# iDC-NEU/NeutronStarLite

Measured on NVIDIA H100. Metric: gcn_aggregated_edges_per_sec, higher is better.
Workload: dtype f32

## Files before the change

### include/nts_b200.h

```cpp
#ifndef NTS_B200_H
#define NTS_B200_H

#include <stddef.h>
#include <stdint.h>

#ifdef __cplusplus
extern "C" {
#endif

typedef uint32_t nts_vid_t;

int nts_version(void);
const char *nts_last_error(void);
int nts_device_count(void);
int nts_set_device(int device);
int nts_device_sm_count(int *sm_count);
int nts_device_synchronize(void);
int nts_device_reset(void);

void *nts_malloc_device(size_t bytes);
int nts_free_device(void *ptr);
void *nts_malloc_pinned(size_t bytes);
int nts_free_pinned(void *ptr);
void *nts_pinned_device_pointer(void *host_ptr);
int nts_memcpy_h2d(void *dst_device, const void *src_host, size_t bytes, void *stream, int sync);
int nts_memcpy_d2h(void *dst_host, const void *src_device, size_t bytes, void *stream, int sync);
int nts_memcpy_d2d(void *dst_device, const void *src_device, size_t bytes, void *stream);
int nts_zero(void *device_ptr, size_t bytes, void *stream);

void *nts_stream_create(int non_blocking);
int nts_stream_destroy(void *stream);
int nts_stream_synchronize(void *stream);
void *nts_event_create(int with_timing);
int nts_event_destroy(void *event);
int nts_event_record(void *event, void *stream);
int nts_stream_wait_event(void *stream, void *event);
int nts_event_elapsed_ms(void *start, void *stop, float *ms);

int nts_segment_gather_sum(const float *input, float *output, const float *weight,
                           const nts_vid_t *indices, const nts_vid_t *offsets, nts_vid_t index_base,
                           nts_vid_t n_rows, uint64_t n_edges, nts_vid_t feature_size, void *stream);

int nts_gather_by_dst_from_src(const float *input, float *output, const float *weight_forward,
                               const nts_vid_t *row_indices, const nts_vid_t *column_offset,
                               nts_vid_t src_start, nts_vid_t src_end, nts_vid_t dst_start,
                               nts_vid_t dst_end, nts_vid_t edges, nts_vid_t batch_size,
                               nts_vid_t feature_size, int with_weight, void *stream);

int nts_gather_by_src_from_dst(const float *input, float *output, const float *weight_backward,
                               const nts_vid_t *row_offset, const nts_vid_t *column_indices,
                               nts_vid_t src_start, nts_vid_t src_end, nts_vid_t dst_start,
                               nts_vid_t dst_end, nts_vid_t edges, nts_vid_t batch_size,
                               nts_vid_t feature_size, int with_weight, void *stream);

int nts_segment_gather_sum_range(const float *input, float *output, const float *weight, const nts_vid_t *indices,
                                 const nts_vid_t *offsets, const nts_vid_t *slot_of, nts_vid_t index_base,
                                 nts_vid_t n_rows, uint64_t edge_begin, uint64_t edge_end, nts_vid_t feature_size,
                                 void *stream);

typedef struct nts_gather_plan nts_gather_plan;
int nts_gather_plan_pick_slabs(nts_vid_t gather_rows, uint64_t n_edges, nts_vid_t n_rows, nts_vid_t feature_size,
                               uint64_t l2_budget_bytes );
nts_gather_plan *nts_gather_plan_create(const nts_vid_t *offsets, const nts_vid_t *indices, const float *weight,
                                        const nts_vid_t *slot_of, nts_vid_t index_base, nts_vid_t n_rows,
                                        uint64_t n_edges, nts_vid_t gather_rows, int n_slabs, void *stream);
nts_gather_plan *nts_gather_plan_create_hybrid(const nts_vid_t *offsets, const nts_vid_t *indices,
                                               const float *weight, const nts_vid_t *slot_of, nts_vid_t index_base,
                                               nts_vid_t n_rows, uint64_t n_edges, nts_vid_t gather_rows, int n_slabs,
                                               int n_hub_cols, int n_hub_rows, void *stream);
nts_gather_plan *nts_gather_plan_create_tuned(const nts_vid_t *offsets, const nts_vid_t *indices, const float *weight,
                                              const nts_vid_t *slot_of, nts_vid_t index_base, nts_vid_t n_rows,
                                              uint64_t n_edges, nts_vid_t gather_rows, nts_vid_t feature_size,
                                              void *stream);
typedef struct nts_plan_part {
  const nts_vid_t *offsets, *indices;
  const float *weight;
  const nts_vid_t *slot_of;
  nts_vid_t index_base, index_add, n_rows, row_add;
  uint64_t n_edges;
} nts_plan_part;
nts_gather_plan *nts_gather_plan_create_parts(const nts_plan_part *parts, int n_parts, nts_vid_t n_rows,
                                              nts_vid_t gather_rows, int n_slabs, nts_vid_t feature_size, void *stream);
float nts_gather_plan_tuned_ms(const nts_gather_plan *plan);
int nts_gather_plan_destroy(nts_gather_plan *plan);
int nts_gather_plan_slabs(const nts_gather_plan *plan);
int nts_gather_plan_hubs(const nts_gather_plan *plan, int *cols, int *rows);
int nts_gather_plan_overlap(const nts_gather_plan *plan);
int nts_gather_plan_set_overlap(nts_gather_plan *plan, int overlap);
uint64_t nts_gather_plan_bytes(const nts_gather_plan *plan);
int nts_gather_plan_run(nts_gather_plan *plan, const float *input, float *output, nts_vid_t feature_size,
                        void *stream);
int nts_gather_plan_last_launch(const nts_gather_plan *plan, int *launches, int *grid, int *k, int *u, int *outv);
enum { NTS_DTYPE_F32 = 0, NTS_DTYPE_BF16 = 1 };
int nts_gather_plan_run_bf16(nts_gather_plan *plan, const void *input, int input_dtype, float *output,
                             nts_vid_t feature_size, void *stream);
nts_gather_plan *nts_gather_plan_create_tuned_bf16(const nts_vid_t *offsets, const nts_vid_t *indices,
                                                   const float *weight, const nts_vid_t *slot_of, nts_vid_t index_base,
                                                   nts_vid_t n_rows, uint64_t n_edges, nts_vid_t gather_rows,
                                                   nts_vid_t feature_size, void *stream);
int nts_gather_plan_set_tuning(int u, int min_blocks, int edges_per_warp);
int nts_gather_plan_set_variant(int variant);

int nts_segment_gather_sum_slots(const float *input, float *output, const float *weight,
                                 const nts_vid_t *indices, const nts_vid_t *offsets,
                                 const nts_vid_t *slot_of, nts_vid_t n_rows, uint64_t n_edges,
                                 nts_vid_t feature_size, void *stream);

int nts_segment_gather_sum_heads(const float *input, float *output, const float *weight,
                                 const nts_vid_t *indices, const nts_vid_t *offsets, const nts_vid_t *slot_of,
                                 nts_vid_t index_base, nts_vid_t n_rows, uint64_t n_edges,
                                 nts_vid_t feature_size, nts_vid_t heads, void *stream);

int nts_aggregate_set_variant(int variant, int edges_per_warp);
int nts_aggregate_last_launch(int *grid, int *block, int *smem_bytes, int *variant);
uint64_t nts_kernel_launch_count(void);

int nts_scatter_src_mirror_to_msg(float *message, const float *src_mirror_feature,
                                  const nts_vid_t *row_indices, const nts_vid_t *column_offset,
                                  const nts_vid_t *mirror_index, nts_vid_t batch_size,
                                  nts_vid_t feature_size, void *stream);
int nts_gather_msg_to_src_mirror(float *src_mirror_feature, const float *message,
                                 const nts_vid_t *row_indices, const nts_vid_t *column_offset,
                                 const nts_vid_t *mirror_index, nts_vid_t batch_size,
                                 nts_vid_t feature_size, void *stream);
int nts_scatter_dst_to_msg(float *message, const float *dst_feature, const nts_vid_t *row_indices,
                           const nts_vid_t *column_offset, nts_vid_t batch_size,
                           nts_vid_t feature_size, void *stream);
int nts_gather_msg_to_dst(float *dst_feature, const float *message, const nts_vid_t *row_indices,
                          const nts_vid_t *column_offset, nts_vid_t batch_size,
                          nts_vid_t feature_size, void *stream);
int nts_edge_softmax_forward(float *msg_output, const float *msg_input, float *msg_cached,
                             const nts_vid_t *row_indices, const nts_vid_t *column_offset,
                             nts_vid_t batch_size, nts_vid_t feature_size, void *stream);
int nts_edge_softmax_backward(float *msg_input_grad, const float *msg_output_grad,
                              const float *msg_cached, const nts_vid_t *row_indices,
                              const nts_vid_t *column_offset, nts_vid_t batch_size,
                              nts_vid_t feature_size, void *stream);
int nts_scatter_grad_back_to_message(const float *input, float *message_grad,
                                     const nts_vid_t *row_indices, const nts_vid_t *column_offset,
                                     nts_vid_t batch_size, nts_vid_t feature_size, void *stream);

int nts_aggregate_dst_fuse_weight_backward(float *mirror_grad, float *edge_weight_grad,
                                           const float *mirror, const float *edge_weight,
                                           const float *dst_grad, const nts_vid_t *row_indices,
                                           const nts_vid_t *column_offset,
                                           const nts_vid_t *mirror_index, nts_vid_t batch_size,
                                           nts_vid_t feature_size, void *stream);
int nts_aggregate_dst_fuse_weight_backward_heads(float *mirror_grad, float *edge_weight_grad,
                                                 const float *mirror, const float *edge_weight,
                                                 const float *dst_grad, const nts_vid_t *row_indices,
                                                 const nts_vid_t *column_offset,
                                                 const nts_vid_t *mirror_index, nts_vid_t batch_size,
                                                 nts_vid_t feature_size, nts_vid_t heads, void *stream);

int nts_gat_softmax_stats(float *seg_max, float *seg_sum, const float *src_score, const float *dst_score,
                          const nts_vid_t *row_indices, const nts_vid_t *column_offset,
                          const nts_vid_t *mirror_index, nts_vid_t batch_size, nts_vid_t heads,
                          float negative_slope, void *stream);
int nts_gat_fused_aggregate_forward(const float *mirror, float *output, const float *src_score,
                                    const float *dst_score, const float *seg_max, const float *seg_sum,
                                    const nts_vid_t *row_indices, const nts_vid_t *column_offset,
                                    const nts_vid_t *mirror_index, nts_vid_t batch_size, uint64_t n_edges,
                                    nts_vid_t feature_size, nts_vid_t heads, float negative_slope, void *stream);
int nts_gat_fused_aggregate_backward(float *mirror_grad, float *src_score_grad, float *dst_score_grad,
                                     const float *mirror, const float *src_score, const float *dst_score,
                                     const float *seg_max, const float *seg_sum, const float *out_dot_grad,
                                     const float *dst_grad, const nts_vid_t *row_indices,
                                     const nts_vid_t *column_offset, const nts_vid_t *mirror_index,
                                     nts_vid_t batch_size, nts_vid_t feature_size, nts_vid_t heads,
                                     float negative_slope, void *stream);
int nts_gat_fused_aggregate_backward_two_pass(float *mirror_grad, float *src_score_grad, float *dst_score_grad,
                                              float *dst_pack, const float *mirror, const float *src_score,
                                              const float *dst_score, const float *seg_max, const float *seg_sum,
                                              const float *out_dot_grad, const float *dst_grad,
                                              const nts_vid_t *row_indices, const nts_vid_t *column_offset,
                                              const nts_vid_t *mirror_index, const nts_vid_t *slot_row_offset,
                                              const nts_vid_t *slot_column_indices, nts_vid_t batch_size,
                                              nts_vid_t mirror_size, nts_vid_t feature_size, nts_vid_t heads,
                                              float negative_slope, void *stream);
int nts_gat_fused_aggregate_forward_bf16(const void *mirror, float *output, const float *src_score,
                                         const float *dst_score, const float *seg_max, const float *seg_sum,
                                         const nts_vid_t *row_indices, const nts_vid_t *column_offset,
                                         const nts_vid_t *mirror_index, nts_vid_t batch_size, uint64_t n_edges,
                                         nts_vid_t feature_size, nts_vid_t ld, nts_vid_t heads, float negative_slope,
                                         void *stream);
int nts_gat_fused_aggregate_backward_two_pass_bf16(float *mirror_grad, float *src_score_grad, float *dst_score_grad,
                                                   float *dst_pack, const void *mirror, const float *src_score,
                                                   const float *dst_score, const float *seg_max, const float *seg_sum,
                                                   const float *out_dot_grad, const void *dst_grad,
                                                   const nts_vid_t *row_indices, const nts_vid_t *column_offset,
                                                   const nts_vid_t *mirror_index, const nts_vid_t *slot_row_offset,
                                                   const nts_vid_t *slot_column_indices, nts_vid_t batch_size,
                                                   nts_vid_t mirror_size, nts_vid_t feature_size, nts_vid_t ld,
                                                   nts_vid_t heads, float negative_slope, void *stream);
int nts_rows_to_bf16(const void *src, int src_dtype, nts_vid_t lds, void *dst, nts_vid_t n_rows, nts_vid_t feature_size,
                     nts_vid_t ld, void *stream);

int nts_deserialize_records(float *mirror, const float *records, nts_vid_t n_records,
                            nts_vid_t feature_size, nts_vid_t partition_start,
                            nts_vid_t partition_end, void *stream);
int nts_aggregate_records(float *aggregate, const float *records, nts_vid_t n_records,
                          nts_vid_t feature_size, nts_vid_t partition_start,
                          nts_vid_t partition_end, void *stream);

int nts_gather_rows(float *dst, const float *src, const nts_vid_t *rows, nts_vid_t n_rows,
                    nts_vid_t feature_size, void *stream);
int nts_scatter_add_rows(float *dst, const float *src, const nts_vid_t *rows, nts_vid_t n_rows,
                         nts_vid_t feature_size, void *stream);
int nts_scatter_add_rows_atomic(float *dst, const float *src, const nts_vid_t *rows, nts_vid_t n_rows,
                                nts_vid_t feature_size, void *stream);

int nts_adam_update(float *W, float *M, float *V, const float *grad, uint64_t n, float weight_decay, float beta1,
                    float beta2, float alpha, float epsilon, void *stream);

#define NTS_IPC_HANDLE_BYTES 64
int nts_ipc_get_handle(void *device_ptr, unsigned char handle[NTS_IPC_HANDLE_BYTES]);
void *nts_ipc_open_handle(const unsigned char handle[NTS_IPC_HANDLE_BYTES]);
int nts_ipc_close_handle(void *peer_ptr);
int nts_signal_set(uint32_t *flag, uint32_t value, void *stream);
int nts_signal_wait_geq(const uint32_t *flag, uint32_t value, void *stream);

typedef struct nts_exchange nts_exchange;
typedef struct nts_exchange_chunk {
  const nts_vid_t *column_offset;
  const nts_vid_t *slots;
  const float *weight_forward;
  const nts_vid_t *row_offset_compact;
  const nts_vid_t *column_indices;
  const float *weight_backward;
  uint64_t edges;
} nts_exchange_chunk;
typedef struct nts_exchange_desc {
  int partitions, rank;
  nts_vid_t owned_vertices, dst_start;
  const nts_vid_t *local_column_offset, *local_row_indices, *local_row_offset, *local_column_indices;
  const float *local_weight_forward, *local_weight_backward;
  nts_vid_t local_edges;
  const nts_exchange_chunk *chunks;
  const nts_vid_t *need_count;
  const nts_vid_t *send_count;
  const nts_vid_t *send_rows_all;
  const nts_vid_t *fwd_push_offset;
  const nts_vid_t *bwd_push_offset;
  const nts_vid_t *local_need;
  nts_vid_t local_need_count;
} nts_exchange_desc;

nts_exchange *nts_exchange_create(const nts_exchange_desc *desc);
int nts_exchange_destroy(nts_exchange *ex);
uint64_t nts_exchange_required_floats(const nts_exchange *ex, nts_vid_t feature_size);
uint64_t nts_exchange_required_floats_bf16(const nts_exchange *ex, nts_vid_t feature_size);
uint64_t nts_exchange_capacity_floats(const nts_exchange *ex);
int nts_exchange_release_peers(nts_exchange *ex);
int nts_exchange_reserve(nts_exchange *ex, uint64_t floats_per_buffer, int n_buffers);
int nts_exchange_handles(nts_exchange *ex, unsigned char window_handle[64], unsigned char flags_handle[64]);
int nts_exchange_open_peers(nts_exchange *ex, const unsigned char *window_handles, const unsigned char *flag_handles);
int nts_exchange_forward(nts_exchange *ex, const float *x, float *y, nts_vid_t feature_size, void *stream);
int nts_exchange_backward(nts_exchange *ex, const float *g, float *dx, nts_vid_t feature_size, void *stream);
int nts_exchange_forward_bf16(nts_exchange *ex, const void *x, int x_dtype, float *y, nts_vid_t feature_size,
                              void *stream);
int nts_exchange_backward_bf16(nts_exchange *ex, const float *g, float *dx, nts_vid_t feature_size, void *stream);
int nts_exchange_set_trace(nts_exchange *ex, int enable);
int nts_exchange_last_timeline(nts_exchange *ex, float *ms, int capacity);
int nts_exchange_fetch_mirrors(nts_exchange *ex, const float *x, float *mirror, nts_vid_t feature_size, void *stream);
int nts_exchange_return_mirror_grads(nts_exchange *ex, const float *mirror_grad, float *dx, nts_vid_t feature_size,
                                     void *stream);

typedef struct nts_host_chunk {
  const nts_vid_t *column_offset, *row_indices, *row_offset, *column_indices;
  const float *edge_weight_forward, *edge_weight_backward;
  nts_vid_t src_start, src_end, dst_start, dst_end;
  uint64_t edges;
} nts_host_chunk;
typedef struct nts_exchange_plan nts_exchange_plan;
nts_exchange_plan *nts_exchange_plan_create(const nts_host_chunk *chunks, int partitions, int rank);
void nts_exchange_plan_destroy(nts_exchange_plan *plan);
const nts_vid_t *nts_exchange_plan_need(const nts_exchange_plan *plan, int i, nts_vid_t *count);
uint64_t nts_exchange_plan_packed_rows(const nts_exchange_plan *plan);
int nts_exchange_plan_pack_needs(const nts_exchange_plan *plan, nts_vid_t *need_counts, nts_vid_t *need_rows);
int nts_exchange_plan_set_peer_needs(nts_exchange_plan *plan, int j, const nts_vid_t *need_counts,
                                     const nts_vid_t *need_rows);
int nts_exchange_plan_finalize(nts_exchange_plan *plan);
typedef struct nts_exchange_plan_view {
  int partitions, rank;
  nts_vid_t owned_vertices, recv_total, send_total, backward_rows;
  uint64_t remote_edges;
  const nts_vid_t *need_count, *send_count, *peer_bwd_offset;
  const nts_vid_t *fwd_push_offset, *bwd_push_offset;
  const nts_vid_t *remote_column_offset, *remote_slots;
  const float *remote_weight;
  const nts_vid_t *backward_offsets, *backward_indices;
  const float *backward_weight;
  const nts_vid_t *send_rows_all;
} nts_exchange_plan_view;
int nts_exchange_plan_get_view(const nts_exchange_plan *plan, nts_exchange_plan_view *view);
int nts_exchange_plan_chunk(const nts_exchange_plan *plan, int i, const nts_vid_t **slots,
                            const nts_vid_t **row_offset_compact);
typedef struct nts_device_chunk {
  const nts_vid_t *column_offset, *row_indices, *row_offset, *column_indices;
  const float *edge_weight_forward, *edge_weight_backward;
} nts_device_chunk;
nts_exchange *nts_exchange_create_from_plan(nts_exchange_plan *plan, const nts_device_chunk *device_chunks);

int nts_host_degrees(const nts_vid_t *edges_src_dst, uint64_t n_edges, nts_vid_t n_vertices,
                     nts_vid_t *out_degree, nts_vid_t *in_degree);
int nts_host_partition_offsets(const nts_vid_t *edges_src_dst, uint64_t n_edges, nts_vid_t n_vertices,
                               int partitions, nts_vid_t *partition_offset);
int nts_host_chunk_edge_counts(const nts_vid_t *edges_src_dst, uint64_t n_edges,
                               const nts_vid_t *partition_offset, int partitions, int rank,
                               uint64_t *counts);
int nts_host_build_chunk(const nts_vid_t *edges_src_dst, uint64_t n_edges, nts_vid_t n_vertices,
                         const nts_vid_t *partition_offset, int partitions, int rank, int src_partition,
                         const nts_vid_t *out_degree, const nts_vid_t *in_degree,
                         nts_vid_t *column_offset, nts_vid_t *row_indices, float *edge_weight_forward,
                         nts_vid_t *row_offset, nts_vid_t *column_indices, float *edge_weight_backward,
                         unsigned char *source_active);
int nts_host_mirror_index(const nts_vid_t *edges_src_dst, uint64_t n_edges, nts_vid_t n_vertices,
                          const nts_vid_t *partition_offset, int rank, nts_vid_t *mirror_index,
                          nts_vid_t *owned);

typedef struct nts_graph_build nts_graph_build;
enum { NTS_GRAPH_BUILD_DIST = 1 };
enum { NTS_INDEX_I32 = 0, NTS_INDEX_I64 = 1 };
nts_graph_build *nts_graph_build_from_file(const char *path, nts_vid_t n_vertices, int partitions, int rank,
                                           const nts_vid_t *partition_offset, uint64_t block_edges, int flags,
                                           void *stream);
nts_graph_build *nts_graph_build_from_device(const void *src, const void *dst, int index_dtype, uint64_t n_edges,
                                             nts_vid_t n_vertices, int partitions, int rank,
                                             const nts_vid_t *partition_offset, const void *out_degree,
                                             const void *in_degree, int flags, void *stream);
int nts_graph_build_info(const nts_graph_build *build, nts_vid_t *partition_offset, uint64_t *chunk_edges,
                         nts_vid_t *owned_mirrors, uint64_t *scratch_peak_bytes, double *pass_seconds);
int nts_graph_build_export_chunk(const nts_graph_build *build, int i, nts_vid_t *column_offset, nts_vid_t *row_indices,
                                 float *edge_weight_forward, nts_vid_t *row_offset, nts_vid_t *column_indices,
                                 float *edge_weight_backward, unsigned char *source_active, void *stream);
int nts_graph_build_export_dist(const nts_graph_build *build, nts_vid_t *mirror_index, nts_vid_t *column_offset,
                                nts_vid_t *row_indices, void *stream);
int nts_graph_build_export_degrees(const nts_graph_build *build, nts_vid_t *out_degree, nts_vid_t *in_degree,
                                   void *stream);
int nts_graph_build_destroy(nts_graph_build *build);

int nts_host_read_feature_label_mask(const char *feature_path, const char *label_path, const char *mask_path,
                                     nts_vid_t feature_size, nts_vid_t v_begin, nts_vid_t v_end, float *features,
                                     int64_t *labels, int32_t *masks);
int nts_host_read_feature_binary(const char *path, nts_vid_t feature_size, nts_vid_t v_begin, nts_vid_t v_end,
                                 float *features);

#ifdef __cplusplus
}
#endif
#endif
```

### neutronstarlite_b200/_lib.py

```python
from __future__ import annotations

import ctypes as C
import os
import re

PKG = os.path.dirname(os.path.abspath(__file__))
ROOT = os.path.dirname(PKG)
LIB_PATH = os.path.join(PKG, "lib", "libnts_b200.so")
HEADER = os.path.join(ROOT, "include", "nts_b200.h")

_vp = C.c_void_p
_u32 = C.c_uint32
_u64 = C.c_uint64
_int = C.c_int
_sz = C.c_size_t

SIGNATURES = {
    "nts_version": (_int, []),
    "nts_last_error": (C.c_char_p, []),
    "nts_device_count": (_int, []),
    "nts_set_device": (_int, [_int]),
    "nts_device_sm_count": (_int, [C.POINTER(_int)]),
    "nts_device_synchronize": (_int, []),
    "nts_device_reset": (_int, []),
    "nts_malloc_device": (_vp, [_sz]),
    "nts_free_device": (_int, [_vp]),
    "nts_malloc_pinned": (_vp, [_sz]),
    "nts_free_pinned": (_int, [_vp]),
    "nts_pinned_device_pointer": (_vp, [_vp]),
    "nts_memcpy_h2d": (_int, [_vp, _vp, _sz, _vp, _int]),
    "nts_memcpy_d2h": (_int, [_vp, _vp, _sz, _vp, _int]),
    "nts_memcpy_d2d": (_int, [_vp, _vp, _sz, _vp]),
    "nts_zero": (_int, [_vp, _sz, _vp]),
    "nts_stream_create": (_vp, [_int]),
    "nts_stream_destroy": (_int, [_vp]),
    "nts_stream_synchronize": (_int, [_vp]),
    "nts_event_create": (_vp, [_int]),
    "nts_event_destroy": (_int, [_vp]),
    "nts_event_record": (_int, [_vp, _vp]),
    "nts_stream_wait_event": (_int, [_vp, _vp]),
    "nts_event_elapsed_ms": (_int, [_vp, _vp, C.POINTER(C.c_float)]),
    "nts_segment_gather_sum": (_int, [_vp, _vp, _vp, _vp, _vp, _u32, _u32, _u64, _u32, _vp]),
    "nts_gather_by_dst_from_src": (_int, [_vp, _vp, _vp, _vp, _vp, _u32, _u32, _u32, _u32, _u32, _u32, _u32, _int, _vp]),
    "nts_gather_by_src_from_dst": (_int, [_vp, _vp, _vp, _vp, _vp, _u32, _u32, _u32, _u32, _u32, _u32, _u32, _int, _vp]),
    "nts_segment_gather_sum_range": (_int, [_vp, _vp, _vp, _vp, _vp, _vp, _u32, _u32, _u64, _u64, _u32, _vp]),
    "nts_gather_plan_pick_slabs": (_int, [_u32, _u64, _u32, _u32, _u64]),
    "nts_gather_plan_create": (_vp, [_vp, _vp, _vp, _vp, _u32, _u32, _u64, _u32, _int, _vp]),
    "nts_gather_plan_create_hybrid": (_vp, [_vp, _vp, _vp, _vp, _u32, _u32, _u64, _u32, _int, _int, _int, _vp]),
    "nts_gather_plan_create_tuned": (_vp, [_vp, _vp, _vp, _vp, _u32, _u32, _u64, _u32, _u32, _vp]),
    "nts_gather_plan_create_parts": (_vp, [_vp, _int, _u32, _u32, _int, _u32, _vp]),
    "nts_gather_plan_tuned_ms": (C.c_float, [_vp]),
    "nts_gather_plan_destroy": (_int, [_vp]),
    "nts_gather_plan_slabs": (_int, [_vp]),
    "nts_gather_plan_hubs": (_int, [_vp, C.POINTER(_int), C.POINTER(_int)]),
    "nts_gather_plan_overlap": (_int, [_vp]),
    "nts_gather_plan_set_overlap": (_int, [_vp, _int]),
    "nts_gather_plan_bytes": (_u64, [_vp]),
    "nts_gather_plan_run": (_int, [_vp, _vp, _vp, _u32, _vp]),
    "nts_gather_plan_run_bf16": (_int, [_vp, _vp, _int, _vp, _u32, _vp]),
    "nts_gather_plan_create_tuned_bf16": (_vp, [_vp, _vp, _vp, _vp, _u32, _u32, _u64, _u32, _u32, _vp]),
    "nts_gather_plan_last_launch": (_int, [_vp] + [C.POINTER(_int)] * 5),
    "nts_gather_plan_set_tuning": (_int, [_int, _int, _int]),
    "nts_gather_plan_set_variant": (_int, [_int]),
    "nts_segment_gather_sum_slots": (_int, [_vp, _vp, _vp, _vp, _vp, _vp, _u32, _u64, _u32, _vp]),
    "nts_segment_gather_sum_heads": (_int, [_vp, _vp, _vp, _vp, _vp, _vp, _u32, _u32, _u64, _u32, _u32, _vp]),
    "nts_aggregate_set_variant": (_int, [_int, _int]),
    "nts_aggregate_last_launch": (_int, [C.POINTER(_int)] * 4),
    "nts_kernel_launch_count": (_u64, []),
    "nts_scatter_src_mirror_to_msg": (_int, [_vp, _vp, _vp, _vp, _vp, _u32, _u32, _vp]),
    "nts_gather_msg_to_src_mirror": (_int, [_vp, _vp, _vp, _vp, _vp, _u32, _u32, _vp]),
    "nts_scatter_dst_to_msg": (_int, [_vp, _vp, _vp, _vp, _u32, _u32, _vp]),
    "nts_gather_msg_to_dst": (_int, [_vp, _vp, _vp, _vp, _u32, _u32, _vp]),
    "nts_edge_softmax_forward": (_int, [_vp, _vp, _vp, _vp, _vp, _u32, _u32, _vp]),
    "nts_edge_softmax_backward": (_int, [_vp, _vp, _vp, _vp, _vp, _u32, _u32, _vp]),
    "nts_scatter_grad_back_to_message": (_int, [_vp, _vp, _vp, _vp, _u32, _u32, _vp]),
    "nts_aggregate_dst_fuse_weight_backward": (_int, [_vp, _vp, _vp, _vp, _vp, _vp, _vp, _vp, _u32, _u32, _vp]),
    "nts_aggregate_dst_fuse_weight_backward_heads": (_int, [_vp] * 8 + [_u32, _u32, _u32, _vp]),
    "nts_gat_softmax_stats": (_int, [_vp] * 7 + [_u32, _u32, C.c_float, _vp]),
    "nts_gat_fused_aggregate_forward": (_int, [_vp] * 9 + [_u32, _u64, _u32, _u32, C.c_float, _vp]),
    "nts_gat_fused_aggregate_backward": (_int, [_vp] * 13 + [_u32, _u32, _u32, C.c_float, _vp]),
    "nts_gat_fused_aggregate_backward_two_pass": (_int, [_vp] * 16 + [_u32, _u32, _u32, _u32, C.c_float, _vp]),
    "nts_gat_fused_aggregate_forward_bf16": (_int, [_vp] * 9 + [_u32, _u64, _u32, _u32, _u32, C.c_float, _vp]),
    "nts_gat_fused_aggregate_backward_two_pass_bf16": (_int, [_vp] * 16 + [_u32] * 5 + [C.c_float, _vp]),
    "nts_rows_to_bf16": (_int, [_vp, _int, _u32, _vp, _u32, _u32, _u32, _vp]),
    "nts_deserialize_records": (_int, [_vp, _vp, _u32, _u32, _u32, _u32, _vp]),
    "nts_aggregate_records": (_int, [_vp, _vp, _u32, _u32, _u32, _u32, _vp]),
    "nts_gather_rows": (_int, [_vp, _vp, _vp, _u32, _u32, _vp]),
    "nts_scatter_add_rows": (_int, [_vp, _vp, _vp, _u32, _u32, _vp]),
    "nts_scatter_add_rows_atomic": (_int, [_vp, _vp, _vp, _u32, _u32, _vp]),
    "nts_ipc_get_handle": (_int, [_vp, C.c_char_p]),
    "nts_ipc_open_handle": (_vp, [C.c_char_p]),
    "nts_ipc_close_handle": (_int, [_vp]),
    "nts_adam_update": (_int, [_vp, _vp, _vp, _vp, _u64] + [C.c_float] * 5 + [_vp]),
    "nts_signal_set": (_int, [_vp, _u32, _vp]),
    "nts_signal_wait_geq": (_int, [_vp, _u32, _vp]),
    "nts_host_degrees": (_int, [_vp, _u64, _u32, _vp, _vp]),
    "nts_host_partition_offsets": (_int, [_vp, _u64, _u32, _int, _vp]),
    "nts_host_chunk_edge_counts": (_int, [_vp, _u64, _vp, _int, _int, _vp]),
    "nts_host_build_chunk": (_int, [_vp, _u64, _u32, _vp, _int, _int, _int, _vp, _vp, _vp, _vp, _vp, _vp, _vp, _vp, _vp]),
    "nts_host_mirror_index": (_int, [_vp, _u64, _u32, _vp, _int, _vp, _vp]),
    "nts_host_read_feature_label_mask": (_int, [C.c_char_p, C.c_char_p, C.c_char_p, _u32, _u32, _u32, _vp, _vp, _vp]),
    "nts_host_read_feature_binary": (_int, [C.c_char_p, _u32, _u32, _u32, _vp]),
    "nts_graph_build_from_file": (_vp, [C.c_char_p, _u32, _int, _int, _vp, _u64, _int, _vp]),
    "nts_graph_build_from_device": (_vp, [_vp, _vp, _int, _u64, _u32, _int, _int, _vp, _vp, _vp, _int, _vp]),
    "nts_graph_build_info": (_int, [_vp] * 6),
    "nts_graph_build_export_chunk": (_int, [_vp, _int] + [_vp] * 8),
    "nts_graph_build_export_dist": (_int, [_vp] * 5),
    "nts_graph_build_export_degrees": (_int, [_vp] * 4),
    "nts_graph_build_destroy": (_int, [_vp]),
}



class ExchangeChunk(C.Structure):
    _fields_ = [
        ("column_offset", _vp), ("slots", _vp), ("weight_forward", _vp), ("row_offset_compact", _vp),
        ("column_indices", _vp), ("weight_backward", _vp), ("edges", _u64),
    ]


class ExchangeDesc(C.Structure):
    _fields_ = [
        ("partitions", _int), ("rank", _int), ("owned_vertices", _u32), ("dst_start", _u32),
        ("local_column_offset", _vp), ("local_row_indices", _vp), ("local_row_offset", _vp),
        ("local_column_indices", _vp), ("local_weight_forward", _vp), ("local_weight_backward", _vp),
        ("local_edges", _u32),
        ("chunks", C.POINTER(ExchangeChunk)),
        ("need_count", C.POINTER(_u32)), ("send_count", C.POINTER(_u32)),
        ("send_rows_all", _vp), ("fwd_push_offset", C.POINTER(_u32)), ("bwd_push_offset", C.POINTER(_u32)),
        ("local_need", _vp), ("local_need_count", _u32),
    ]


class DeviceChunk(C.Structure):
    _fields_ = [
        ("column_offset", _vp), ("row_indices", _vp), ("row_offset", _vp), ("column_indices", _vp),
        ("edge_weight_forward", _vp), ("edge_weight_backward", _vp),
    ]


SIGNATURES.update({
    "nts_exchange_create": (_vp, [C.POINTER(ExchangeDesc)]),
    "nts_exchange_destroy": (_int, [_vp]),
    "nts_exchange_required_floats": (_u64, [_vp, _u32]),
    "nts_exchange_capacity_floats": (_u64, [_vp]),
    "nts_exchange_release_peers": (_int, [_vp]),
    "nts_exchange_reserve": (_int, [_vp, _u64, _int]),
    "nts_exchange_handles": (_int, [_vp, C.c_char_p, C.c_char_p]),
    "nts_exchange_open_peers": (_int, [_vp, C.c_char_p, C.c_char_p]),
    "nts_exchange_forward": (_int, [_vp, _vp, _vp, _u32, _vp]),
    "nts_exchange_backward": (_int, [_vp, _vp, _vp, _u32, _vp]),
    "nts_exchange_forward_bf16": (_int, [_vp, _vp, _int, _vp, _u32, _vp]),
    "nts_exchange_backward_bf16": (_int, [_vp, _vp, _vp, _u32, _vp]),
    "nts_exchange_required_floats_bf16": (_u64, [_vp, _u32]),
    "nts_exchange_set_trace": (_int, [_vp, _int]),
    "nts_exchange_last_timeline": (_int, [_vp, C.POINTER(C.c_float), _int]),
    "nts_exchange_fetch_mirrors": (_int, [_vp, _vp, _vp, _u32, _vp]),
    "nts_exchange_return_mirror_grads": (_int, [_vp, _vp, _vp, _u32, _vp]),
})



class HostChunk(C.Structure):
    _fields_ = [
        ("column_offset", _vp), ("row_indices", _vp), ("row_offset", _vp), ("column_indices", _vp),
        ("edge_weight_forward", _vp), ("edge_weight_backward", _vp),
        ("src_start", _u32), ("src_end", _u32), ("dst_start", _u32), ("dst_end", _u32), ("edges", _u64),
    ]


class ExchangePlanView(C.Structure):
    _fields_ = [
        ("partitions", _int), ("rank", _int),
        ("owned_vertices", _u32), ("recv_total", _u32), ("send_total", _u32), ("backward_rows", _u32),
        ("remote_edges", _u64),
        ("need_count", C.POINTER(_u32)), ("send_count", C.POINTER(_u32)), ("peer_bwd_offset", C.POINTER(_u32)),
        ("fwd_push_offset", C.POINTER(_u32)), ("bwd_push_offset", C.POINTER(_u32)),
        ("remote_column_offset", C.POINTER(_u32)), ("remote_slots", C.POINTER(_u32)),
        ("remote_weight", C.POINTER(C.c_float)),
        ("backward_offsets", C.POINTER(_u32)), ("backward_indices", C.POINTER(_u32)),
        ("backward_weight", C.POINTER(C.c_float)),
        ("send_rows_all", C.POINTER(_u32)),
    ]


SIGNATURES.update({
    "nts_exchange_plan_create": (_vp, [C.POINTER(HostChunk), _int, _int]),
    "nts_exchange_plan_destroy": (None, [_vp]),
    "nts_exchange_plan_need": (C.POINTER(_u32), [_vp, _int, C.POINTER(_u32)]),
    "nts_exchange_plan_packed_rows": (_u64, [_vp]),
    "nts_exchange_plan_pack_needs": (_int, [_vp, _vp, _vp]),
    "nts_exchange_plan_set_peer_needs": (_int, [_vp, _int, _vp, _vp]),
    "nts_exchange_plan_finalize": (_int, [_vp]),
    "nts_exchange_plan_get_view": (_int, [_vp, C.POINTER(ExchangePlanView)]),
    "nts_exchange_plan_chunk": (_int, [_vp, _int, C.POINTER(C.POINTER(_u32)), C.POINTER(C.POINTER(_u32))]),
    "nts_exchange_create_from_plan": (_vp, [_vp, C.POINTER(DeviceChunk)]),
})

_lib = None


class NtsError(RuntimeError):
    pass


def header_symbols():
    text = open(HEADER).read()
    text = re.sub(r"/\*.*?\*/", "", text, flags=re.S)
    return sorted(set(re.findall(r"\b(nts_[a-z0-9_]+)\s*\(", text)))


def load():
    global _lib
    if _lib is not None:
        return _lib
    if not os.path.exists(LIB_PATH):
        raise NtsError("libnts_b200.so not found at %s - run `python -m neutronstarlite_b200.build` "
                       "(there is no CPU fallback)" % LIB_PATH)
    lib = C.CDLL(LIB_PATH, mode=C.RTLD_GLOBAL)
    for name, (res, args) in SIGNATURES.items():
        fn = getattr(lib, name)
        fn.restype = res
        fn.argtypes = args
    _lib = lib
    return lib


def check(rc, what=""):
    if rc != 0:
        msg = load().nts_last_error().decode(errors="replace")
        raise NtsError("libnts_b200 %s failed (rc=%d): %s" % (what, rc, msg))


def call(name, *args):
    rc = getattr(load(), name)(*args)
    check(rc, name)
```

### neutronstarlite_b200/csrc/nts_common.cuh

```cuda
#pragma once
#include <cuda_bf16.h>
#include <cuda_runtime.h>
#include <stdint.h>
#include <stdio.h>
#include <stdlib.h>
#include <string.h>

#include "nts_b200.h"

namespace nts {

char *last_error_buffer();
bool abort_on_error();
void count_launch();

inline int fail(int code, const char *what, const char *file, int line) {
  snprintf(last_error_buffer(), 512, "%s (%s:%d)", what, file, line);
  if (abort_on_error()) {
    fprintf(stderr, "libnts_b200: %s\n", last_error_buffer());
    exit(1);
  }
  return code;
}

#define NTS_CUDA_OK(expr)                                                                         \
  do {                                                                                            \
    cudaError_t nts_e_ = (expr);                                                                  \
    if (nts_e_ != cudaSuccess)                                                                    \
      return ::nts::fail((int)nts_e_, cudaGetErrorString(nts_e_), __FILE__, __LINE__);            \
  } while (0)

#define NTS_ARG_CHECK(cond, msg)                                                                  \
  do {                                                                                            \
    if (!(cond))                                                                                  \
      return ::nts::fail(-1, msg, __FILE__, __LINE__);                                            \
  } while (0)

#define NTS_LAUNCH_CHECK()                                                                        \
  do {                                                                                            \
    ::nts::count_launch();                                                                        \
    NTS_CUDA_OK(cudaGetLastError());                                                              \
  } while (0)

inline cudaStream_t as_stream(void *s) { return reinterpret_cast<cudaStream_t>(s); }

inline bool aligned_to(const void *p, size_t a) { return (reinterpret_cast<uintptr_t>(p) & (a - 1)) == 0; }

int sm_count();

int run_plan_bf16(nts_gather_plan *pl, const void *input, int dtype, uint32_t lds, float *output, uint32_t F,
                  cudaStream_t st);
int to_bf16_rows(const void *src, int dtype, uint32_t lds, void *dst, uint32_t n_rows, uint32_t F, uint32_t ld,
                 cudaStream_t st);

int check_gat_bf16_layout(uint32_t F, uint32_t ld, uint32_t heads);

struct __align__(16) float8v {
  float4 lo, hi;
};

template <int VEC> struct Vec;
template <> struct Vec<1> { using type = float; };
template <> struct Vec<2> { using type = float2; };
template <> struct Vec<4> { using type = float4; };
template <> struct Vec<8> { using type = float8v; };

template <class T, int VEC> struct Ld { using type = typename Vec<VEC>::type; };
template <> struct Ld<__nv_bfloat16, 2> { using type = uint32_t; };
template <> struct Ld<__nv_bfloat16, 4> { using type = uint2; };
template <> struct Ld<__nv_bfloat16, 8> { using type = uint4; };
__device__ __forceinline__ float widen(float v) { return v; }
__device__ __forceinline__ float2 widen(float2 v) { return v; }
__device__ __forceinline__ float4 widen(float4 v) { return v; }
__device__ __forceinline__ float2 widen(uint32_t u) {
  return make_float2(__uint_as_float(u << 16), __uint_as_float(u & 0xffff0000u));
}
__device__ __forceinline__ float4 widen(uint2 u) {
  const float2 a = widen(u.x), b = widen(u.y);
  return make_float4(a.x, a.y, b.x, b.y);
}
__device__ __forceinline__ float8v widen(uint4 u) { return {widen(make_uint2(u.x, u.y)), widen(make_uint2(u.z, u.w))}; }

}

extern "C" nts_gather_plan *nts_plan_create_parts_typed(const nts_plan_part *parts, int n_parts, nts_vid_t n_rows,
                                                        nts_vid_t gather_rows, int n_slabs, nts_vid_t feature_size,
                                                        int bf16, void *stream);
```

### neutronstarlite_b200/csrc/nts_plan.cu

```cuda
#include <cub/cub.cuh>
#include <cuda_bf16.h>

#include <algorithm>
#include <type_traits>
#include <vector>

#include "nts_common.cuh"

struct nts_gather_plan {
  uint32_t n_rows = 0;
  uint64_t n_edges = 0;
  uint32_t gather_rows = 0;
  int slabs = 1;
  uint32_t slab_rows = 0;
  uint2 *pairs = nullptr;
  uint32_t *voff = nullptr;
  std::vector<uint64_t> slab_edge;
  float *workspace = nullptr;
  size_t workspace_floats = 0;
  __nv_bfloat16 *workspace_bf16 = nullptr;
  size_t workspace_bf16_elems = 0;
  int hub_cols = 0, hub_rows = 0;
  uint32_t *hub_col_ids = nullptr;
  uint32_t *hub_row_ids = nullptr;
  uint32_t lda_c = 0, lda_r = 0;
  float *dense = nullptr;
  size_t dense_floats = 0;
  int overlap = 0;
  int last_grid = 0, last_launches = 0, last_k = 0, last_u = 0, last_outv = 0;
  float tuned_ms = 0.f;
};

namespace nts {

static int g_plan_u = 0, g_plan_minb = 0, g_plan_q = 0, g_plan_variant = 0;

__device__ __forceinline__ uint32_t plan_find_row(const uint32_t *__restrict__ off, uint32_t n_rows, uint32_t e) {
  uint32_t lo = 0, hi = n_rows;
  while (hi - lo > 1) {
    uint32_t mid = lo + ((hi - lo) >> 1);
    if (__ldg(off + mid) <= e)
      lo = mid;
    else
      hi = mid;
  }
  return lo;
}

__global__ void plan_keys_kernel(const uint32_t *__restrict__ off, const uint32_t *__restrict__ idx,
                                 const uint32_t *__restrict__ slot_of, uint32_t base, uint32_t n_rows, uint32_t n_edges,
                                 uint32_t slab_rows, uint32_t slabs, uint32_t *__restrict__ key,
                                 uint32_t *__restrict__ val) {
  for (uint64_t e = (uint64_t)blockIdx.x * blockDim.x + threadIdx.x; e < n_edges; e += (uint64_t)gridDim.x * blockDim.x) {
    const uint32_t r = plan_find_row(off, n_rows, (uint32_t)e);
    const uint32_t id = __ldg(idx + e);
    const uint32_t g = slot_of ? __ldg(slot_of + id) : id - base;
    uint32_t s = g / slab_rows;
    if (s >= slabs)
      s = slabs - 1;
    key[e] = s * n_rows + r;
    val[e] = (uint32_t)e;
  }
}

__global__ void plan_pairs_kernel(const uint32_t *__restrict__ perm, const uint32_t *__restrict__ idx,
                                  const float *__restrict__ w, const uint32_t *__restrict__ slot_of, uint32_t base,
                                  uint32_t n_edges, uint2 *__restrict__ pairs) {
  for (uint64_t i = (uint64_t)blockIdx.x * blockDim.x + threadIdx.x; i < n_edges; i += (uint64_t)gridDim.x * blockDim.x) {
    const uint32_t e = perm ? __ldg(perm + i) : (uint32_t)i;
    const uint32_t id = __ldg(idx + e);
    const uint32_t g = slot_of ? __ldg(slot_of + id) : id - base;
    const float wt = w ? __ldg(w + e) : 1.f;
    pairs[i] = make_uint2(g, __float_as_uint(wt));
  }
}

__global__ void plan_part_keys_kernel(const uint32_t *__restrict__ off, const uint32_t *__restrict__ idx,
                                      const uint32_t *__restrict__ slot_of, const float *__restrict__ w, uint32_t base,
                                      uint32_t index_add, uint32_t n_rows_part, uint32_t row_add, uint32_t n_edges,
                                      uint32_t e_off, uint32_t n_rows_total, uint32_t slab_rows, uint32_t slabs,
                                      uint32_t *__restrict__ key, uint32_t *__restrict__ val,
                                      uint2 *__restrict__ unsorted) {
  for (uint64_t e = (uint64_t)blockIdx.x * blockDim.x + threadIdx.x; e < n_edges; e += (uint64_t)gridDim.x * blockDim.x) {
    const uint32_t r = plan_find_row(off, n_rows_part, (uint32_t)e) + row_add;
    const uint32_t id = __ldg(idx + e);
    const uint32_t g = (slot_of ? __ldg(slot_of + id) : id - base) + index_add;
    uint32_t s = g / slab_rows;
    if (s >= slabs)
      s = slabs - 1;
    key[e_off + e] = s * n_rows_total + r;
    val[e_off + e] = e_off + (uint32_t)e;
    unsorted[e_off + e] = make_uint2(g, __float_as_uint(w ? __ldg(w + e) : 1.f));
  }
}
__global__ void plan_permute_pairs_kernel(const uint32_t *__restrict__ perm, const uint2 *__restrict__ unsorted,
                                          uint32_t n_edges, uint2 *__restrict__ pairs) {
  for (uint64_t i = (uint64_t)blockIdx.x * blockDim.x + threadIdx.x; i < n_edges; i += (uint64_t)gridDim.x * blockDim.x)
    pairs[i] = unsorted[__ldg(perm + i)];
}

template <class KeyT>
__global__ void plan_offsets_kernel(const KeyT *__restrict__ sorted_key, uint32_t n_edges, uint32_t n_keys,
                                    uint32_t *__restrict__ voff) {
  for (uint64_t k = (uint64_t)blockIdx.x * blockDim.x + threadIdx.x; k <= n_keys; k += (uint64_t)gridDim.x * blockDim.x) {
    uint32_t lo = 0, hi = n_edges;
    while (lo < hi) {
      uint32_t mid = lo + ((hi - lo) >> 1);
      if (__ldg(sorted_key + mid) < (KeyT)k)
        lo = mid + 1;
      else
        hi = mid;
    }
    voff[k] = lo;
  }
}

constexpr uint32_t kNoHub = 0xffffffffu;

__global__ void plan_ref_count_kernel(const uint32_t *__restrict__ idx, const uint32_t *__restrict__ slot_of,
                                      uint32_t base, uint32_t n_edges, uint32_t *__restrict__ cnt) {
  for (uint64_t e = (uint64_t)blockIdx.x * blockDim.x + threadIdx.x; e < n_edges; e += (uint64_t)gridDim.x * blockDim.x) {
    const uint32_t id = __ldg(idx + e);
    atomicAdd(cnt + (slot_of ? __ldg(slot_of + id) : id - base), 1u);
  }
}

__global__ void plan_hybrid_keys_kernel(const uint32_t *__restrict__ off, const uint32_t *__restrict__ idx,
                                        const uint32_t *__restrict__ slot_of, uint32_t base, uint32_t n_rows,
                                        uint32_t n_edges, uint32_t slab_rows, uint32_t slabs,
                                        const uint32_t *__restrict__ col_slot, const uint32_t *__restrict__ row_slot,
                                        uint32_t lda_c, uint64_t dc_cells, uint32_t lda_r, uint64_t *__restrict__ key,
                                        uint32_t *__restrict__ val) {
  const uint64_t n_keys = (uint64_t)slabs * n_rows;
  for (uint64_t e = (uint64_t)blockIdx.x * blockDim.x + threadIdx.x; e < n_edges; e += (uint64_t)gridDim.x * blockDim.x) {
    const uint32_t r = plan_find_row(off, n_rows, (uint32_t)e);
    const uint32_t id = __ldg(idx + e);
    const uint32_t g = slot_of ? __ldg(slot_of + id) : id - base;
    const uint32_t cs = __ldg(col_slot + g), rs = __ldg(row_slot + r);
    uint64_t k;
    if (cs != kNoHub) {
      k = n_keys + (uint64_t)cs * lda_c + r;
    } else if (rs != kNoHub) {
      k = n_keys + dc_cells + (uint64_t)g * lda_r + rs;
    } else {
      uint32_t s = g / slab_rows;
      if (s >= slabs)
        s = slabs - 1;
      k = (uint64_t)s * n_rows + r;
    }
    key[e] = k;
    val[e] = (uint32_t)e;
  }
}

__global__ void plan_cell_sum_kernel(const uint64_t *__restrict__ cell_key, const uint32_t *__restrict__ run_start,
                                     const uint32_t *__restrict__ run_len, uint32_t n_runs,
                                     const uint32_t *__restrict__ perm, const float *__restrict__ w, uint64_t n_keys,
                                     float *__restrict__ dense) {
  const uint32_t lane = threadIdx.x & 31;
  for (uint64_t run = ((uint64_t)blockIdx.x * blockDim.x + threadIdx.x) >> 5; run < n_runs;
       run += ((uint64_t)gridDim.x * blockDim.x) >> 5) {
    const uint32_t b = __ldg(run_start + run), n = __ldg(run_len + run);
    float s = 0.f;
    for (uint32_t j = lane; j < n; j += 32)
      s += w ? __ldg(w + __ldg(perm + b + j)) : 1.f;
#pragma unroll
    for (int o = 16; o > 0; o >>= 1)
      s += __shfl_xor_sync(0xffffffffu, s, o);
    if (lane == 0)
      dense[__ldg(cell_key + run) - n_keys] = s;
  }
}

__global__ void pad_rows_kernel(const float *__restrict__ src, float *__restrict__ dst, uint32_t n_rows, uint32_t F,
                                uint32_t ld) {
  const uint64_t total = (uint64_t)n_rows * ld;
  for (uint64_t i = (uint64_t)blockIdx.x * blockDim.x + threadIdx.x; i < total; i += (uint64_t)gridDim.x * blockDim.x) {
    const uint64_t r = i / ld;
    const uint32_t c = (uint32_t)(i - r * ld);
    dst[i] = c < F ? __ldg(src + r * F + c) : 0.f;
  }
}

template <class S>
__global__ void bf16_rows_kernel(const S *__restrict__ src, uint32_t lds, uint4 *__restrict__ dst, uint32_t n_rows,
                                 uint32_t F, uint32_t ld) {
  const uint32_t ld8 = ld / 8;
  const uint64_t total = (uint64_t)n_rows * ld8;
  for (uint64_t i = (uint64_t)blockIdx.x * blockDim.x + threadIdx.x; i < total; i += (uint64_t)gridDim.x * blockDim.x) {
    const uint64_t r = i / ld8;
    const uint32_t c = (uint32_t)(i - r * ld8) * 8;
    const S *s = src + r * lds;
    uint32_t w[4];
#pragma unroll
    for (int j = 0; j < 4; j++) {
      const uint32_t c0 = c + 2 * j, c1 = c0 + 1;
      if constexpr (std::is_same<S, float>::value) {
        const __nv_bfloat162 h = __floats2bfloat162_rn(c0 < F ? __ldg(s + c0) : 0.f, c1 < F ? __ldg(s + c1) : 0.f);
        w[j] = *reinterpret_cast<const uint32_t *>(&h);
      } else {
        const uint16_t *u = reinterpret_cast<const uint16_t *>(s);
        w[j] = (c0 < F ? (uint32_t)__ldg(u + c0) : 0u) | ((c1 < F ? (uint32_t)__ldg(u + c1) : 0u) << 16);
      }
    }
    dst[i] = make_uint4(w[0], w[1], w[2], w[3]);
  }
}

__device__ __forceinline__ uint32_t p_smem_u32(const void *p) { return (uint32_t)__cvta_generic_to_shared(p); }
__device__ __forceinline__ void p_mbar_init(uint64_t *bar, uint32_t count) {
  asm volatile("mbarrier.init.shared::cta.b64 [%0], %1;" ::"r"(p_smem_u32(bar)), "r"(count));
}
__device__ __forceinline__ void p_mbar_expect_tx(uint64_t *bar, uint32_t bytes) {
  asm volatile("mbarrier.arrive.expect_tx.shared::cta.b64 _, [%0], %1;" ::"r"(p_smem_u32(bar)), "r"(bytes) : "memory");
}
__device__ __forceinline__ void p_mbar_wait(uint64_t *bar, uint32_t parity) {
  asm volatile("{\n\t"
               ".reg .pred p;\n\t"
               "WAIT_%=:\n\t"
               "mbarrier.try_wait.parity.shared::cta.b64 p, [%0], %1;\n\t"
               "@p bra DONE_%=;\n\t"
               "bra WAIT_%=;\n\t"
               "DONE_%=:\n\t"
               "}" ::"r"(p_smem_u32(bar)),
               "r"(parity)
               : "memory");
}
__device__ __forceinline__ void p_bulk_g2s(void *smem_dst, const void *gmem_src, uint32_t bytes, uint64_t *bar) {
  asm volatile("cp.async.bulk.shared::cluster.global.mbarrier::complete_tx::bytes [%0], [%1], %2, [%3];" ::"r"(
                   p_smem_u32(smem_dst)),
               "l"(gmem_src), "r"(bytes), "r"(p_smem_u32(bar))
               : "memory");
}

constexpr int kPlanWarps = 8;

template <int OUTV, bool ATOMIC>
__device__ __forceinline__ void flush_chunk(float *__restrict__ orow, uint32_t col, uint32_t F, float4 a) {
  if constexpr (OUTV == 4) {
    float4 *p = reinterpret_cast<float4 *>(orow + col);
    if constexpr (ATOMIC) {
      asm volatile("red.global.add.v4.f32 [%0], {%1, %2, %3, %4};" ::"l"(p), "f"(a.x), "f"(a.y), "f"(a.z), "f"(a.w)
                   : "memory");
    } else {
      float4 o = *p;
      o.x += a.x, o.y += a.y, o.z += a.z, o.w += a.w;
      *p = o;
    }
  } else if constexpr (OUTV == 2) {
    float2 *p = reinterpret_cast<float2 *>(orow + col);
    if constexpr (ATOMIC) {
      asm volatile("red.global.add.v2.f32 [%0], {%1, %2};" ::"l"(p), "f"(a.x), "f"(a.y) : "memory");
      if (col + 2 < F)
        asm volatile("red.global.add.v2.f32 [%0], {%1, %2};" ::"l"(p + 1), "f"(a.z), "f"(a.w) : "memory");
    } else {
      float2 o = p[0];
      o.x += a.x, o.y += a.y;
      p[0] = o;
      if (col + 2 < F) {
        float2 o1 = p[1];
        o1.x += a.z, o1.y += a.w;
        p[1] = o1;
      }
    }
  } else {
    const float v[4] = {a.x, a.y, a.z, a.w};
#pragma unroll
    for (int i = 0; i < 4; i++)
      if (col + i < F) {
        if constexpr (ATOMIC)
          atomicAdd(orow + col + i, v[i]);
        else
          orow[col + i] += v[i];
      }
  }
}

template <class T> struct GatherT;
template <> struct GatherT<float> {
  using chunk = float4;
  static constexpr int V = 4;
  __device__ static __forceinline__ void widen(const float4 &c, float (&v)[4]) {
    v[0] = c.x, v[1] = c.y, v[2] = c.z, v[3] = c.w;
  }
};
template <> struct GatherT<__nv_bfloat16> {
  using chunk = uint4;
  static constexpr int V = 8;
  __device__ static __forceinline__ void widen(const uint4 &c, float (&v)[8]) {
    const uint32_t u[4] = {c.x, c.y, c.z, c.w};
#pragma unroll
    for (int i = 0; i < 4; i++) {
      v[2 * i] = __uint_as_float(u[i] << 16);
      v[2 * i + 1] = __uint_as_float(u[i] & 0xffff0000u);
    }
  }
};

template <class T, int K, int U, int OUTV, int G>
__device__ __forceinline__ void planned_gather_body(unsigned char *smem_raw, uint32_t vblock,
                                                    const typename GatherT<T>::chunk *__restrict__ in, uint32_t ldc,
                                                    float *__restrict__ out, uint32_t F,
                                                    const uint2 *__restrict__ pairs, const uint32_t *__restrict__ off,
                                                    uint32_t n_rows, uint32_t e_begin, uint32_t e_end, uint32_t Q,
                                                    uint32_t tiles, uint32_t tile_vecs) {
  static_assert(G == 1 || K == 1, "virtual warps are for rows narrower than a warp");
  using Chunk = typename GatherT<T>::chunk;
  constexpr int V = GatherT<T>::V;
  constexpr uint32_t GS = 32 / G;
  const uint32_t lane = threadIdx.x & (GS - 1);
  const uint32_t vwarp_in_block = threadIdx.x / GS;
  const uint64_t gwarp = (uint64_t)vblock * (kPlanWarps * G) + vwarp_in_block;
  const uint32_t tile = (uint32_t)(gwarp % tiles);
  const uint64_t q = gwarp / tiles;
  const uint64_t e0_64 = e_begin + q * (uint64_t)Q;

  uint64_t *bar = reinterpret_cast<uint64_t *>(smem_raw);
  uint2 *s_pair = reinterpret_cast<uint2 *>(smem_raw + 16);
  uint32_t cta_e_base = 0, bulk_bytes = 0;
  {
    const uint64_t cta_w0 = (uint64_t)vblock * (kPlanWarps * G);
    const uint64_t first_q = cta_w0 / tiles;
    const uint64_t last_q = (cta_w0 + kPlanWarps * G - 1) / tiles;
    uint64_t ce0 = e_begin + first_q * (uint64_t)Q;
    uint64_t ce1 = e_begin + (last_q + 1) * (uint64_t)Q;
    if (ce1 > e_end)
      ce1 = e_end;
    if (ce0 < ce1) {
      cta_e_base = (uint32_t)(ce0 & ~1ull);
      const uint32_t n_el = (uint32_t)(ce1 - cta_e_base);
      bulk_bytes = (n_el * 8u) & ~15u;
      if (threadIdx.x == 0) {
        p_mbar_init(bar, 1);
        asm volatile("fence.mbarrier_init.release.cluster;" ::: "memory");
        if (n_el & 1u)
          s_pair[n_el - 1] = __ldg(pairs + cta_e_base + n_el - 1);
      }
      __syncthreads();
      if (threadIdx.x == 0 && bulk_bytes) {
        p_mbar_expect_tx(bar, bulk_bytes);
        p_bulk_g2s(s_pair, pairs + cta_e_base, bulk_bytes, bar);
      }
    }
  }
  if (e0_64 >= e_end)
    return;
  const uint32_t e0 = (uint32_t)e0_64;
  const uint32_t e1 = (e0_64 + Q < e_end) ? e0 + Q : e_end;

  const uint32_t c0 = tile * tile_vecs + lane;
  bool act[K];
#pragma unroll
  for (int k = 0; k < K; k++)
    act[k] = (k * GS + lane) < tile_vecs && (c0 + k * GS) < ldc;

  uint32_t row = plan_find_row(off, n_rows, e0);
  uint32_t row_end = __ldg(off + row + 1);
  bool row_started_inside = __ldg(off + row) >= e0;

  float acc[K][V];
#pragma unroll
  for (int k = 0; k < K; k++)
#pragma unroll
    for (int j = 0; j < V; j++)
      acc[k][j] = 0.f;

  auto flush = [&](bool whole) {
    float *orow = out + (size_t)row * F;
#pragma unroll
    for (int k = 0; k < K; k++) {
#pragma unroll
      for (int h = 0; h < V; h += 4) {
        const uint32_t col = (c0 + k * GS) * V + h;
        const float4 a = make_float4(acc[k][h], acc[k][h + 1], acc[k][h + 2], acc[k][h + 3]);
        if (act[k] && col < F) {
          if (whole)
            flush_chunk<OUTV, false>(orow, col, F, a);
          else
            flush_chunk<OUTV, true>(orow, col, F, a);
        }
      }
#pragma unroll
      for (int j = 0; j < V; j++)
        acc[k][j] = 0.f;
    }
  };
  auto advance = [&](uint32_t ee) {
    flush(row_started_inside);
    do {
      row++;
      row_end = __ldg(off + row + 1);
    } while (ee >= row_end);
    row_started_inside = true;
  };

  if (bulk_bytes)
    p_mbar_wait(bar, 0);

  const uint2 *sp = s_pair - cta_e_base;
  uint32_t e = e0;
  auto fma_chunk = [&](int k, float w, const Chunk &c) {
    float x[V];
    GatherT<T>::widen(c, x);
#pragma unroll
    for (int j = 0; j < V; j++)
      acc[k][j] = fmaf(w, x[j], acc[k][j]);
  };
  for (; e + U <= e1; e += U) {
    Chunk v[U][K];
    float wu[U];
#pragma unroll
    for (int u = 0; u < U; u++) {
      const uint2 pr = sp[e + u];
      wu[u] = __uint_as_float(pr.y);
      const Chunk *p = in + (size_t)pr.x * ldc + c0;
#pragma unroll
      for (int k = 0; k < K; k++)
        if (act[k])
          v[u][k] = __ldg(p + k * GS);
    }
#pragma unroll
    for (int u = 0; u < U; u++) {
      if (e + u >= row_end)
        advance(e + u);
#pragma unroll
      for (int k = 0; k < K; k++)
        if (act[k])
          fma_chunk(k, wu[u], v[u][k]);
    }
  }
  for (; e < e1; e++) {
    const uint2 pr = sp[e];
    const float wj = __uint_as_float(pr.y);
    const Chunk *p = in + (size_t)pr.x * ldc + c0;
    Chunk v1[K];
#pragma unroll
    for (int k = 0; k < K; k++)
      if (act[k])
        v1[k] = __ldg(p + k * GS);
    if (e >= row_end)
      advance(e);
#pragma unroll
    for (int k = 0; k < K; k++)
      if (act[k])
        fma_chunk(k, wj, v1[k]);
  }
  flush(row_started_inside && row_end <= e1);
}

template <class T, int K, int U, int OUTV, int MINB, int G = 1>
__global__ void __launch_bounds__(kPlanWarps * 32, MINB)
    planned_gather_sum_kernel(const typename GatherT<T>::chunk *__restrict__ in, uint32_t ldc, float *__restrict__ out,
                              uint32_t F, const uint2 *__restrict__ pairs, const uint32_t *__restrict__ off,
                              uint32_t n_rows, uint32_t e_begin, uint32_t e_end, uint32_t Q, uint32_t tiles,
                              uint32_t tile_vecs) {
  extern __shared__ __align__(16) unsigned char smem_raw[];
  planned_gather_body<T, K, U, OUTV, G>(smem_raw, blockIdx.x, in, ldc, out, F, pairs, off, n_rows, e_begin, e_end, Q,
                                        tiles, tile_vecs);
}

struct PlanShape;
template <int K, int STAGES, int OUTV, int MINB>
__global__ void __launch_bounds__(kPlanWarps * 32, MINB)
    planned_gather_sum_tma_kernel(const float4 *__restrict__ in, uint32_t ld4, float *__restrict__ out, uint32_t F,
                                  const uint2 *__restrict__ pairs, const uint32_t *__restrict__ off, uint32_t n_rows,
                                  uint32_t e_begin, uint32_t e_end, uint32_t Q, uint32_t tiles, uint32_t tile_vecs,
                                  uint32_t pair_bytes) {
  const uint32_t lane = threadIdx.x & 31;
  const uint32_t warp_in_block = threadIdx.x >> 5;
  const uint64_t gwarp = (uint64_t)blockIdx.x * kPlanWarps + warp_in_block;
  const uint32_t tile = (uint32_t)(gwarp % tiles);
  const uint64_t q = gwarp / tiles;
  const uint64_t e0_64 = e_begin + q * (uint64_t)Q;

  extern __shared__ __align__(16) unsigned char smem_raw[];
  uint64_t *bar = reinterpret_cast<uint64_t *>(smem_raw);
  uint2 *s_pair = reinterpret_cast<uint2 *>(smem_raw + 16);
  const uint32_t ring_bytes = 8u * STAGES + 8u * (STAGES & 1) + STAGES * tile_vecs * 16u;
  unsigned char *ring = smem_raw + 16 + pair_bytes + (size_t)warp_in_block * ring_bytes;
  uint64_t *sbar = reinterpret_cast<uint64_t *>(ring);
  float4 *sbuf = reinterpret_cast<float4 *>(ring + 8u * STAGES + 8u * (STAGES & 1));
  uint32_t cta_e_base = 0, bulk_bytes = 0;
  {
    const uint64_t cta_w0 = (uint64_t)blockIdx.x * kPlanWarps;
    const uint64_t first_q = cta_w0 / tiles;
    const uint64_t last_q = (cta_w0 + kPlanWarps - 1) / tiles;
    uint64_t ce0 = e_begin + first_q * (uint64_t)Q;
    uint64_t ce1 = e_begin + (last_q + 1) * (uint64_t)Q;
    if (ce1 > e_end)
      ce1 = e_end;
    if (lane == 0)
      for (int s = 0; s < STAGES; s++)
        p_mbar_init(sbar + s, 1);
    if (ce0 < ce1) {
      cta_e_base = (uint32_t)(ce0 & ~1ull);
      const uint32_t n_el = (uint32_t)(ce1 - cta_e_base);
      bulk_bytes = (n_el * 8u) & ~15u;
      if (threadIdx.x == 0) {
        p_mbar_init(bar, 1);
        if (n_el & 1u)
          s_pair[n_el - 1] = __ldg(pairs + cta_e_base + n_el - 1);
      }
    }
    asm volatile("fence.mbarrier_init.release.cluster;" ::: "memory");
    __syncthreads();
    if (threadIdx.x == 0 && bulk_bytes) {
      p_mbar_expect_tx(bar, bulk_bytes);
      p_bulk_g2s(s_pair, pairs + cta_e_base, bulk_bytes, bar);
    }
  }
  if (e0_64 >= e_end)
    return;
  const uint32_t e0 = (uint32_t)e0_64;
  const uint32_t e1 = (e0_64 + Q < e_end) ? e0 + Q : e_end;
  const uint32_t c0 = tile * tile_vecs + lane;
  const uint32_t my_vecs = min(tile_vecs, ld4 - tile * tile_vecs);
  const uint32_t row_bytes = my_vecs * 16u;
  bool act[K];
#pragma unroll
  for (int k = 0; k < K; k++)
    act[k] = (k * 32 + lane) < my_vecs;

  uint32_t row = plan_find_row(off, n_rows, e0);
  uint32_t row_end = __ldg(off + row + 1);
  bool row_started_inside = __ldg(off + row) >= e0;
  float4 acc[K];
#pragma unroll
  for (int k = 0; k < K; k++)
    acc[k] = make_float4(0.f, 0.f, 0.f, 0.f);
  auto flush = [&](bool whole) {
    float *orow = out + (size_t)row * F;
#pragma unroll
    for (int k = 0; k < K; k++) {
      const uint32_t col = (c0 + k * 32) * 4;
      if (act[k] && col < F) {
        if (whole)
          flush_chunk<OUTV, false>(orow, col, F, acc[k]);
        else
          flush_chunk<OUTV, true>(orow, col, F, acc[k]);
      }
      acc[k] = make_float4(0.f, 0.f, 0.f, 0.f);
    }
  };
  auto advance = [&](uint32_t ee) {
    flush(row_started_inside);
    do {
      row++;
      row_end = __ldg(off + row + 1);
    } while (ee >= row_end);
    row_started_inside = true;
  };
  if (bulk_bytes)
    p_mbar_wait(bar, 0);
  const uint2 *sp = s_pair - cta_e_base;
  auto issue = [&](uint32_t e, uint32_t stage) {
    const uint32_t src_row = sp[e].x;
    p_mbar_expect_tx(sbar + stage, row_bytes);
    p_bulk_g2s(sbuf + (size_t)stage * tile_vecs, in + (size_t)src_row * ld4 + tile * tile_vecs, row_bytes, sbar + stage);
  };
  if (lane == 0)
    for (uint32_t s = 0; s < STAGES && e0 + s < e1; s++)
      issue(e0 + s, s);
  uint32_t stage = 0, parity = 0;
  for (uint32_t e = e0; e < e1; e++) {
    const float w = __uint_as_float(sp[e].y);
    p_mbar_wait(sbar + stage, parity);
    const float4 *b = sbuf + (size_t)stage * tile_vecs + lane;
    float4 v[K];
#pragma unroll
    for (int k = 0; k < K; k++)
      if (act[k])
        v[k] = b[k * 32];
    if (e >= row_end)
      advance(e);
#pragma unroll
    for (int k = 0; k < K; k++)
      if (act[k]) {
        acc[k].x = fmaf(w, v[k].x, acc[k].x);
        acc[k].y = fmaf(w, v[k].y, acc[k].y);
        acc[k].z = fmaf(w, v[k].z, acc[k].z);
        acc[k].w = fmaf(w, v[k].w, acc[k].w);
      }
    __syncwarp();
    if (lane == 0 && e + STAGES < e1)
      issue(e + STAGES, stage);
    if (++stage == STAGES) {
      stage = 0;
      parity ^= 1u;
    }
  }
  flush(row_started_inside && row_end <= e1);
}

template <int K, int STAGES, int OUTV, int MINB>
static int launch_planned_tma(nts_gather_plan *pl, const PlanShape &sh, const float4 *in, uint32_t ld4, float *out,
                              uint32_t F, uint32_t Q, cudaStream_t st);

struct PlanShape {
  int k, u, outv, minb, g;
  uint32_t tiles, tile_vecs;
};

template <class T, int K, int U, int OUTV, int MINB, int G = 1>
static int launch_planned(nts_gather_plan *pl, const PlanShape &sh, const T *in_rows, uint32_t ldc, float *out,
                          uint32_t F, uint32_t Q, cudaStream_t st) {
  auto kern = planned_gather_sum_kernel<T, K, U, OUTV, MINB, G>;
  const auto *in = reinterpret_cast<const typename GatherT<T>::chunk *>(in_rows);
  const size_t smem = 16 + ((size_t)kPlanWarps * G * Q + 4) * 8;
  NTS_CUDA_OK(cudaFuncSetAttribute(kern, cudaFuncAttributeMaxDynamicSharedMemorySize, (int)smem));
  pl->last_launches = 0;
  for (int s = 0; s < pl->slabs; s++) {
    const uint64_t eb = pl->slab_edge[s], ee = pl->slab_edge[s + 1];
    if (ee <= eb)
      continue;
    const uint64_t quanta = (ee - eb + Q - 1) / Q;
    const uint64_t blocks = (quanta * sh.tiles + kPlanWarps * G - 1) / (kPlanWarps * G);
    NTS_ARG_CHECK(blocks <= 0x7fffffffull, "aggregation grid too large");
    kern<<<(unsigned)blocks, kPlanWarps * 32, smem, st>>>(in, ldc, out, F, pl->pairs, pl->voff + (size_t)s * pl->n_rows,
                                                          pl->n_rows, (uint32_t)eb, (uint32_t)ee, Q, sh.tiles,
                                                          sh.tile_vecs);
    NTS_LAUNCH_CHECK();
    pl->last_grid = (int)blocks;
    pl->last_launches++;
  }
  return 0;
}

template <int K, int STAGES, int OUTV, int MINB>
static int launch_planned_tma(nts_gather_plan *pl, const PlanShape &sh, const float4 *in, uint32_t ld4, float *out,
                              uint32_t F, uint32_t Q, cudaStream_t st) {
  auto kern = planned_gather_sum_tma_kernel<K, STAGES, OUTV, MINB>;
  const uint32_t pair_bytes = (kPlanWarps * Q + 4) * 8;
  const uint32_t ring_bytes = 8u * STAGES + 8u * (STAGES & 1) + STAGES * sh.tile_vecs * 16u;
  const size_t smem = 16 + pair_bytes + (size_t)kPlanWarps * ring_bytes;
  NTS_ARG_CHECK(smem <= 227 * 1024, "row-staging ring does not fit shared memory");
  NTS_CUDA_OK(cudaFuncSetAttribute(kern, cudaFuncAttributeMaxDynamicSharedMemorySize, (int)smem));
  pl->last_launches = 0;
  for (int s = 0; s < pl->slabs; s++) {
    const uint64_t eb = pl->slab_edge[s], ee = pl->slab_edge[s + 1];
    if (ee <= eb)
      continue;
    const uint64_t quanta = (ee - eb + Q - 1) / Q;
    const uint64_t blocks = (quanta * sh.tiles + kPlanWarps - 1) / kPlanWarps;
    NTS_ARG_CHECK(blocks <= 0x7fffffffull, "aggregation grid too large");
    kern<<<(unsigned)blocks, kPlanWarps * 32, smem, st>>>(in, ld4, out, F, pl->pairs, pl->voff + (size_t)s * pl->n_rows,
                                                          pl->n_rows, (uint32_t)eb, (uint32_t)ee, Q, sh.tiles,
                                                          sh.tile_vecs, pair_bytes);
    NTS_LAUNCH_CHECK();
    pl->last_grid = (int)blocks;
    pl->last_launches++;
  }
  return 0;
}

#define NTS_PLAN_TMA_CASE(K_, S_, B_)                                                                               \
  if (sh.k == K_ && stages == S_ && sh.minb == B_) {                                                                \
    if (sh.outv == 4)                                                                                               \
      return launch_planned_tma<K_, S_, 4, B_>(pl, sh, in4, ld4, out, F, Q, st);                                    \
    if (sh.outv == 2)                                                                                               \
      return launch_planned_tma<K_, S_, 2, B_>(pl, sh, in4, ld4, out, F, Q, st);                                    \
    return launch_planned_tma<K_, S_, 1, B_>(pl, sh, in4, ld4, out, F, Q, st);                                      \
  }

#define NTS_PLAN_CASE_G(U_, B_, G_)                                                                                 \
  if (sh.k == 1 && sh.u == U_ && sh.minb == B_ && sh.g == G_) {                                                     \
    if (sh.outv == 4)                                                                                               \
      return launch_planned<T, 1, U_, 4, B_, G_>(pl, sh, in, ldc, out, F, Q, st);                                   \
    if (sh.outv == 2)                                                                                               \
      return launch_planned<T, 1, U_, 2, B_, G_>(pl, sh, in, ldc, out, F, Q, st);                                   \
    return launch_planned<T, 1, U_, 1, B_, G_>(pl, sh, in, ldc, out, F, Q, st);                                     \
  }

#define NTS_PLAN_CASE(K_, U_, B_)                                                                                   \
  if (sh.k == K_ && sh.u == U_ && sh.minb == B_) {                                                                  \
    if (sh.outv == 4)                                                                                               \
      return launch_planned<T, K_, U_, 4, B_>(pl, sh, in, ldc, out, F, Q, st);                                       \
    if (sh.outv == 2)                                                                                               \
      return launch_planned<T, K_, U_, 2, B_>(pl, sh, in, ldc, out, F, Q, st);                                       \
    return launch_planned<T, K_, U_, 1, B_>(pl, sh, in, ldc, out, F, Q, st);                                         \
  }

constexpr int kHubBM = 128, kHubBN = 128, kHubBK = 16, kHubThreads = 256;

__device__ __forceinline__ void p_cp_async16(void *smem_dst, const void *gmem_src, bool full) {
  asm volatile("cp.async.cg.shared.global [%0], [%1], 16, %2;" ::"r"(p_smem_u32(smem_dst)), "l"(gmem_src),
               "r"(full ? 16 : 0)
               : "memory");
}

template <int TN, class TB> struct HubSmem {
  static constexpr uint32_t kBN = 16 * TN;
  float As[2][kHubBK][kHubBM];
  TB Bs[2][kHubBK][kBN];
};

template <class TB, int OUTV, bool SPLIT, int TN, int KKU>
__device__ __forceinline__ void hub_gemm_tile(HubSmem<TN, TB> &sm, uint32_t tile, const float *__restrict__ At,
                                              uint32_t lda, uint32_t M, uint32_t k_lo, uint32_t k_hi, uint32_t k_split,
                                              const TB *__restrict__ B, uint32_t ldb,
                                              const uint32_t *__restrict__ colmap, float *__restrict__ out, uint32_t F,
                                              const uint32_t *__restrict__ rowmap, uint32_t m_tiles, uint32_t n_tiles) {
  constexpr bool kBf16 = std::is_same<TB, __nv_bfloat16>::value;
  constexpr uint32_t kBV = 16 / sizeof(TB);
  constexpr uint32_t kBN = HubSmem<TN, TB>::kBN;
  constexpr uint32_t kBChunks = kHubBK * kBN / kBV;
  auto &As = sm.As;
  auto &Bs = sm.Bs;
  const uint32_t t = threadIdx.x;
  const uint32_t n_tile = tile % n_tiles, rest = tile / n_tiles;
  const uint32_t m0 = (rest % m_tiles) * kHubBM, n0 = n_tile * kBN;
  const uint32_t k_begin = k_lo + (rest / m_tiles) * k_split;
  const uint32_t k_end = min(k_hi, k_begin + k_split);
  if (k_begin >= k_end)
    return;
  const uint32_t n_kt = (k_end - k_begin + kHubBK - 1) / kHubBK;

  auto load = [&](uint32_t kt, int buf) {
#pragma unroll
    for (int i = 0; i < 2; i++) {
      const uint32_t c = t + i * kHubThreads, kk = c >> 5, c4 = (c & 31) * 4;
      const uint32_t k = k_begin + kt * kHubBK + kk;
      const bool a_ok = k < k_end && m0 + c4 < lda;
      p_cp_async16(&As[buf][kk][c4], a_ok ? At + (size_t)k * lda + m0 + c4 : At, a_ok);
    }
#pragma unroll
    for (int i = 0; i < (int)((kBChunks + kHubThreads - 1) / kHubThreads); i++) {
      constexpr uint32_t kRowChunks = kBN / kBV;
      const uint32_t c = t + i * kHubThreads, kk = c / kRowChunks, cv = (c % kRowChunks) * kBV;
      if (kBChunks % kHubThreads != 0 && c >= kBChunks)
        break;
      const uint32_t k = k_begin + kt * kHubBK + kk;
      const bool b_ok = k < k_end && n0 + cv < ldb;
      const uint32_t brow = b_ok ? (colmap ? __ldg(colmap + k) : k) : 0;
      p_cp_async16(&Bs[buf][kk][cv], B + (size_t)brow * ldb + (b_ok ? n0 + cv : 0), b_ok);
    }
    asm volatile("cp.async.commit_group;" ::: "memory");
  };
  auto read_b4 = [&](int buf, int kk, uint32_t n) -> float4 {
    if constexpr (kBf16) {
      const uint2 u = *reinterpret_cast<const uint2 *>(&Bs[buf][kk][n]);
      return make_float4(__uint_as_float(u.x << 16), __uint_as_float(u.x & 0xffff0000u), __uint_as_float(u.y << 16),
                         __uint_as_float(u.y & 0xffff0000u));
    } else {
      return *reinterpret_cast<const float4 *>(&Bs[buf][kk][n]);
    }
  };

  const uint32_t tx = t & 15, ty = t >> 4;
  float acc[8][TN];
#pragma unroll
  for (int i = 0; i < 8; i++)
#pragma unroll
    for (int j = 0; j < TN; j++)
      acc[i][j] = 0.f;

  load(0, 0);
  for (uint32_t kt = 0; kt < n_kt; kt++) {
    const int buf = kt & 1;
    if (kt + 1 < n_kt) {
      load(kt + 1, buf ^ 1);
      asm volatile("cp.async.wait_group 1;" ::: "memory");
    } else {
      asm volatile("cp.async.wait_group 0;" ::: "memory");
    }
    __syncthreads();
#pragma unroll(KKU)
    for (int kk = 0; kk < kHubBK; kk++) {
      const float4 a0 = *reinterpret_cast<const float4 *>(&As[buf][kk][ty * 4]);
      const float4 a1 = *reinterpret_cast<const float4 *>(&As[buf][kk][64 + ty * 4]);
      const float a[8] = {a0.x, a0.y, a0.z, a0.w, a1.x, a1.y, a1.z, a1.w};
      float b[TN];
#pragma unroll
      for (int h = 0; h < TN / 4; h++) {
        const float4 bh = read_b4(buf, kk, h * 64 + tx * 4);
        b[4 * h] = bh.x, b[4 * h + 1] = bh.y, b[4 * h + 2] = bh.z, b[4 * h + 3] = bh.w;
      }
#pragma unroll
      for (int i = 0; i < 8; i++)
#pragma unroll
        for (int j = 0; j < TN; j++)
          acc[i][j] = fmaf(a[i], b[j], acc[i][j]);
    }
    __syncthreads();
  }

#pragma unroll
  for (int i = 0; i < 8; i++) {
    const uint32_t m = m0 + (i >> 2) * 64 + ty * 4 + (i & 3);
    if (m >= M)
      continue;
    float *orow = out + (size_t)(rowmap ? __ldg(rowmap + m) : m) * F;
#pragma unroll
    for (int j = 0; j < TN / 4; j++) {
      const uint32_t col = n0 + j * 64 + tx * 4;
      if (col < F)
        flush_chunk<OUTV, SPLIT>(orow, col, F,
                                 make_float4(acc[i][j * 4], acc[i][j * 4 + 1], acc[i][j * 4 + 2], acc[i][j * 4 + 3]));
    }
  }
}

template <class TB, int OUTV, bool SPLIT>
__global__ void __launch_bounds__(kHubThreads, 2)
    hub_block_gemm_kernel(const float *__restrict__ At, uint32_t lda, uint32_t M, uint32_t K, uint32_t k_split,
                          const TB *__restrict__ B, uint32_t ldb, const uint32_t *__restrict__ colmap,
                          float *__restrict__ out, uint32_t F, const uint32_t *__restrict__ rowmap, uint32_t m_tiles,
                          uint32_t n_tiles) {
  __shared__ __align__(16) HubSmem<8, TB> sm;
  hub_gemm_tile<TB, OUTV, SPLIT, 8, kHubBK>(sm, blockIdx.x, At, lda, M, 0, K, k_split, B, ldb, colmap, out, F, rowmap, m_tiles,
                                    n_tiles);
}

static uint32_t hub_row_k_split(uint32_t K, uint32_t m_tiles, uint32_t n_tiles) {
  const uint64_t want = (uint64_t)sm_count() * 2 * 4;
  const uint64_t splits = (want + (uint64_t)m_tiles * n_tiles - 1) / ((uint64_t)m_tiles * n_tiles);
  const uint32_t k_split = (uint32_t)((K + splits - 1) / splits);
  return std::max<uint32_t>((k_split + kHubBK - 1) / kHubBK * kHubBK, 16 * kHubBK);
}

template <class TB, int OUTV>
static int launch_hub_blocks(nts_gather_plan *pl, const TB *in, uint32_t ldb, float *out, uint32_t F, bool rows,
                             cudaStream_t st) {
  const uint32_t n_tiles = (F + kHubBN - 1) / kHubBN;
  if (pl->hub_cols) {
    const uint32_t m_tiles = (pl->n_rows + kHubBM - 1) / kHubBM;
    const uint64_t blocks = (uint64_t)m_tiles * n_tiles;
    NTS_ARG_CHECK(blocks <= 0x7fffffffull, "hub column block grid too large");
    hub_block_gemm_kernel<TB, OUTV, false><<<(unsigned)blocks, kHubThreads, 0, st>>>(
        pl->dense, pl->lda_c, pl->n_rows, (uint32_t)pl->hub_cols, (uint32_t)pl->hub_cols, in, ldb, pl->hub_col_ids, out,
        F, nullptr, m_tiles, n_tiles);
    NTS_LAUNCH_CHECK();
  }
  if (pl->hub_rows && rows) {
    const uint32_t m_tiles = (pl->hub_rows + kHubBM - 1) / kHubBM;
    const uint32_t K = pl->gather_rows;
    const uint32_t k_split = hub_row_k_split(K, m_tiles, n_tiles);
    const uint64_t splits = (K + k_split - 1) / k_split;
    hub_block_gemm_kernel<TB, OUTV, true><<<(unsigned)(splits * m_tiles * n_tiles), kHubThreads, 0, st>>>(
        pl->dense + (size_t)pl->hub_cols * pl->lda_c, pl->lda_r, (uint32_t)pl->hub_rows, K, k_split, in, ldb, nullptr,
        out, F, pl->hub_row_ids, m_tiles, n_tiles);
    NTS_LAUNCH_CHECK();
  }
  return 0;
}

struct HubRowArgs {
  const float *At;
  uint32_t lda, M;
  uint32_t k_lo, k_hi, k_split;
  const uint32_t *rowmap;
  uint32_t m_tiles, n_tiles, n_gemm;
  uint32_t period;
};

template <class T, int K, int U, int OUTV, int MINB, int G>
__global__ void __launch_bounds__(kPlanWarps * 32, MINB)
    planned_slab_hub_kernel(const typename GatherT<T>::chunk *__restrict__ in, uint32_t ldc, float *__restrict__ out,
                            uint32_t F, const uint2 *__restrict__ pairs, const uint32_t *__restrict__ off,
                            uint32_t n_rows, uint32_t e_begin, uint32_t e_end, uint32_t Q, uint32_t tiles,
                            uint32_t tile_vecs, const HubRowArgs hub) {
  static_assert(kPlanWarps * 32 == kHubThreads, "both bodies run 256 threads");
  constexpr int TN = MINB <= 2 ? 8 : 4;
  extern __shared__ __align__(16) unsigned char smem_raw[];
  const uint32_t b = blockIdx.x, grp = b / hub.period;
  if (grp < hub.n_gemm && b - grp * hub.period == hub.period - 1)
    hub_gemm_tile<T, OUTV, true, TN, TN == 8 ? kHubBK : 4>(
        *reinterpret_cast<HubSmem<TN, T> *>(smem_raw), grp, hub.At, hub.lda, hub.M, hub.k_lo, hub.k_hi, hub.k_split,
        reinterpret_cast<const T *>(in), ldc * GatherT<T>::V, nullptr, out, F, hub.rowmap, hub.m_tiles, hub.n_tiles);
  else
    planned_gather_body<T, K, U, OUTV, G>(smem_raw, b - min(grp, hub.n_gemm), in, ldc, out, F, pairs, off, n_rows,
                                          e_begin, e_end, Q, tiles, tile_vecs);
}

template <class T, int K, int U, int OUTV, int MINB, int G = 1>
static int launch_fused(nts_gather_plan *pl, const PlanShape &sh, const T *in_rows, uint32_t ldc, float *out,
                        uint32_t F, uint32_t Q, cudaStream_t st) {
  constexpr int TN = MINB <= 2 ? 8 : 4;
  auto kern = planned_slab_hub_kernel<T, K, U, OUTV, MINB, G>;
  const auto *in = reinterpret_cast<const typename GatherT<T>::chunk *>(in_rows);
  const size_t smem = std::max(16 + ((size_t)kPlanWarps * G * Q + 4) * 8, sizeof(HubSmem<TN, T>));
  NTS_CUDA_OK(cudaFuncSetAttribute(kern, cudaFuncAttributeMaxDynamicSharedMemorySize, (int)smem));
  HubRowArgs hub;
  hub.At = pl->dense + (size_t)pl->hub_cols * pl->lda_c;
  hub.lda = pl->lda_r;
  hub.M = (uint32_t)pl->hub_rows;
  hub.rowmap = pl->hub_row_ids;
  hub.m_tiles = (hub.M + kHubBM - 1) / kHubBM;
  hub.n_tiles = (F + 16 * TN - 1) / (16 * TN);
  hub.k_split = hub_row_k_split(pl->gather_rows, hub.m_tiles, hub.n_tiles);
  pl->last_launches = 0;
  for (int s = 0; s < pl->slabs; s++) {
    hub.k_lo = (uint32_t)std::min<uint64_t>((uint64_t)s * pl->slab_rows, pl->gather_rows);
    hub.k_hi = s + 1 == pl->slabs ? pl->gather_rows
                                  : (uint32_t)std::min<uint64_t>((uint64_t)(s + 1) * pl->slab_rows, pl->gather_rows);
    const uint64_t splits = hub.k_hi > hub.k_lo ? (hub.k_hi - hub.k_lo + hub.k_split - 1) / hub.k_split : 0;
    const uint64_t n_gemm = splits * hub.m_tiles * hub.n_tiles;
    const uint64_t eb = pl->slab_edge[s], ee = pl->slab_edge[s + 1];
    const uint64_t quanta = ee > eb ? (ee - eb + Q - 1) / Q : 0;
    const uint64_t blocks = n_gemm + (quanta * sh.tiles + kPlanWarps * G - 1) / (kPlanWarps * G);
    if (!blocks)
      continue;
    NTS_ARG_CHECK(blocks <= 0x7fffffffull, "aggregation grid too large");
    hub.n_gemm = (uint32_t)n_gemm;
    hub.period = n_gemm ? (uint32_t)(blocks / n_gemm) : 1;
    kern<<<(unsigned)blocks, kPlanWarps * 32, smem, st>>>(in, ldc, out, F, pl->pairs, pl->voff + (size_t)s * pl->n_rows,
                                                          pl->n_rows, (uint32_t)eb, (uint32_t)ee, Q, sh.tiles,
                                                          sh.tile_vecs, hub);
    NTS_LAUNCH_CHECK();
    pl->last_grid = (int)blocks;
    pl->last_launches++;
  }
  return 0;
}

#define NTS_PLAN_FUSED_CASE(K_, U_, B_, G_)                                                                         \
  if (sh.k == K_ && sh.u == U_ && sh.minb == B_ && sh.g == G_) {                                                    \
    if (sh.outv == 4)                                                                                               \
      return launch_fused<T, K_, U_, 4, B_, G_>(pl, sh, in, ldc, out, F, Q, st);                                    \
    if (sh.outv == 2)                                                                                               \
      return launch_fused<T, K_, U_, 2, B_, G_>(pl, sh, in, ldc, out, F, Q, st);                                    \
    return launch_fused<T, K_, U_, 1, B_, G_>(pl, sh, in, ldc, out, F, Q, st);                                      \
  }

template <class T>
static int run_gather(nts_gather_plan *pl, const T *in, uint32_t ld, float *output, uint32_t F, cudaStream_t st) {
  constexpr bool kBf16 = std::is_same<T, __nv_bfloat16>::value;
  PlanShape sh;
  const uint32_t ldc = ld / GatherT<T>::V;
  const uint32_t chunks = (ldc + 31) / 32;
  const uint32_t kmax = 5;
  sh.tiles = (chunks + kmax - 1) / kmax;
  sh.tile_vecs = (ldc + sh.tiles - 1) / sh.tiles;
  sh.k = (int)((sh.tile_vecs + 31) / 32);
  sh.tiles = (ldc + sh.tile_vecs - 1) / sh.tile_vecs;
  sh.outv = (F % 4 == 0 && aligned_to(output, 16)) ? 4 : ((F % 2 == 0 && aligned_to(output, 8)) ? 2 : 1);
  const bool fused = pl->overlap && pl->hub_rows;
  NTS_ARG_CHECK(!fused || g_plan_variant == 0, "the fused slab launches use the register-staging gather (variant 0)");
  if (pl->hub_cols || pl->hub_rows) {
    const int rc = sh.outv == 4   ? launch_hub_blocks<T, 4>(pl, in, ld, output, F, !fused, st)
                   : sh.outv == 2 ? launch_hub_blocks<T, 2>(pl, in, ld, output, F, !fused, st)
                                  : launch_hub_blocks<T, 1>(pl, in, ld, output, F, !fused, st);
    if (rc)
      return rc;
  }
  sh.g = ldc <= 8 ? 4 : (ldc <= 16 ? 2 : 1);
  if (g_plan_variant == 1 || getenv("NTS_PLAN_NO_SUBWARP"))
    sh.g = 1;
  sh.minb = sh.k >= 3 ? 2 : (sh.k == 2 ? 3 : 4);
  sh.u = sh.k == 4 ? 2 : 4;
  if constexpr (kBf16) {
    sh.minb = sh.k >= 4 ? 2 : (sh.k >= 2 ? 3 : 4);
    sh.u = sh.k == 1 ? 4 : 2;
  }
  {
    static int env_read = 0;
    if (!env_read) {
      env_read = 1;
      if (const char *t = getenv("NTS_PLAN_TUNE"))
        sscanf(t, "%d,%d,%d", &g_plan_u, &g_plan_minb, &g_plan_q);
    }
    if (g_plan_u > 0)
      sh.u = g_plan_u;
    if (g_plan_minb > 0)
      sh.minb = g_plan_minb;
  }
  uint32_t Q = g_plan_q > 0 ? (uint32_t)g_plan_q : 512u / sh.g;
  if (g_plan_q <= 0) {
    const uint64_t per_slab = pl->slab_edge[pl->slabs] / (uint64_t)pl->slabs + 1;
    const uint64_t want_warps = (uint64_t)sm_count() * 64 * sh.g;
    while (Q > 32 && ((per_slab + Q - 1) / Q) * sh.tiles < want_warps)
      Q >>= 1;
  }
  Q = (Q + 31u) & ~31u;
  if (Q * sh.g > 1024)
    Q = (1024 / sh.g) & ~31u;
  pl->last_k = sh.k, pl->last_u = sh.u, pl->last_outv = sh.outv;
  float *out = output;
  if (fused) {
    if constexpr (kBf16) {
      NTS_PLAN_FUSED_CASE(1, 4, 4, 2)
      NTS_PLAN_FUSED_CASE(1, 4, 4, 4)
      NTS_PLAN_FUSED_CASE(1, 4, 4, 1)
      NTS_PLAN_FUSED_CASE(2, 2, 3, 1)
      NTS_PLAN_FUSED_CASE(3, 2, 3, 1)
      NTS_PLAN_FUSED_CASE(4, 2, 2, 1)
      NTS_PLAN_FUSED_CASE(5, 2, 2, 1)
    } else {
      NTS_PLAN_FUSED_CASE(1, 4, 4, 2)
      NTS_PLAN_FUSED_CASE(1, 4, 4, 4)
      NTS_PLAN_FUSED_CASE(1, 4, 4, 1)
      NTS_PLAN_FUSED_CASE(2, 4, 3, 1)
      NTS_PLAN_FUSED_CASE(3, 4, 2, 1)
      NTS_PLAN_FUSED_CASE(4, 2, 2, 1)
      NTS_PLAN_FUSED_CASE(5, 4, 2, 1)
    }
    return fail(-1, "no fused slab/hub-row instantiation for this (chunks, U, occupancy) point", __FILE__, __LINE__);
  }
  if constexpr (kBf16) {
    NTS_PLAN_CASE_G(4, 4, 2)
    NTS_PLAN_CASE_G(4, 4, 4)
    NTS_PLAN_CASE_G(8, 2, 2)
    NTS_PLAN_CASE_G(8, 2, 4)
    if (sh.g != 1)
      return fail(-1, "no BF16 virtual-warp instantiation for this (U, occupancy) point", __FILE__, __LINE__);
    NTS_PLAN_CASE(1, 4, 4)
    NTS_PLAN_CASE(1, 8, 2)
    NTS_PLAN_CASE(2, 2, 3)
    NTS_PLAN_CASE(2, 4, 2)
    NTS_PLAN_CASE(3, 4, 2)
    NTS_PLAN_CASE(3, 2, 3)
    NTS_PLAN_CASE(3, 6, 1)
    NTS_PLAN_CASE(4, 2, 2)
    NTS_PLAN_CASE(4, 4, 2)
    NTS_PLAN_CASE(5, 2, 2)
    return fail(-1, "no BF16 planned-aggregation instantiation for this (chunks, U, occupancy) point", __FILE__,
                __LINE__);
  } else {
  const float4 *in4 = reinterpret_cast<const float4 *>(in);
  const uint32_t ld4 = ldc;
  if (g_plan_variant == 1) {
    const int stages = sh.u >= 8 ? 8 : (sh.u >= 4 ? 4 : 2);
    sh.minb = g_plan_minb > 0 ? g_plan_minb : (sh.k >= 4 ? 2 : 4);
    NTS_PLAN_TMA_CASE(1, 8, 4)
    NTS_PLAN_TMA_CASE(1, 4, 4)
    NTS_PLAN_TMA_CASE(1, 8, 3)
    NTS_PLAN_TMA_CASE(2, 4, 3)
    NTS_PLAN_TMA_CASE(2, 4, 2)
    NTS_PLAN_TMA_CASE(3, 4, 2)
    NTS_PLAN_TMA_CASE(4, 4, 2)
    NTS_PLAN_TMA_CASE(4, 2, 2)
    NTS_PLAN_TMA_CASE(5, 4, 2)
    NTS_PLAN_TMA_CASE(5, 2, 2)
    NTS_PLAN_TMA_CASE(5, 4, 1)
    NTS_PLAN_TMA_CASE(5, 8, 1)
    return fail(-1, "no TMA row-staging instantiation for this (chunks, stages, occupancy) point", __FILE__, __LINE__);
  }
  NTS_PLAN_CASE_G(4, 4, 2)
  NTS_PLAN_CASE_G(4, 4, 4)
  NTS_PLAN_CASE_G(8, 3, 2)
  NTS_PLAN_CASE_G(8, 3, 4)
  if (sh.g != 1)
    return fail(-1, "no virtual-warp instantiation for this (U, occupancy) point", __FILE__, __LINE__);
  NTS_PLAN_CASE(1, 8, 4)
  NTS_PLAN_CASE(1, 4, 4)
  NTS_PLAN_CASE(1, 8, 3)
  NTS_PLAN_CASE(1, 16, 2)
  NTS_PLAN_CASE(2, 4, 3)
  NTS_PLAN_CASE(2, 8, 2)
  NTS_PLAN_CASE(3, 4, 3)
  NTS_PLAN_CASE(3, 4, 2)
  NTS_PLAN_CASE(4, 2, 2)
  NTS_PLAN_CASE(4, 4, 2)
  NTS_PLAN_CASE(5, 2, 2)
  NTS_PLAN_CASE(5, 1, 3)
  NTS_PLAN_CASE(5, 2, 3)
  NTS_PLAN_CASE(5, 4, 1)
  NTS_PLAN_CASE(5, 4, 2)
  return fail(-1, "no planned-aggregation instantiation for this (chunks, U, occupancy) point", __FILE__, __LINE__);
  }
}

template <class E> static int ensure_workspace(E *&ws, size_t &have, size_t elems) {
  if (elems <= have)
    return 0;
  if (ws)
    NTS_CUDA_OK(cudaFree(ws));
  ws = nullptr;
  have = 0;
  NTS_CUDA_OK(cudaMalloc(reinterpret_cast<void **>(&ws), elems * sizeof(E)));
  have = elems;
  return 0;
}

static int run_plan(nts_gather_plan *pl, const float *input, float *output, uint32_t F, cudaStream_t st) {
  if (pl->n_rows == 0 || pl->n_edges == 0 || F == 0)
    return 0;
  NTS_ARG_CHECK(input && output, "null feature pointer");
  const uint32_t ld = (F + 3u) & ~3u;
  const float *in = input;
  if (ld != F || !aligned_to(input, 16)) {
    if (const int rc = ensure_workspace(pl->workspace, pl->workspace_floats, (size_t)pl->gather_rows * ld))
      return rc;
    const uint64_t total = (uint64_t)pl->gather_rows * ld;
    const unsigned blocks = (unsigned)std::min<uint64_t>((total + 255) / 256, (uint64_t)sm_count() * 32);
    pad_rows_kernel<<<blocks, 256, 0, st>>>(input, pl->workspace, pl->gather_rows, F, ld);
    NTS_LAUNCH_CHECK();
    in = pl->workspace;
  }
  return run_gather<float>(pl, in, ld, output, F, st);
}

int to_bf16_rows(const void *src, int dtype, uint32_t lds, void *dst, uint32_t n_rows, uint32_t F, uint32_t ld,
                 cudaStream_t st) {
  NTS_ARG_CHECK(dtype == NTS_DTYPE_F32 || dtype == NTS_DTYPE_BF16, "input dtype must be NTS_DTYPE_F32 or NTS_DTYPE_BF16");
  NTS_ARG_CHECK(ld % 8 == 0 && ld >= F && lds >= F && aligned_to(dst, 16), "bad BF16 row layout");
  if (!n_rows || !F)
    return 0;
  const uint64_t total = (uint64_t)n_rows * (ld / 8);
  const unsigned blocks = (unsigned)std::min<uint64_t>((total + 255) / 256, (uint64_t)sm_count() * 32);
  uint4 *d = static_cast<uint4 *>(dst);
  if (dtype == NTS_DTYPE_F32)
    bf16_rows_kernel<float><<<blocks, 256, 0, st>>>(static_cast<const float *>(src), lds, d, n_rows, F, ld);
  else
    bf16_rows_kernel<__nv_bfloat16><<<blocks, 256, 0, st>>>(static_cast<const __nv_bfloat16 *>(src), lds, d, n_rows,
                                                            F, ld);
  NTS_LAUNCH_CHECK();
  return 0;
}

int run_plan_bf16(nts_gather_plan *pl, const void *input, int dtype, uint32_t lds, float *output, uint32_t F,
                  cudaStream_t st) {
  NTS_ARG_CHECK(dtype == NTS_DTYPE_F32 || dtype == NTS_DTYPE_BF16, "input dtype must be NTS_DTYPE_F32 or NTS_DTYPE_BF16");
  NTS_ARG_CHECK(g_plan_variant == 0, "the TMA row-staging variant (nts_gather_plan_set_variant(1)) gathers FP32 rows only");
  if (pl->n_rows == 0 || pl->n_edges == 0 || F == 0)
    return 0;
  NTS_ARG_CHECK(input && output, "null feature pointer");
  NTS_ARG_CHECK(lds >= F, "row stride below the feature width");
  if (dtype == NTS_DTYPE_BF16 && lds % 8 == 0 && aligned_to(input, 16))
    return run_gather<__nv_bfloat16>(pl, static_cast<const __nv_bfloat16 *>(input), lds, output, F, st);
  const uint32_t ld = (F + 7u) & ~7u;
  if (const int rc = ensure_workspace(pl->workspace_bf16, pl->workspace_bf16_elems, (size_t)pl->gather_rows * ld))
    return rc;
  if (const int rc = to_bf16_rows(input, dtype, lds, pl->workspace_bf16, pl->gather_rows, F, ld, st))
    return rc;
  return run_gather<__nv_bfloat16>(pl, pl->workspace_bf16, ld, output, F, st);
}

}

using namespace nts;

extern "C" {

static int pick_slabs_for_rows(nts_vid_t gather_rows, uint64_t n_edges, nts_vid_t n_rows, uint64_t row_bytes,
                               uint64_t l2_budget_bytes) {
  if (!l2_budget_bytes)
    l2_budget_bytes = 16ull << 20;
  const uint64_t bytes = (uint64_t)gather_rows * row_bytes;
  uint64_t s = (bytes + l2_budget_bytes - 1) / l2_budget_bytes;
  const uint64_t by_degree = n_rows ? n_edges / ((uint64_t)n_rows * 16ull) : 1;
  if (s > by_degree)
    s = by_degree;
  if (s > 64)
    s = 64;
  return s < 1 ? 1 : (int)s;
}

int nts_gather_plan_pick_slabs(nts_vid_t gather_rows, uint64_t n_edges, nts_vid_t n_rows, nts_vid_t feature_size,
                               uint64_t l2_budget_bytes) {
  return pick_slabs_for_rows(gather_rows, n_edges, n_rows, ((feature_size + 3ull) & ~3ull) * 4ull, l2_budget_bytes);
}

static bool hub_counts(const nts_vid_t *offsets, const nts_vid_t *indices, const nts_vid_t *slot_of, nts_vid_t base,
                       uint32_t n_rows, uint32_t E, uint32_t gather_rows, std::vector<uint32_t> &col_cnt,
                       std::vector<uint32_t> &seg, cudaStream_t st) {
  uint32_t *cnt = nullptr;
  std::vector<uint32_t> off(n_rows + 1);
  col_cnt.assign(gather_rows, 0);
  const unsigned blocks = (unsigned)std::min<uint64_t>(((uint64_t)E + 255) / 256, (uint64_t)sm_count() * 32);
  bool ok = cudaMalloc(reinterpret_cast<void **>(&cnt), (size_t)gather_rows * 4) == cudaSuccess &&
            cudaMemsetAsync(cnt, 0, (size_t)gather_rows * 4, st) == cudaSuccess;
  if (ok && E) {
    plan_ref_count_kernel<<<blocks, 256, 0, st>>>(indices, slot_of, base, E, cnt);
    count_launch();
  }
  ok = ok && cudaMemcpyAsync(col_cnt.data(), cnt, (size_t)gather_rows * 4, cudaMemcpyDeviceToHost, st) == cudaSuccess &&
       cudaMemcpyAsync(off.data(), offsets, ((size_t)n_rows + 1) * 4, cudaMemcpyDeviceToHost, st) == cudaSuccess &&
       cudaStreamSynchronize(st) == cudaSuccess;
  cudaFree(cnt);
  seg.resize(n_rows);
  for (uint32_t r = 0; r < n_rows; r++)
    seg[r] = off[r + 1] - off[r];
  return ok;
}

static std::vector<uint32_t> top_ids(const std::vector<uint32_t> &cnt, size_t h) {
  std::vector<uint32_t> ids(cnt.size());
  for (size_t i = 0; i < ids.size(); i++)
    ids[i] = (uint32_t)i;
  h = std::min(h, ids.size());
  std::partial_sort(ids.begin(), ids.begin() + h, ids.end(),
                    [&](uint32_t a, uint32_t b) { return cnt[a] != cnt[b] ? cnt[a] > cnt[b] : a < b; });
  ids.resize(h);
  return ids;
}

static bool build_hybrid(nts_gather_plan *pl, const nts_vid_t *offsets, const nts_vid_t *indices, const float *weight,
                         const nts_vid_t *slot_of, nts_vid_t index_base, int n_hub_cols, int n_hub_rows,
                         cudaStream_t st) {
  const uint32_t E = (uint32_t)pl->n_edges, n_rows = pl->n_rows, G = pl->gather_rows;
  std::vector<uint32_t> col_cnt, seg;
  if (!hub_counts(offsets, indices, slot_of, index_base, n_rows, E, G, col_cnt, seg, st))
    return false;
  const std::vector<uint32_t> cols = top_ids(col_cnt, (size_t)n_hub_cols), rows = top_ids(seg, (size_t)n_hub_rows);
  pl->hub_cols = (int)cols.size();
  pl->hub_rows = (int)rows.size();
  pl->lda_c = (n_rows + 3u) & ~3u;
  pl->lda_r = ((uint32_t)pl->hub_rows + 3u) & ~3u;
  const uint64_t dc_cells = (uint64_t)pl->hub_cols * pl->lda_c;
  pl->dense_floats = dc_cells + (pl->hub_rows ? (uint64_t)G * pl->lda_r : 0);
  std::vector<uint32_t> col_slot(G, kNoHub), row_slot(n_rows, kNoHub);
  for (size_t i = 0; i < cols.size(); i++)
    col_slot[cols[i]] = (uint32_t)i;
  for (size_t i = 0; i < rows.size(); i++)
    row_slot[rows[i]] = (uint32_t)i;

  const uint64_t n_keys = (uint64_t)pl->slabs * n_rows;
  int bits = 1;
  while (bits < 64 && (1ull << bits) < n_keys + pl->dense_floats)
    bits++;
  uint64_t *key_in = nullptr, *key_out = nullptr;
  uint32_t *val_in = nullptr, *val_out = nullptr, *d_col_slot = nullptr, *d_row_slot = nullptr, *d_runs = nullptr;
  void *tmp = nullptr;
  size_t tmp_bytes = 0;
  bool ok =
      cudaMalloc(reinterpret_cast<void **>(&pl->pairs), (size_t)E * sizeof(uint2)) == cudaSuccess &&
      cudaMalloc(reinterpret_cast<void **>(&pl->voff), ((size_t)n_keys + 1) * 4) == cudaSuccess &&
      cudaMalloc(reinterpret_cast<void **>(&pl->dense), pl->dense_floats * 4) == cudaSuccess &&
      cudaMalloc(reinterpret_cast<void **>(&pl->hub_col_ids), cols.size() * 4 + 4) == cudaSuccess &&
      cudaMalloc(reinterpret_cast<void **>(&pl->hub_row_ids), rows.size() * 4 + 4) == cudaSuccess &&
      cudaMalloc(reinterpret_cast<void **>(&d_col_slot), (size_t)G * 4 + 4) == cudaSuccess &&
      cudaMalloc(reinterpret_cast<void **>(&d_row_slot), (size_t)n_rows * 4 + 4) == cudaSuccess &&
      cudaMalloc(reinterpret_cast<void **>(&key_in), (size_t)E * 8) == cudaSuccess &&
      cudaMalloc(reinterpret_cast<void **>(&key_out), (size_t)E * 8) == cudaSuccess &&
      cudaMalloc(reinterpret_cast<void **>(&val_in), (size_t)E * 4) == cudaSuccess &&
      cudaMalloc(reinterpret_cast<void **>(&val_out), (size_t)E * 4) == cudaSuccess &&
      cudaMalloc(reinterpret_cast<void **>(&d_runs), 4) == cudaSuccess &&
      cub::DeviceRadixSort::SortPairs(nullptr, tmp_bytes, key_in, key_out, val_in, val_out, (int64_t)E, 0, bits, st) ==
          cudaSuccess &&
      cudaMalloc(&tmp, tmp_bytes ? tmp_bytes : 16) == cudaSuccess &&
      cudaMemcpyAsync(pl->hub_col_ids, cols.data(), cols.size() * 4, cudaMemcpyHostToDevice, st) == cudaSuccess &&
      cudaMemcpyAsync(pl->hub_row_ids, rows.data(), rows.size() * 4, cudaMemcpyHostToDevice, st) == cudaSuccess &&
      cudaMemcpyAsync(d_col_slot, col_slot.data(), (size_t)G * 4, cudaMemcpyHostToDevice, st) == cudaSuccess &&
      cudaMemcpyAsync(d_row_slot, row_slot.data(), (size_t)n_rows * 4, cudaMemcpyHostToDevice, st) == cudaSuccess &&
      cudaMemsetAsync(pl->dense, 0, pl->dense_floats * 4, st) == cudaSuccess;
  const unsigned blocks = (unsigned)std::min<uint64_t>(((uint64_t)E + 255) / 256, (uint64_t)sm_count() * 32);
  if (ok) {
    plan_hybrid_keys_kernel<<<blocks, 256, 0, st>>>(offsets, indices, slot_of, index_base, n_rows, E, pl->slab_rows,
                                                    (uint32_t)pl->slabs, d_col_slot, d_row_slot, pl->lda_c, dc_cells,
                                                    pl->lda_r, key_in, val_in);
    count_launch();
    ok = cub::DeviceRadixSort::SortPairs(tmp, tmp_bytes, key_in, key_out, val_in, val_out, (int64_t)E, 0, bits, st) ==
         cudaSuccess;
  }
  if (ok) {
    const unsigned kb = (unsigned)std::min<uint64_t>((n_keys + 256) / 256, (uint64_t)sm_count() * 32);
    plan_offsets_kernel<uint64_t><<<kb, 256, 0, st>>>(key_out, E, (uint32_t)n_keys, pl->voff);
    count_launch();
    std::vector<uint32_t> h(pl->slabs + 1);
    ok = cudaStreamSynchronize(st) == cudaSuccess;
    for (int s = 0; s <= pl->slabs && ok; s++)
      ok = cudaMemcpy(&h[s], pl->voff + (size_t)s * n_rows, 4, cudaMemcpyDeviceToHost) == cudaSuccess;
    for (int s = 0; s <= pl->slabs; s++)
      pl->slab_edge[s] = h[s];
  }
  const uint32_t n_res = (uint32_t)pl->slab_edge[pl->slabs], n_dense = E - n_res;
  if (ok && n_res) {
    plan_pairs_kernel<<<blocks, 256, 0, st>>>(val_out, indices, weight, slot_of, index_base, n_res, pl->pairs);
    count_launch();
  }
  if (ok && n_dense) {
    uint32_t n_runs = 0;
    size_t b1 = 0, b2 = 0;
    ok = cub::DeviceRunLengthEncode::Encode(nullptr, b1, key_out + n_res, key_in, val_in, d_runs, (int64_t)n_dense,
                                            st) == cudaSuccess &&
         cub::DeviceScan::ExclusiveSum(nullptr, b2, val_in, d_col_slot, (int64_t)n_dense, st) == cudaSuccess;
    if (ok && std::max(b1, b2) > tmp_bytes) {
      cudaFree(tmp);
      tmp_bytes = std::max(b1, b2);
      ok = cudaMalloc(&tmp, tmp_bytes) == cudaSuccess;
    }
    uint32_t *run_start = nullptr;
    ok = ok && cudaMalloc(reinterpret_cast<void **>(&run_start), (size_t)n_dense * 4) == cudaSuccess &&
         cub::DeviceRunLengthEncode::Encode(tmp, b1, key_out + n_res, key_in, val_in, d_runs, (int64_t)n_dense, st) ==
             cudaSuccess &&
         cudaMemcpyAsync(&n_runs, d_runs, 4, cudaMemcpyDeviceToHost, st) == cudaSuccess &&
         cudaStreamSynchronize(st) == cudaSuccess &&
         cub::DeviceScan::ExclusiveSum(tmp, b2, val_in, run_start, (int64_t)n_runs, st) == cudaSuccess;
    if (ok) {
      const unsigned rb = (unsigned)std::min<uint64_t>(((uint64_t)n_runs * 32 + 255) / 256, (uint64_t)sm_count() * 32);
      plan_cell_sum_kernel<<<rb, 256, 0, st>>>(key_in, run_start, val_in, n_runs, val_out + n_res, weight, n_keys,
                                               pl->dense);
      count_launch();
      ok = cudaStreamSynchronize(st) == cudaSuccess;
    }
    cudaFree(run_start);
  }
  cudaFree(key_in), cudaFree(key_out), cudaFree(val_in), cudaFree(val_out), cudaFree(tmp);
  cudaFree(d_col_slot), cudaFree(d_row_slot), cudaFree(d_runs);
  return ok;
}

nts_gather_plan *nts_gather_plan_create(const nts_vid_t *offsets, const nts_vid_t *indices, const float *weight,
                                        const nts_vid_t *slot_of, nts_vid_t index_base, nts_vid_t n_rows,
                                        uint64_t n_edges, nts_vid_t gather_rows, int n_slabs, void *stream) {
  return nts_gather_plan_create_hybrid(offsets, indices, weight, slot_of, index_base, n_rows, n_edges, gather_rows,
                                       n_slabs, 0, 0, stream);
}

nts_gather_plan *nts_gather_plan_create_hybrid(const nts_vid_t *offsets, const nts_vid_t *indices,
                                               const float *weight, const nts_vid_t *slot_of, nts_vid_t index_base,
                                               nts_vid_t n_rows, uint64_t n_edges, nts_vid_t gather_rows, int n_slabs,
                                               int n_hub_cols, int n_hub_rows, void *stream) {
  auto bad = [](const char *m) -> nts_gather_plan * {
    fail(-1, m, __FILE__, __LINE__);
    return nullptr;
  };
  if (n_edges >= 0xffffffffull)
    return bad("chunk edge count must fit uint32 offsets");
  if (n_rows && n_edges && !(offsets && indices))
    return bad("null graph array");
  if (n_hub_cols < 0 || n_hub_rows < 0)
    return bad("negative hub count");
  if (n_slabs < 1)
    n_slabs = 1;
  if (gather_rows == 0)
    n_slabs = 1;
  if ((uint64_t)n_slabs * n_rows >= 0xffffffffull)
    return bad("slabs * rows must fit 32-bit segment keys");
  cudaStream_t st = as_stream(stream);
  nts_gather_plan *pl = new nts_gather_plan();
  pl->n_rows = n_rows;
  pl->n_edges = n_edges;
  pl->gather_rows = gather_rows;
  pl->slabs = n_slabs;
  pl->slab_rows = gather_rows ? (gather_rows + n_slabs - 1) / n_slabs : 1;
  pl->slab_edge.assign(n_slabs + 1, 0);
  if (n_rows == 0 || n_edges == 0)
    return pl;
  const uint32_t E = (uint32_t)n_edges;
  const uint32_t n_keys = (uint32_t)n_slabs * n_rows;
  uint32_t *key_in = nullptr, *key_out = nullptr, *val_in = nullptr, *val_out = nullptr;
  void *tmp = nullptr;
  const bool hubs = gather_rows > 0 && (n_hub_cols > 0 || n_hub_rows > 0);
  bool ok = hubs || (cudaMalloc(reinterpret_cast<void **>(&pl->pairs), (size_t)E * sizeof(uint2)) == cudaSuccess &&
                     cudaMalloc(reinterpret_cast<void **>(&pl->voff), ((size_t)n_keys + 1) * sizeof(uint32_t)) ==
                         cudaSuccess);
  const unsigned blocks = (unsigned)std::min<uint64_t>(((uint64_t)E + 255) / 256, (uint64_t)sm_count() * 32);
  if (hubs) {
    ok = build_hybrid(pl, offsets, indices, weight, slot_of, index_base, n_hub_cols, n_hub_rows, st);
  } else if (ok && n_slabs == 1) {
    plan_pairs_kernel<<<blocks, 256, 0, st>>>(nullptr, indices, weight, slot_of, index_base, E, pl->pairs);
    count_launch();
    ok = cudaMemcpyAsync(pl->voff, offsets, ((size_t)n_rows + 1) * sizeof(uint32_t), cudaMemcpyDeviceToDevice, st) ==
         cudaSuccess;
    pl->slab_edge[0] = 0;
    pl->slab_edge[1] = n_edges;
  } else if (ok) {
    size_t tmp_bytes = 0;
    int bits = 1;
    while (bits < 32 && (1ull << bits) < (uint64_t)n_keys)
      bits++;
    ok = cudaMalloc(reinterpret_cast<void **>(&key_in), (size_t)E * 4) == cudaSuccess &&
         cudaMalloc(reinterpret_cast<void **>(&key_out), (size_t)E * 4) == cudaSuccess &&
         cudaMalloc(reinterpret_cast<void **>(&val_in), (size_t)E * 4) == cudaSuccess &&
         cudaMalloc(reinterpret_cast<void **>(&val_out), (size_t)E * 4) == cudaSuccess &&
         cub::DeviceRadixSort::SortPairs(nullptr, tmp_bytes, key_in, key_out, val_in, val_out, (int64_t)E, 0, bits, st) ==
             cudaSuccess &&
         cudaMalloc(&tmp, tmp_bytes ? tmp_bytes : 16) == cudaSuccess;
    if (ok) {
      plan_keys_kernel<<<blocks, 256, 0, st>>>(offsets, indices, slot_of, index_base, n_rows, E, pl->slab_rows,
                                               (uint32_t)n_slabs, key_in, val_in);
      count_launch();
      ok = cub::DeviceRadixSort::SortPairs(tmp, tmp_bytes, key_in, key_out, val_in, val_out, (int64_t)E, 0, bits, st) ==
           cudaSuccess;
    }
    if (ok) {
      plan_pairs_kernel<<<blocks, 256, 0, st>>>(val_out, indices, weight, slot_of, index_base, E, pl->pairs);
      count_launch();
      const unsigned kb = (unsigned)std::min<uint64_t>(((uint64_t)n_keys + 256) / 256, (uint64_t)sm_count() * 32);
      plan_offsets_kernel<uint32_t><<<kb, 256, 0, st>>>(key_out, E, n_keys, pl->voff);
      count_launch();
      std::vector<uint32_t> h(n_slabs + 1);
      ok = cudaStreamSynchronize(st) == cudaSuccess;
      for (int s = 0; s <= n_slabs && ok; s++)
        ok = cudaMemcpy(&h[s], pl->voff + (size_t)s * n_rows, 4, cudaMemcpyDeviceToHost) == cudaSuccess;
      for (int s = 0; s <= n_slabs; s++)
        pl->slab_edge[s] = h[s];
    }
  }
  if (ok)
    ok = cudaStreamSynchronize(st) == cudaSuccess && cudaGetLastError() == cudaSuccess;
  cudaFree(key_in), cudaFree(key_out), cudaFree(val_in), cudaFree(val_out), cudaFree(tmp);
  if (!ok) {
    nts_gather_plan_destroy(pl);
    fail(-1, "nts_gather_plan_create: device allocation or preprocessing failed", __FILE__, __LINE__);
    return nullptr;
  }
  return pl;
}

static nts_gather_plan *build_plan_parts(const nts_plan_part *parts, int n_parts, nts_vid_t n_rows, nts_vid_t gather_rows,
                                         int n_slabs, cudaStream_t st) {
  auto bad = [](const char *m) -> nts_gather_plan * {
    fail(-1, m, __FILE__, __LINE__);
    return nullptr;
  };
  uint64_t total = 0;
  for (int k = 0; k < n_parts; k++) {
    if (parts[k].n_edges && !(parts[k].offsets && parts[k].indices))
      return bad("null graph array in a plan part");
    if ((uint64_t)parts[k].row_add + parts[k].n_rows > n_rows)
      return bad("plan part rows exceed the output rows");
    total += parts[k].n_edges;
  }
  if (total >= 0xffffffffull)
    return bad("merged edge count must fit uint32 offsets");
  if (n_slabs < 1 || gather_rows == 0)
    n_slabs = 1;
  if ((uint64_t)n_slabs * n_rows >= 0xffffffffull)
    return bad("slabs * rows must fit 32-bit segment keys");
  nts_gather_plan *pl = new nts_gather_plan();
  pl->n_rows = n_rows;
  pl->n_edges = total;
  pl->gather_rows = gather_rows;
  pl->slabs = n_slabs;
  pl->slab_rows = gather_rows ? (gather_rows + n_slabs - 1) / n_slabs : 1;
  pl->slab_edge.assign(n_slabs + 1, 0);
  if (n_rows == 0 || total == 0)
    return pl;
  const uint32_t E = (uint32_t)total, n_keys = (uint32_t)n_slabs * n_rows;
  uint32_t *key_in = nullptr, *key_out = nullptr, *val_in = nullptr, *val_out = nullptr;
  uint2 *unsorted = nullptr;
  void *tmp = nullptr;
  size_t tmp_bytes = 0;
  int bits = 1;
  while (bits < 32 && (1ull << bits) < (uint64_t)n_keys)
    bits++;
  bool ok = cudaMalloc(reinterpret_cast<void **>(&pl->pairs), (size_t)E * sizeof(uint2)) == cudaSuccess &&
            cudaMalloc(reinterpret_cast<void **>(&pl->voff), ((size_t)n_keys + 1) * sizeof(uint32_t)) == cudaSuccess &&
            cudaMalloc(reinterpret_cast<void **>(&unsorted), (size_t)E * sizeof(uint2)) == cudaSuccess &&
            cudaMalloc(reinterpret_cast<void **>(&key_in), (size_t)E * 4) == cudaSuccess &&
            cudaMalloc(reinterpret_cast<void **>(&key_out), (size_t)E * 4) == cudaSuccess &&
            cudaMalloc(reinterpret_cast<void **>(&val_in), (size_t)E * 4) == cudaSuccess &&
            cudaMalloc(reinterpret_cast<void **>(&val_out), (size_t)E * 4) == cudaSuccess &&
            cub::DeviceRadixSort::SortPairs(nullptr, tmp_bytes, key_in, key_out, val_in, val_out, (int64_t)E, 0, bits, st) ==
                cudaSuccess &&
            cudaMalloc(&tmp, tmp_bytes ? tmp_bytes : 16) == cudaSuccess;
  uint32_t e_off = 0;
  for (int k = 0; k < n_parts && ok; k++) {
    const nts_plan_part &pt = parts[k];
    if (!pt.n_edges)
      continue;
    const unsigned blocks = (unsigned)std::min<uint64_t>((pt.n_edges + 255) / 256, (uint64_t)sm_count() * 32);
    plan_part_keys_kernel<<<blocks, 256, 0, st>>>(pt.offsets, pt.indices, pt.slot_of, pt.weight, pt.index_base,
                                                  pt.index_add, pt.n_rows, pt.row_add, (uint32_t)pt.n_edges, e_off, n_rows,
                                                  pl->slab_rows, (uint32_t)n_slabs, key_in, val_in, unsorted);
    count_launch();
    e_off += (uint32_t)pt.n_edges;
  }
  if (ok)
    ok = cub::DeviceRadixSort::SortPairs(tmp, tmp_bytes, key_in, key_out, val_in, val_out, (int64_t)E, 0, bits, st) ==
         cudaSuccess;
  if (ok) {
    const unsigned blocks = (unsigned)std::min<uint64_t>(((uint64_t)E + 255) / 256, (uint64_t)sm_count() * 32);
    plan_permute_pairs_kernel<<<blocks, 256, 0, st>>>(val_out, unsorted, E, pl->pairs);
    count_launch();
    const unsigned kb = (unsigned)std::min<uint64_t>(((uint64_t)n_keys + 256) / 256, (uint64_t)sm_count() * 32);
    plan_offsets_kernel<uint32_t><<<kb, 256, 0, st>>>(key_out, E, n_keys, pl->voff);
    count_launch();
    std::vector<uint32_t> h(n_slabs + 1);
    ok = cudaStreamSynchronize(st) == cudaSuccess;
    for (int s = 0; s <= n_slabs && ok; s++)
      ok = cudaMemcpy(&h[s], pl->voff + (size_t)s * n_rows, 4, cudaMemcpyDeviceToHost) == cudaSuccess;
    for (int s = 0; s <= n_slabs; s++)
      pl->slab_edge[s] = h[s];
  }
  if (ok)
    ok = cudaStreamSynchronize(st) == cudaSuccess && cudaGetLastError() == cudaSuccess;
  cudaFree(key_in), cudaFree(key_out), cudaFree(val_in), cudaFree(val_out), cudaFree(tmp), cudaFree(unsorted);
  if (!ok) {
    fail(-1, "nts_gather_plan_create_parts: device allocation or preprocessing failed", __FILE__, __LINE__);
    cudaFree(pl->pairs), cudaFree(pl->voff);
    delete pl;
    return nullptr;
  }
  return pl;
}

nts_gather_plan *nts_plan_create_parts_typed(const nts_plan_part *parts, int n_parts, nts_vid_t n_rows,
                                             nts_vid_t gather_rows, int n_slabs, nts_vid_t feature_size, int bf16,
                                             void *stream) {
  if (!parts || n_parts < 1) {
    fail(-1, "no plan parts", __FILE__, __LINE__);
    return nullptr;
  }
  cudaStream_t st = as_stream(stream);
  if (n_slabs >= 1)
    return build_plan_parts(parts, n_parts, n_rows, gather_rows, n_slabs, st);
  uint64_t total = 0;
  for (int k = 0; k < n_parts; k++)
    total += parts[k].n_edges;
  const uint64_t row_bytes = bf16 ? ((feature_size + 7ull) & ~7ull) * 2ull : ((feature_size + 3ull) & ~3ull) * 4ull;
  const int s_max = pick_slabs_for_rows(gather_rows, total, n_rows, row_bytes, 16ull << 20);
  nts_gather_plan *best = build_plan_parts(parts, n_parts, n_rows, gather_rows, 1, st);
  if (!best || s_max <= 1 || total == 0 || feature_size == 0)
    return best;
  float *x = nullptr, *y = nullptr;
  cudaEvent_t e0 = nullptr, e1 = nullptr;
  const size_t xb = (size_t)gather_rows * feature_size * (bf16 ? 2 : sizeof(float)),
               yb = (size_t)n_rows * feature_size * sizeof(float);
  bool ok = cudaMalloc(reinterpret_cast<void **>(&x), xb) == cudaSuccess &&
            cudaMalloc(reinterpret_cast<void **>(&y), yb) == cudaSuccess &&
            cudaMemsetAsync(x, 0, xb, st) == cudaSuccess && cudaMemsetAsync(y, 0, yb, st) == cudaSuccess &&
            cudaEventCreate(&e0) == cudaSuccess && cudaEventCreate(&e1) == cudaSuccess;
  auto time_plan = [&](nts_gather_plan *pl, float *ms) -> bool {
    *ms = 1e30f;
    for (int it = 0; it < 3; it++) {
      float t = 0.f;
      if (cudaEventRecord(e0, st) != cudaSuccess ||
          (bf16 ? run_plan_bf16(pl, x, NTS_DTYPE_BF16, feature_size, y, feature_size, st)
                : run_plan(pl, x, y, feature_size, st)) != 0 ||
          cudaEventRecord(e1, st) != cudaSuccess || cudaEventSynchronize(e1) != cudaSuccess ||
          cudaEventElapsedTime(&t, e0, e1) != cudaSuccess)
        return false;
      if (it > 0 && t < *ms)
        *ms = t;
    }
    return true;
  };
  float best_ms = 0.f;
  ok = ok && time_plan(best, &best_ms);
  for (int s = 2; ok; s *= 2) {
    const int cand = s > s_max ? s_max : s;
    nts_gather_plan *pl = build_plan_parts(parts, n_parts, n_rows, gather_rows, cand, st);
    float ms = 0.f;
    if (!pl || !time_plan(pl, &ms)) {
      nts_gather_plan_destroy(pl);
      break;
    }
    if (ms < best_ms) {
      nts_gather_plan_destroy(best);
      best = pl;
      best_ms = ms;
    } else {
      nts_gather_plan_destroy(pl);
      if (ms > 1.1f * best_ms)
        break;
    }
    if (cand == s_max)
      break;
  }
  cudaFree(x), cudaFree(y);
  if (e0)
    cudaEventDestroy(e0);
  if (e1)
    cudaEventDestroy(e1);
  best->tuned_ms = best_ms;
  return best;
}

nts_gather_plan *nts_gather_plan_create_parts(const nts_plan_part *parts, int n_parts, nts_vid_t n_rows,
                                              nts_vid_t gather_rows, int n_slabs, nts_vid_t feature_size, void *stream) {
  return nts_plan_create_parts_typed(parts, n_parts, n_rows, gather_rows, n_slabs, feature_size, 0, stream);
}

float nts_gather_plan_tuned_ms(const nts_gather_plan *pl) { return pl ? pl->tuned_ms : 0.f; }

static constexpr double kHubFloor = 0.05;
static constexpr int kHubMax = 512;

static nts_gather_plan *create_tuned(const nts_vid_t *offsets, const nts_vid_t *indices, const float *weight,
                                     const nts_vid_t *slot_of, nts_vid_t index_base, nts_vid_t n_rows, uint64_t n_edges,
                                     nts_vid_t gather_rows, nts_vid_t feature_size, bool bf16, void *stream) {
  cudaStream_t st = as_stream(stream);
  const uint64_t row_bytes = bf16 ? ((feature_size + 7ull) & ~7ull) * 2ull : ((feature_size + 3ull) & ~3ull) * 4ull;
  const int s_max = pick_slabs_for_rows(gather_rows, n_edges, n_rows, row_bytes, 16ull << 20);
  const char *hub_env = getenv("NTS_PLAN_HUBS");
  const bool try_hubs = !(hub_env && strcmp(hub_env, "0") == 0) && n_rows > 0 && gather_rows > 0;
  nts_gather_plan *best = nts_gather_plan_create(offsets, indices, weight, slot_of, index_base, n_rows, n_edges,
                                                 gather_rows, 1, stream);
  if (!best || (s_max <= 1 && !try_hubs) || n_edges == 0 || feature_size == 0)
    return best;
  float *x = nullptr, *y = nullptr;
  cudaEvent_t e0 = nullptr, e1 = nullptr;
  const size_t xb = (size_t)gather_rows * feature_size * (bf16 ? 2 : sizeof(float)),
               yb = (size_t)n_rows * feature_size * sizeof(float);
  bool ok = cudaMalloc(reinterpret_cast<void **>(&x), xb) == cudaSuccess &&
            cudaMalloc(reinterpret_cast<void **>(&y), yb) == cudaSuccess &&
            cudaMemsetAsync(x, 0, xb, st) == cudaSuccess && cudaMemsetAsync(y, 0, yb, st) == cudaSuccess &&
            cudaEventCreate(&e0) == cudaSuccess && cudaEventCreate(&e1) == cudaSuccess;
  auto run_one = [&](nts_gather_plan *pl) {
    return bf16 ? run_plan_bf16(pl, x, NTS_DTYPE_BF16, feature_size, y, feature_size, st)
                : run_plan(pl, x, y, feature_size, st);
  };
  auto time_plan = [&](nts_gather_plan *pl, float *ms) -> bool {
    *ms = 1e30f;
    for (int it = 0; it < 3; it++) {
      float t = 0.f;
      if (cudaEventRecord(e0, st) != cudaSuccess || run_one(pl) != 0 ||
          cudaEventRecord(e1, st) != cudaSuccess || cudaEventSynchronize(e1) != cudaSuccess ||
          cudaEventElapsedTime(&t, e0, e1) != cudaSuccess)
        return false;
      if (it > 0 && t < *ms)
        *ms = t;
    }
    return true;
  };
  float best_ms = 0.f;
  ok = ok && time_plan(best, &best_ms);
  auto consider = [&](int s, int hc, int hr, float *ms, int overlap = 0) -> int {
    nts_gather_plan *pl = nts_gather_plan_create_hybrid(offsets, indices, weight, slot_of, index_base, n_rows, n_edges,
                                                        gather_rows, s, hc, hr, stream);
    if (pl)
      pl->overlap = overlap;
    if (!pl || !time_plan(pl, ms)) {
      nts_gather_plan_destroy(pl);
      return -1;
    }
    if (*ms < best_ms) {
      nts_gather_plan_destroy(best);
      best = pl;
      best_ms = *ms;
      return 1;
    }
    nts_gather_plan_destroy(pl);
    return 0;
  };
  for (int s = 2; ok && s_max > 1; s *= 2) {
    const int cand = s > s_max ? s_max : s;
    float ms = 0.f;
    const int r = consider(cand, 0, 0, &ms);
    if (r < 0 || (r == 0 && ms > 1.1f * best_ms))
      break;
    if (cand == s_max)
      break;
  }
  if (ok && try_hubs) {
    std::vector<uint32_t> col_cnt, seg;
    ok = hub_counts(offsets, indices, slot_of, index_base, n_rows, (uint32_t)n_edges, gather_rows, col_cnt, seg, st);
    int n_c = 0, n_r = 0;
    for (uint32_t c : col_cnt)
      n_c += c > kHubFloor * n_rows;
    for (uint32_t s : seg)
      n_r += s > kHubFloor * gather_rows;
    const int plain_slabs = best->slabs;
    float ms = 0.f;
    for (int c = 32; ok && c <= std::min(n_c, kHubMax); c *= 2)
      if (consider(best->slabs, c, 0, &ms) != 1)
        break;
    for (int r = 32; ok && r <= std::min(n_r, kHubMax); r *= 2)
      if (consider(best->slabs, best->hub_cols, r, &ms) != 1)
        break;
    if (best->hub_cols || best->hub_rows) {
      const int hc = best->hub_cols, hr = best->hub_rows;
      for (int s : {plain_slabs / 2, std::min(plain_slabs * 2, s_max)})
        if (s >= 1 && s != plain_slabs && s != best->slabs)
          consider(s, hc, hr, &ms);
    }
    const char *ov_env = getenv("NTS_PLAN_OVERLAP");
    if (ok && best->hub_rows && !(ov_env && strcmp(ov_env, "0") == 0)) {
      best->overlap = 1;
      float fused_ms = 0.f;
      if (time_plan(best, &fused_ms) && fused_ms < best_ms) {
        best_ms = fused_ms;
        for (int r = 2 * best->hub_rows; r <= std::min(n_r, kHubMax); r *= 2)
          if (consider(best->slabs, best->hub_cols, r, &ms, 1) != 1)
            break;
      } else {
        best->overlap = 0;
      }
    }
  }
  cudaFree(x), cudaFree(y);
  if (e0)
    cudaEventDestroy(e0);
  if (e1)
    cudaEventDestroy(e1);
  best->tuned_ms = best_ms;
  return best;
}

nts_gather_plan *nts_gather_plan_create_tuned(const nts_vid_t *offsets, const nts_vid_t *indices, const float *weight,
                                              const nts_vid_t *slot_of, nts_vid_t index_base, nts_vid_t n_rows,
                                              uint64_t n_edges, nts_vid_t gather_rows, nts_vid_t feature_size,
                                              void *stream) {
  return create_tuned(offsets, indices, weight, slot_of, index_base, n_rows, n_edges, gather_rows, feature_size, false,
                      stream);
}

nts_gather_plan *nts_gather_plan_create_tuned_bf16(const nts_vid_t *offsets, const nts_vid_t *indices,
                                                   const float *weight, const nts_vid_t *slot_of, nts_vid_t index_base,
                                                   nts_vid_t n_rows, uint64_t n_edges, nts_vid_t gather_rows,
                                                   nts_vid_t feature_size, void *stream) {
  return create_tuned(offsets, indices, weight, slot_of, index_base, n_rows, n_edges, gather_rows, feature_size, true,
                      stream);
}

int nts_gather_plan_destroy(nts_gather_plan *pl) {
  if (!pl)
    return 0;
  cudaFree(pl->pairs);
  cudaFree(pl->voff);
  cudaFree(pl->workspace);
  cudaFree(pl->workspace_bf16);
  cudaFree(pl->dense);
  cudaFree(pl->hub_col_ids);
  cudaFree(pl->hub_row_ids);
  delete pl;
  return 0;
}

int nts_gather_plan_slabs(const nts_gather_plan *pl) { return pl ? pl->slabs : 0; }

int nts_gather_plan_hubs(const nts_gather_plan *pl, int *cols, int *rows) {
  NTS_ARG_CHECK(pl != nullptr, "null plan");
  if (cols)
    *cols = pl->hub_cols;
  if (rows)
    *rows = pl->hub_rows;
  return 0;
}

int nts_gather_plan_overlap(const nts_gather_plan *pl) { return pl ? pl->overlap : 0; }

int nts_gather_plan_set_overlap(nts_gather_plan *pl, int overlap) {
  NTS_ARG_CHECK(pl != nullptr, "null plan");
  NTS_ARG_CHECK(overlap == 0 || overlap == 1, "overlap must be 0 (sequential) or 1 (fused slab launches)");
  pl->overlap = overlap;
  return 0;
}

uint64_t nts_gather_plan_bytes(const nts_gather_plan *pl) {
  if (!pl)
    return 0;
  return pl->n_edges * 8ull + ((uint64_t)pl->slabs * pl->n_rows + 1) * 4ull + pl->workspace_floats * 4ull +
         pl->workspace_bf16_elems * 2ull + pl->dense_floats * 4ull + ((uint64_t)pl->hub_cols + pl->hub_rows) * 4ull;
}

int nts_gather_plan_last_launch(const nts_gather_plan *pl, int *launches, int *grid, int *k, int *u, int *outv) {
  NTS_ARG_CHECK(pl != nullptr, "null plan");
  if (launches)
    *launches = pl->last_launches;
  if (grid)
    *grid = pl->last_grid;
  if (k)
    *k = pl->last_k;
  if (u)
    *u = pl->last_u;
  if (outv)
    *outv = pl->last_outv;
  return 0;
}

int nts_gather_plan_run(nts_gather_plan *pl, const float *input, float *output, nts_vid_t feature_size, void *stream) {
  NTS_ARG_CHECK(pl != nullptr, "null plan");
  return run_plan(pl, input, output, feature_size, as_stream(stream));
}

int nts_gather_plan_run_bf16(nts_gather_plan *pl, const void *input, int input_dtype, float *output,
                             nts_vid_t feature_size, void *stream) {
  NTS_ARG_CHECK(pl != nullptr, "null plan");
  return run_plan_bf16(pl, input, input_dtype, feature_size, output, feature_size, as_stream(stream));
}

int nts_rows_to_bf16(const void *src, int src_dtype, nts_vid_t lds, void *dst, nts_vid_t n_rows, nts_vid_t feature_size,
                     nts_vid_t ld, void *stream) {
  NTS_ARG_CHECK((src && dst) || n_rows == 0 || feature_size == 0, "null pointer passed to nts_rows_to_bf16");
  return to_bf16_rows(src, src_dtype, lds, dst, n_rows, feature_size, ld, as_stream(stream));
}

int nts_gather_plan_set_variant(int variant) {
  NTS_ARG_CHECK(variant == 0 || variant == 1, "variant must be 0 (register staging) or 1 (TMA row staging)");
  g_plan_variant = variant;
  return 0;
}

int nts_gather_plan_set_tuning(int u, int min_blocks, int edges_per_warp) {
  NTS_ARG_CHECK(u >= 0 && min_blocks >= 0 && edges_per_warp >= 0 && edges_per_warp <= 4096, "bad tuning point");
  g_plan_u = u;
  g_plan_minb = min_blocks;
  g_plan_q = edges_per_warp;
  return 0;
}

}
```

### neutronstarlite_b200/ops.py

```python
from __future__ import annotations

import ctypes as C
import time as _time

import torch

from . import _lib


def _stream():
    return torch.cuda.current_stream().cuda_stream


def _check_input(t, name="input"):
    if not t.is_cuda:
        raise _lib.NtsError("%s must be a CUDA tensor (libnts_b200 has no CPU fallback)" % name)
    if t.dtype != torch.float32 or t.dim() != 2:
        raise _lib.NtsError("%s must be a 2-D float32 tensor" % name)
    if not t.is_contiguous():
        raise _lib.NtsError("%s must be contiguous" % name)
    return t


def _check_gather_dtype(gather_dtype):
    if gather_dtype is not None and gather_dtype != torch.bfloat16:
        raise _lib.NtsError("gather_dtype must be None or torch.bfloat16, not %s" % (gather_dtype,))
    return gather_dtype


def _check_gathered(t, name, gather_dtype):
    if gather_dtype is None or (t.is_cuda and t.dtype == torch.float32):
        return _check_input(t, name)
    if not t.is_cuda:
        raise _lib.NtsError("%s must be a CUDA tensor (libnts_b200 has no CPU fallback)" % name)
    if t.dtype != torch.bfloat16 or t.dim() != 2:
        raise _lib.NtsError("%s must be a 2-D float32 or bfloat16 tensor" % name)
    if not t.is_contiguous():
        raise _lib.NtsError("%s must be contiguous" % name)
    return t


_DTYPE_CODE = {torch.float32: 0, torch.bfloat16: 1}


def _ptr(t):
    return 0 if t is None else t.data_ptr()


class KernelTimer:

    def __init__(self):
        self.records = []

    def bracket(self, tag, F, edges, rows):
        start = torch.cuda.Event(enable_timing=True)
        stop = torch.cuda.Event(enable_timing=True)
        self.records.append((tag, int(F), int(edges), int(rows), start, stop))
        return start, stop

    def summary(self):
        torch.cuda.synchronize()
        out = {}
        for tag, F, edges, rows, a, b in self.records:
            d = out.setdefault((tag, F), {"calls": 0, "ms": 0.0, "edges": 0, "rows": 0})
            d["calls"] += 1
            d["ms"] += a.elapsed_time(b)
            d["edges"] += edges
            d["rows"] += rows
        return out


_timer = None


def set_kernel_timer(timer):
    global _timer
    _timer = timer


class _timed:

    def __init__(self, tag, F, edges, rows):
        self.ev = _timer.bracket(tag, F, edges, rows) if _timer else None

    def __enter__(self):
        if self.ev:
            self.ev[0].record()

    def __exit__(self, *exc):
        if self.ev:
            self.ev[1].record()
        return False


def segment_gather_sum(out, x, weight, indices, offsets, index_base, n_rows, n_edges):
    _lib.call("nts_segment_gather_sum", _ptr(x), _ptr(out), _ptr(weight), _ptr(indices), _ptr(offsets),
              int(index_base), int(n_rows), int(n_edges), int(x.shape[1]), _stream())
    return out


class GatherPlan:

    def __init__(self, offsets, indices, weight, index_base, n_rows, n_edges, gather_rows, slabs, slot_of=None,
                 tune_for=0, hubs=(0, 0), gather_dtype=None):
        L = _lib.load()
        _check_gather_dtype(gather_dtype)
        t0 = _time.perf_counter()
        if slabs > 0:
            self.handle = L.nts_gather_plan_create_hybrid(_ptr(offsets), _ptr(indices), _ptr(weight), _ptr(slot_of),
                                                          int(index_base), int(n_rows), int(n_edges),
                                                          int(gather_rows), int(slabs), int(hubs[0]), int(hubs[1]),
                                                          _stream())
        else:
            create = L.nts_gather_plan_create_tuned_bf16 if gather_dtype is not None else L.nts_gather_plan_create_tuned
            self.handle = create(_ptr(offsets), _ptr(indices), _ptr(weight), _ptr(slot_of), int(index_base),
                                 int(n_rows), int(n_edges), int(gather_rows), int(tune_for), _stream())
        self.build_s = _time.perf_counter() - t0
        if not self.handle:
            raise _lib.NtsError("nts_gather_plan_create failed: " + L.nts_last_error().decode(errors="replace"))
        self.slabs = int(L.nts_gather_plan_slabs(self.handle))
        hc, hr = C.c_int(0), C.c_int(0)
        _lib.call("nts_gather_plan_hubs", self.handle, C.byref(hc), C.byref(hr))
        self.hub_cols, self.hub_rows = hc.value, hr.value
        self.n_rows, self.n_edges = int(n_rows), int(n_edges)

    @property
    def overlap(self):
        return bool(_lib.load().nts_gather_plan_overlap(self.handle))

    def set_overlap(self, overlap):
        _lib.call("nts_gather_plan_set_overlap", self.handle, int(bool(overlap)))

    def key(self):
        return ((self.slabs,) + ((self.hub_cols, self.hub_rows) if self.hub_cols or self.hub_rows else ())
                + (("overlap",) if self.overlap else ()))

    def run(self, x, out, gather_dtype=None):
        if _check_gather_dtype(gather_dtype) is not None:
            if x.dtype not in _DTYPE_CODE:
                raise _lib.NtsError("BF16 gathers take a float32 or bfloat16 input, not %s" % x.dtype)
            _lib.call("nts_gather_plan_run_bf16", self.handle, _ptr(x), _DTYPE_CODE[x.dtype], _ptr(out),
                      int(x.shape[1]), _stream())
            return out
        if x.dtype == torch.bfloat16:
            raise _lib.NtsError("a bfloat16 input needs gather_dtype=torch.bfloat16")
        _lib.call("nts_gather_plan_run", self.handle, _ptr(x), _ptr(out), int(x.shape[1]), _stream())
        return out

    def bytes(self):
        return int(_lib.load().nts_gather_plan_bytes(self.handle))

    def __del__(self):
        try:
            if getattr(self, "handle", None):
                _lib.load().nts_gather_plan_destroy(self.handle)
                self.handle = None
        except Exception:
            pass


import os as _os

PLAN_MIN_EDGES = 1 << 20
_plan_mode = {"0": "off", "1": "on"}.get(_os.environ.get("NTS_PLAN", ""), "auto")
_plan_slabs = int(_os.environ.get("NTS_PLAN_SLABS", "0"))


def set_plan_mode(mode, slabs=0):
    global _plan_mode, _plan_slabs
    if mode not in ("auto", "on", "off"):
        raise ValueError("plan mode must be auto, on or off")
    _plan_mode, _plan_slabs = mode, int(slabs)


def _chunk_plan(chunk, direction, F, gather_dtype=None):
    if gather_dtype is None and (_plan_mode == "off" or (_plan_mode == "auto" and chunk.edge_size < PLAN_MIN_EDGES)):
        return None
    if direction == "fwd":
        n_rows, gather_rows = chunk.batch_size_forward, chunk.batch_size_backward
    else:
        n_rows, gather_rows = chunk.batch_size_backward, chunk.batch_size_forward
    plans = chunk.__dict__.setdefault("_gather_plans", {})
    tuned = chunk.__dict__.setdefault("_gather_plan_for", {})
    key = (direction, _plan_slabs) if _plan_slabs else (direction, "F", int(F))
    if gather_dtype is not None and not _plan_slabs:
        key += ("bf16",)
    plan = plans.get(key) if _plan_slabs else tuned.get(key)
    if plan is None:
        if direction == "fwd":
            plan = GatherPlan(chunk.column_offset_gpu, chunk.row_indices_gpu, chunk.edge_weight_forward_gpu,
                              chunk.src_range[0], n_rows, chunk.edge_size, gather_rows, _plan_slabs, tune_for=int(F),
                              gather_dtype=gather_dtype)
        else:
            plan = GatherPlan(chunk.row_offset_gpu, chunk.column_indices_gpu, chunk.edge_weight_backward_gpu,
                              chunk.dst_range[0], n_rows, chunk.edge_size, gather_rows, _plan_slabs, tune_for=int(F),
                              gather_dtype=gather_dtype)
        share = (direction,) + plan.key()
        if share in plans:
            plan = plans[share]
        plans[share] = plan
        if not _plan_slabs:
            tuned[key] = plan
    return plan


def _bf16_plan(chunk, direction, F, with_weight, gather_dtype):
    if _check_gather_dtype(gather_dtype) is None:
        return _chunk_plan(chunk, direction, F) if with_weight else None
    if not with_weight:
        raise _lib.NtsError("BF16 gathers always apply the edge weights (with_weight=True)")
    return _chunk_plan(chunk, direction, F, gather_dtype)


def gather_by_dst_from_src(chunk, out, x, with_weight=True, gather_dtype=None):
    plan = _bf16_plan(chunk, "fwd", x.shape[1], with_weight, gather_dtype)
    ev = _timer.bracket("fwd", x.shape[1], chunk.edge_size, chunk.batch_size_forward) if _timer else None
    if ev:
        ev[0].record()
    if plan is not None:
        plan.run(x, out, gather_dtype)
    else:
        _lib.call("nts_gather_by_dst_from_src", _ptr(x), _ptr(out), _ptr(chunk.edge_weight_forward_gpu),
                  _ptr(chunk.row_indices_gpu), _ptr(chunk.column_offset_gpu), chunk.src_range[0], chunk.src_range[1],
                  chunk.dst_range[0], chunk.dst_range[1], chunk.edge_size, chunk.batch_size_forward,
                  int(x.shape[1]), 1 if with_weight else 0, _stream())
    if ev:
        ev[1].record()
    return out


def gather_by_src_from_dst(chunk, out, grad, with_weight=True, gather_dtype=None):
    plan = _bf16_plan(chunk, "bwd", grad.shape[1], with_weight, gather_dtype)
    ev = _timer.bracket("bwd", grad.shape[1], chunk.edge_size, chunk.batch_size_backward) if _timer else None
    if ev:
        ev[0].record()
    if plan is not None:
        plan.run(grad, out, gather_dtype)
    else:
        _lib.call("nts_gather_by_src_from_dst", _ptr(grad), _ptr(out), _ptr(chunk.edge_weight_backward_gpu),
                  _ptr(chunk.row_offset_gpu), _ptr(chunk.column_indices_gpu), chunk.src_range[0], chunk.src_range[1],
                  chunk.dst_range[0], chunk.dst_range[1], chunk.edge_size, chunk.batch_size_backward,
                  int(grad.shape[1]), 1 if with_weight else 0, _stream())
    if ev:
        ev[1].record()
    return out


class ntsGraphOp:

    def __init__(self, partitioned_graph, active=None):
        self.partitioned_graph_ = partitioned_graph
        self.active_ = active

    def forward(self, f_input, f_input1=None):
        raise NotImplementedError

    def backward(self, output_grad):
        raise NotImplementedError

    def get_additional_grad(self):
        raise NotImplementedError("get_additional_grad is not implemented")


class ForwardSingleGPUfuseOp(ntsGraphOp):

    def __init__(self, partitioned_graph, active=None, gather_dtype=None):
        super().__init__(partitioned_graph, active)
        self.gather_dtype = _check_gather_dtype(gather_dtype)

    def forward(self, f_input, f_input1=None):
        x = _check_gathered(f_input, "input", self.gather_dtype)
        c = self.partitioned_graph_.graph_chunks[0]
        y = torch.zeros((c.batch_size_forward, x.shape[1]), dtype=torch.float32, device=x.device)
        return gather_by_dst_from_src(c, y, x, gather_dtype=self.gather_dtype)

    def backward(self, f_output_grad):
        g = _check_input(f_output_grad, "output_grad")
        c = self.partitioned_graph_.graph_chunks[0]
        dx = torch.zeros((c.batch_size_backward, g.shape[1]), dtype=torch.float32, device=g.device)
        return gather_by_src_from_dst(c, dx, g, gather_dtype=self.gather_dtype)


class ForwardGPUfuseOp(ntsGraphOp):

    def __init__(self, partitioned_graph, active=None, exchange=None, gather_dtype=None):
        super().__init__(partitioned_graph, active)
        self.gather_dtype = _check_gather_dtype(gather_dtype)
        if exchange is None:
            from .exchange import default_exchange
            exchange = default_exchange(partitioned_graph)
        self.exchange = exchange

    def forward(self, f_input, f_input1=None):
        x = _check_gathered(f_input, "input", self.gather_dtype)
        if self.gather_dtype is None:
            return self.exchange.forward(x)
        return self.exchange.forward(x, gather_dtype=self.gather_dtype)

    def backward(self, f_output_grad):
        g = _check_input(f_output_grad, "output_grad")
        if self.gather_dtype is None:
            return self.exchange.backward(g)
        return self.exchange.backward(g, gather_dtype=self.gather_dtype)


class _EdgeOp(ntsGraphOp):
    def _topo(self):
        pg = self.partitioned_graph_
        if pg.column_offset_gpu is None or pg.row_indices_gpu is None:
            raise _lib.NtsError("whole-partition CSC missing: call PartitionedGraph.generate_all(dist=True, device=...)")
        return pg


class DistGPUGetDepNbrOp(ntsGraphOp):

    def __init__(self, partitioned_graph, active=None, exchange=None):
        super().__init__(partitioned_graph, active)
        if exchange is None:
            from .exchange import default_exchange
            exchange = default_exchange(partitioned_graph)
        self.exchange = exchange

    def forward(self, f_input, f_input1=None):
        return self.exchange.fetch_mirrors(_check_input(f_input))

    def backward(self, f_output_grad):
        return self.exchange.return_mirror_grads(_check_input(f_output_grad, "output_grad"))


class DistGPUScatterSrc(_EdgeOp):

    def forward(self, f_input, f_input1=None):
        pg = self._topo()
        x = _check_input(f_input)
        msg = torch.zeros((pg.owned_edges, x.shape[1]), dtype=torch.float32, device=x.device)
        _lib.call("nts_scatter_src_mirror_to_msg", _ptr(msg), _ptr(x), _ptr(pg.row_indices_gpu),
                  _ptr(pg.column_offset_gpu), _ptr(pg.mirror_index_gpu), pg.owned_vertices, x.shape[1], _stream())
        return msg

    def backward(self, f_output_grad):
        pg = self._topo()
        g = _check_input(f_output_grad, "output_grad")
        out = torch.zeros((pg.owned_mirrors, g.shape[1]), dtype=torch.float32, device=g.device)
        _lib.call("nts_gather_msg_to_src_mirror", _ptr(out), _ptr(g), _ptr(pg.row_indices_gpu),
                  _ptr(pg.column_offset_gpu), _ptr(pg.mirror_index_gpu), pg.owned_vertices, g.shape[1], _stream())
        return out


class DistGPUScatterDst(_EdgeOp):

    def forward(self, f_input, f_input1=None):
        pg = self._topo()
        x = _check_input(f_input)
        msg = torch.zeros((pg.owned_edges, x.shape[1]), dtype=torch.float32, device=x.device)
        _lib.call("nts_scatter_dst_to_msg", _ptr(msg), _ptr(x), _ptr(pg.row_indices_gpu),
                  _ptr(pg.column_offset_gpu), pg.owned_vertices, x.shape[1], _stream())
        return msg

    def backward(self, f_output_grad):
        pg = self._topo()
        g = _check_input(f_output_grad, "output_grad")
        out = torch.zeros((pg.owned_vertices, g.shape[1]), dtype=torch.float32, device=g.device)
        _lib.call("nts_gather_msg_to_dst", _ptr(out), _ptr(g), _ptr(pg.row_indices_gpu),
                  _ptr(pg.column_offset_gpu), pg.owned_vertices, g.shape[1], _stream())
        return out


class DistGPUAggregateDst(_EdgeOp):

    def forward(self, f_input, f_input1=None):
        pg = self._topo()
        m = _check_input(f_input)
        out = torch.zeros((pg.owned_vertices, m.shape[1]), dtype=torch.float32, device=m.device)
        _lib.call("nts_gather_msg_to_dst", _ptr(out), _ptr(m), _ptr(pg.row_indices_gpu),
                  _ptr(pg.column_offset_gpu), pg.owned_vertices, m.shape[1], _stream())
        return out

    def backward(self, f_output_grad):
        pg = self._topo()
        g = _check_input(f_output_grad, "output_grad")
        msg = torch.zeros((pg.owned_edges, g.shape[1]), dtype=torch.float32, device=g.device)
        _lib.call("nts_scatter_dst_to_msg", _ptr(msg), _ptr(g), _ptr(pg.row_indices_gpu),
                  _ptr(pg.column_offset_gpu), pg.owned_vertices, g.shape[1], _stream())
        return msg


class DistGPUEdgeSoftMax(_EdgeOp):

    def __init__(self, partitioned_graph, active=None):
        super().__init__(partitioned_graph, active)
        self.IntermediateResult = None

    def forward(self, f_input, f_input1=None):
        pg = self._topo()
        m = _check_input(f_input)
        out = torch.zeros_like(m)
        self.IntermediateResult = torch.zeros_like(m)
        _lib.call("nts_edge_softmax_forward", _ptr(out), _ptr(m), _ptr(self.IntermediateResult),
                  _ptr(pg.row_indices_gpu), _ptr(pg.column_offset_gpu), pg.owned_vertices, m.shape[1], _stream())
        return out

    def backward(self, f_output_grad):
        pg = self._topo()
        g = _check_input(f_output_grad, "output_grad")
        out = torch.zeros_like(g)
        _lib.call("nts_edge_softmax_backward", _ptr(out), _ptr(g), _ptr(self.IntermediateResult),
                  _ptr(pg.row_indices_gpu), _ptr(pg.column_offset_gpu), pg.owned_vertices, g.shape[1], _stream())
        return out


class DistGPUAggregateDstFuseWeight(_EdgeOp):

    def __init__(self, partitioned_graph, active=None):
        super().__init__(partitioned_graph, active)
        self._mirror = None
        self._a = None
        self.e_weight_grad = None

    def forward(self, f_input, e_weight=None):
        pg = self._topo()
        x = _check_input(f_input)
        a = _check_input(e_weight, "edge weight")
        self._mirror, self._a = x, a
        heads = int(a.shape[1])
        out = torch.zeros((pg.owned_vertices, x.shape[1]), dtype=torch.float32, device=x.device)
        _lib.call("nts_segment_gather_sum_heads", _ptr(x), _ptr(out), _ptr(a), _ptr(pg.row_indices_gpu),
                  _ptr(pg.column_offset_gpu), _ptr(pg.mirror_index_gpu), 0, pg.owned_vertices, pg.owned_edges,
                  x.shape[1], heads, _stream())
        return out

    def backward(self, f_output_grad):
        pg = self._topo()
        g = _check_input(f_output_grad, "output_grad")
        dm = torch.zeros((pg.owned_mirrors, g.shape[1]), dtype=torch.float32, device=g.device)
        self.e_weight_grad = torch.zeros_like(self._a)
        _lib.call("nts_aggregate_dst_fuse_weight_backward_heads", _ptr(dm), _ptr(self.e_weight_grad),
                  _ptr(self._mirror), _ptr(self._a), _ptr(g), _ptr(pg.row_indices_gpu), _ptr(pg.column_offset_gpu),
                  _ptr(pg.mirror_index_gpu), pg.owned_vertices, g.shape[1], int(self._a.shape[1]), _stream())
        return dm

    def get_additional_grad(self):
        return self.e_weight_grad


class DistGPUFusedGATOp(_EdgeOp):

    def __init__(self, partitioned_graph, active=None, negative_slope=0.2, two_pass_backward=True, gather_dtype=None):
        super().__init__(partitioned_graph, active)
        self.slope = float(negative_slope)
        self.two_pass_backward = bool(two_pass_backward)
        self.gather_dtype = _check_gather_dtype(gather_dtype)
        if self.gather_dtype is not None and not self.two_pass_backward:
            raise _lib.NtsError("BF16 gathers of the fused GAT layer need two_pass_backward=True")
        self._saved = None

    @staticmethod
    def slot_indices(pg):
        cached = getattr(pg, "_slot_indices_gpu", None)
        if cached is None:
            cached = pg.mirror_index_gpu[pg.row_indices_gpu.long()].to(torch.int32).contiguous()
            pg._slot_indices_gpu = cached
        return cached

    @staticmethod
    def slot_csr(pg):
        cached = getattr(pg, "_slot_csr_gpu", None)
        if cached is not None:
            return cached
        col = pg.column_offset_gpu.long()
        V, M = pg.owned_vertices, pg.owned_mirrors
        slot = DistGPUFusedGATOp.slot_indices(pg).long()
        dst = torch.repeat_interleave(torch.arange(V, device=col.device), col[1:V + 1] - col[:V])
        order = torch.sort(slot, stable=True).indices
        csr_dst = dst[order].to(torch.int32).contiguous()
        off = torch.zeros(M + 1, dtype=torch.int64, device=col.device)
        off[1:] = torch.cumsum(torch.bincount(slot, minlength=M), 0)
        pg._slot_csr_gpu = (off.to(torch.int32).contiguous(), csr_dst)
        return pg._slot_csr_gpu

    def forward(self, mirror, src_score, dst_score):
        pg = self._topo()
        x = _check_input(mirror, "mirror")
        s = _check_input(src_score, "src_score")
        d = _check_input(dst_score, "dst_score")
        H = int(s.shape[1])
        seg_max = torch.empty((pg.owned_vertices, H), dtype=torch.float32, device=x.device)
        seg_sum = torch.empty_like(seg_max)
        slots = self.slot_indices(pg)
        with _timed("gat_stats", x.shape[1], pg.owned_edges, pg.owned_vertices):
            _lib.call("nts_gat_softmax_stats", _ptr(seg_max), _ptr(seg_sum), _ptr(s), _ptr(d), _ptr(slots),
                      _ptr(pg.column_offset_gpu), 0, pg.owned_vertices, H, self.slope, _stream())
        F = int(x.shape[1])
        if self.gather_dtype is not None:
            return self._forward_bf16(pg, x, s, d, seg_max, seg_sum, slots, H, F)
        xk, Fk = x, F
        if H == 1 and F % 4 != 0:
            Fk = (F + 3) // 4 * 4
            xk = torch.nn.functional.pad(x, (0, Fk - F))
        out = torch.zeros((pg.owned_vertices, Fk), dtype=torch.float32, device=x.device)
        with _timed("gat_fwd", F, pg.owned_edges, pg.owned_vertices):
            _lib.call("nts_gat_fused_aggregate_forward", _ptr(xk), _ptr(out), _ptr(s), _ptr(d), _ptr(seg_max),
                      _ptr(seg_sum), _ptr(slots), _ptr(pg.column_offset_gpu), 0,
                      pg.owned_vertices, pg.owned_edges, Fk, H, self.slope, _stream())
        if Fk != F:
            out = out[:, :F].contiguous()
        self._saved = (x, s, d, seg_max, seg_sum, out)
        return out

    @staticmethod
    def _to_bf16_rows(t, ld):
        n, F = t.shape
        r = torch.empty((n, ld), dtype=torch.bfloat16, device=t.device)
        with _timed("gat_bf16_round", F, 0, n):
            _lib.call("nts_rows_to_bf16", _ptr(t), _DTYPE_CODE[torch.float32], F, _ptr(r), n, F, ld, _stream())
        return r

    def _forward_bf16(self, pg, x, s, d, seg_max, seg_sum, slots, H, F):
        ld = (F + 7) // 8 * 8
        mt = self._to_bf16_rows(x, ld)
        out = torch.zeros((pg.owned_vertices, ld), dtype=torch.float32, device=x.device)
        with _timed("gat_fwd", F, pg.owned_edges, pg.owned_vertices):
            _lib.call("nts_gat_fused_aggregate_forward_bf16", _ptr(mt), _ptr(out), _ptr(s), _ptr(d), _ptr(seg_max),
                      _ptr(seg_sum), _ptr(slots), _ptr(pg.column_offset_gpu), 0, pg.owned_vertices, pg.owned_edges,
                      F, ld, H, self.slope, _stream())
        if ld != F:
            out = out[:, :F].contiguous()
        self._saved = (mt, s, d, seg_max, seg_sum, out)
        return out

    def _backward_bf16(self, pg, g):
        mt, s, d, seg_max, seg_sum, out = self._saved
        H = int(s.shape[1])
        M, ld = mt.shape
        F = int(out.shape[1])
        gt = self._to_bf16_rows(g, ld)
        out_dot_g = (out.detach() * gt[:, :F].float()).view(-1, H, F // H).sum(-1).contiguous()
        dm = torch.zeros((M, ld), dtype=torch.float32, device=g.device)
        ds = torch.zeros_like(s)
        dd = torch.zeros_like(d)
        slot_off, slot_dst = self.slot_csr(pg)
        pack = torch.empty((pg.owned_vertices, H, 4), dtype=torch.float32, device=g.device)
        with _timed("gat_bwd", F, 2 * pg.owned_edges, pg.owned_vertices):
            _lib.call("nts_gat_fused_aggregate_backward_two_pass_bf16", _ptr(dm), _ptr(ds), _ptr(dd), _ptr(pack),
                      _ptr(mt), _ptr(s), _ptr(d), _ptr(seg_max), _ptr(seg_sum), _ptr(out_dot_g), _ptr(gt),
                      _ptr(self.slot_indices(pg)), _ptr(pg.column_offset_gpu), 0, _ptr(slot_off), _ptr(slot_dst),
                      pg.owned_vertices, M, F, ld, H, self.slope, _stream())
        if ld != F:
            dm = dm[:, :F].contiguous()
        return dm, ds, dd

    def backward(self, f_output_grad):
        pg = self._topo()
        g = _check_input(f_output_grad, "output_grad")
        if self.gather_dtype is not None:
            return self._backward_bf16(pg, g)
        x, s, d, seg_max, seg_sum, out = self._saved
        H = int(s.shape[1])
        D = x.shape[1] // H
        out_dot_g = (out.detach() * g).view(-1, H, D).sum(-1).contiguous()
        dm = torch.zeros_like(x)
        ds = torch.zeros_like(s)
        dd = torch.zeros_like(d)
        if self.two_pass_backward:
            slot_off, slot_dst = self.slot_csr(pg)
            pack = torch.empty((pg.owned_vertices, H, 4), dtype=torch.float32, device=x.device)
            with _timed("gat_bwd", x.shape[1], 2 * pg.owned_edges, pg.owned_vertices):
                _lib.call("nts_gat_fused_aggregate_backward_two_pass", _ptr(dm), _ptr(ds), _ptr(dd), _ptr(pack),
                          _ptr(x), _ptr(s), _ptr(d), _ptr(seg_max), _ptr(seg_sum), _ptr(out_dot_g), _ptr(g),
                          _ptr(self.slot_indices(pg)), _ptr(pg.column_offset_gpu), 0,
                          _ptr(slot_off), _ptr(slot_dst), pg.owned_vertices, x.shape[0], x.shape[1], H, self.slope,
                          _stream())
            return dm, ds, dd
        _lib.call("nts_gat_fused_aggregate_backward", _ptr(dm), _ptr(ds), _ptr(dd), _ptr(x), _ptr(s), _ptr(d),
                  _ptr(seg_max), _ptr(seg_sum), _ptr(out_dot_g), _ptr(g), _ptr(pg.row_indices_gpu),
                  _ptr(pg.column_offset_gpu), _ptr(pg.mirror_index_gpu), pg.owned_vertices, x.shape[1], H,
                  self.slope, _stream())
        return dm, ds, dd
```

### neutronstarlite_b200/toolkits.py

```python
from __future__ import annotations

import math

import numpy as np
import torch
import torch.distributed as dist

from .context import NtsContext
from . import _lib, ops


class Parameter:
    def __init__(self, w, h, alpha, beta1, beta2, epsilon, weight_decay, device=None, generator=None):
        scale = math.sqrt(6.0 / (w + h))
        W = (2 * scale) * torch.rand((w, h), dtype=torch.float32, generator=generator) - scale
        self.W = W.to(device).requires_grad_(True)
        self.M = torch.zeros((w, h), dtype=torch.float32, device=device)
        self.V = torch.zeros((w, h), dtype=torch.float32, device=device)
        self.W_gradient = None
        f32 = np.float32
        self.alpha = f32(alpha)
        self.beta1, self.beta2, self.epsilon = f32(beta1), f32(beta2), f32(epsilon)
        self.alpha_t, self.beta1_t, self.beta2_t = f32(alpha), f32(beta1), f32(beta2)
        self.weight_decay = f32(weight_decay)
        self.curr_epoch = 0
        self.decay_rate, self.decay_epoch = 1, -1

    def init_parameter(self):
        if dist.is_initialized() and dist.get_world_size() > 1:
            dist.broadcast(self.W.data, src=0)

    def set_decay(self, decay_rate, decay_epoch):
        self.decay_rate, self.decay_epoch = int(decay_rate), int(decay_epoch)

    def all_reduce_to_gradient(self, grad):
        self.W_gradient = grad.detach().clone().contiguous()
        if dist.is_initialized() and dist.get_world_size() > 1:
            dist.all_reduce(self.W_gradient, op=dist.ReduceOp.SUM)

    def next(self):
        if self.decay_epoch != -1 and self.curr_epoch != 0 and self.curr_epoch % self.decay_epoch == 0:
            self.alpha_t *= self.decay_rate
        one = np.float32(1)
        self.alpha_t = np.float32(self.alpha_t)
        self.alpha = np.float32(self.alpha_t * np.sqrt(one - self.beta2) / (one - self.beta1))
        self.beta1 = np.float32(self.beta1 * self.beta1_t)
        self.beta2 = np.float32(self.beta2 * self.beta2_t)
        self.curr_epoch += 1

    def forward(self, x):
        return x.mm(self.W)

    def learn_with_decay_Adam(self):
        with torch.no_grad():
            if self.W.is_cuda:
                from . import _lib
                _lib.call("nts_adam_update", self.W.data_ptr(), self.M.data_ptr(), self.V.data_ptr(),
                          self.W_gradient.data_ptr(), self.W.numel(), float(self.weight_decay), float(self.beta1),
                          float(self.beta2), float(self.alpha), float(self.epsilon),
                          torch.cuda.current_stream().cuda_stream)
                return
            one = np.float32(1)
            W_g = self.W * float(self.weight_decay) + self.W_gradient
            self.M = float(self.beta1) * self.M + float(one - self.beta1) * W_g
            self.V = float(self.beta2) * self.V + float(one - self.beta2) * W_g * W_g
            self.W -= float(self.alpha) * self.M / (torch.sqrt(self.V) + float(self.epsilon))

    def zero_grad(self):
        self.W.grad = None


class GCNImpl:

    _input_is_gathered = True

    def __init__(self, partitioned_graph, layers, features, labels, mask, learn_rate=0.01, weight_decay=0.0001,
                 decay_rate=0.97, decay_epoch=100, drop_rate=0.5, op_class=None, op_kwargs=None, seed=0,
                 gather_dtype=None):
        self.pg = partitioned_graph
        self.layers = list(layers)
        self.device = features.device
        self.drop_rate = drop_rate
        self.ctx = NtsContext()
        gen = torch.Generator().manual_seed(seed)
        self.P = []
        for i in range(len(self.layers) - 1):
            p = Parameter(self.layers[i], self.layers[i + 1], learn_rate, 0.9, 0.999, 1e-9, weight_decay,
                          device=self.device, generator=gen)
            p.init_parameter()
            p.set_decay(decay_rate, decay_epoch)
            self.P.append(p)
        self.L_GT = labels.to(self.device)
        self.MASK = mask.to(self.device)
        self.train_rows = (self.MASK == 0).nonzero().view(-1)
        self.X = [None] * len(self.layers)
        self.gather_dtype = ops._check_gather_dtype(gather_dtype)
        if self.gather_dtype is not None and self._input_is_gathered:
            features = features.detach().to(self.gather_dtype)
        self.X[0] = features.requires_grad_(True)
        if op_class is None:
            op_class = ops.ForwardSingleGPUfuseOp if partitioned_graph.partitions == 1 else ops.ForwardGPUfuseOp
        self.op_class = op_class
        self.op_kwargs = dict(op_kwargs or {})
        if self.gather_dtype is not None:
            self.op_kwargs["gather_dtype"] = self.gather_dtype
        self.loss = None
        self.epoch = 0

    def vertexForward(self, a, x, layer):
        if layer < len(self.layers) - 2:
            return torch.relu(self.P[layer].forward(a))
        return self.P[layer].forward(a).log_softmax(1)

    def Forward(self):
        for i in range(len(self.layers) - 1):
            x_i = self.X[i]
            if i != 0 and self.drop_rate > 0:
                dropped = torch.nn.functional.dropout(x_i, self.drop_rate, training=True)
                self.ctx.appendNNOp(x_i, dropped)
                x_i = dropped
            x_i = x_i.contiguous()
            y_i = self.ctx.runGraphOp(self.op_class, self.pg, None, x_i, **self.op_kwargs)
            self.X[i + 1] = self.ctx.runVertexForward(lambda n, v, _l=i: self.vertexForward(n, v, _l), y_i, x_i)

    def Loss(self):
        a = self.X[-1]
        self.loss = torch.nn.functional.nll_loss(a.index_select(0, self.train_rows),
                                                 self.L_GT.index_select(0, self.train_rows))
        self.ctx.appendNNOp(a, self.loss)

    def Update(self):
        for p in self.P:
            p.all_reduce_to_gradient(p.W.grad)
            p.learn_with_decay_Adam()
            p.next()

    def Test(self, s):
        sel = self.MASK == s
        correct = (self.X[-1].argmax(1) == self.L_GT)[sel].sum()
        total = sel.sum()
        pair = torch.stack([correct, total]).to(torch.int64)
        if dist.is_initialized() and dist.get_world_size() > 1:
            dist.all_reduce(pair)
        return pair

    def run_epoch(self, test=False):
        if self.epoch != 0:
            for p in self.P:
                p.zero_grad()
        self.Forward()
        acc = [self.Test(s) for s in (0, 1, 2)] if test else None
        self.Loss()
        self.ctx.self_backward(True)
        self.Update()
        self.epoch += 1
        return self.loss, acc


class GCNEagerImpl(GCNImpl):

    _input_is_gathered = False

    def __init__(self, *args, **kwargs):
        super().__init__(*args, **kwargs)
        self.X[0] = self.X[0].detach()

    def vertexForward(self, a, x, layer):
        if layer == 0:
            return self.P[layer].forward(a)
        if self.drop_rate > 0:
            a = torch.nn.functional.dropout(a, self.drop_rate, training=True)
        return self.P[layer].forward(torch.relu(a))

    def Forward(self):
        for i in range(len(self.layers) - 1):
            y_i = self.ctx.runVertexForward(lambda n, v, _l=i: self.vertexForward(n, v, _l), self.X[i], self.X[i])
            self.X[i + 1] = self.ctx.runGraphOp(self.op_class, self.pg, None, y_i.contiguous(), **self.op_kwargs)

    def Loss(self):
        a = self.X[-1].log_softmax(1)
        self.loss = torch.nn.functional.nll_loss(a.index_select(0, self.train_rows),
                                                 self.L_GT.index_select(0, self.train_rows))
        self.ctx.appendNNOp(self.X[-1], self.loss)


class GATImpl:

    def __init__(self, partitioned_graph, layers, features, labels, mask, heads=8, learn_rate=0.01,
                 weight_decay=0.0001, exchange=None, seed=0, sum_fanout_grads=True, fused_kernel=False,
                 two_pass_backward=True, gather_dtype=None):
        self.pg = partitioned_graph
        self.fused_kernel = fused_kernel
        self.two_pass_backward = two_pass_backward
        self.gather_dtype = ops._check_gather_dtype(gather_dtype)
        if self.gather_dtype is not None and not (fused_kernel and two_pass_backward):
            raise _lib.NtsError("GATImpl gather_dtype needs fused_kernel=True and two_pass_backward=True")
        self.layers = list(layers)
        self.device = features.device
        self.heads = [heads] * (len(self.layers) - 2) + [1]
        self.ctx = NtsContext(sum_fanout_grads=sum_fanout_grads)
        gen = torch.Generator().manual_seed(seed)
        self.P, self.al, self.ar = [], [], []
        for i in range(len(self.layers) - 1):
            H = self.heads[i]
            D = self.layers[i + 1] // H
            assert H * D == self.layers[i + 1], "layer width must be a multiple of heads"
            mk = lambda a, b: Parameter(a, b, learn_rate, 0.9, 0.999, 1e-9, weight_decay, device=self.device,
                                        generator=gen)
            for lst, shape in ((self.P, (self.layers[i], H * D)), (self.al, (H, D)), (self.ar, (H, D))):
                prm = mk(*shape)
                prm.init_parameter()
                lst.append(prm)
        if exchange is None:
            from .exchange import GpuExchange
            exchange = GpuExchange(partitioned_graph)
        self.exchange = exchange
        self.L_GT = labels.to(self.device)
        self.MASK = mask.to(self.device)
        self.train_rows = (self.MASK == 0).nonzero().view(-1)
        self.X = [None] * len(self.layers)
        self.X[0] = features.requires_grad_(True)
        self.loss = None
        self.epoch = 0

    def params(self):
        return self.P + self.al + self.ar

    def Forward(self):
        ctx, pg = self.ctx, self.pg
        for i in range(len(self.layers) - 1):
            H = self.heads[i]
            D = self.layers[i + 1] // H
            last = i == len(self.layers) - 2
            X_trans = ctx.runVertexForward(lambda x, _i=i: self.P[_i].forward(x), self.X[i])
            mirror = ctx.runGraphOp(ops.DistGPUGetDepNbrOp, pg, None, X_trans.contiguous(), exchange=self.exchange)
            src_att = ctx.runVertexForward(
                lambda m, _i=i: (m.view(-1, H, D) * self.al[_i].W).sum(-1).contiguous(), mirror)
            dst_att = ctx.runVertexForward(
                lambda x, _i=i: (x.view(-1, H, D) * self.ar[_i].W).sum(-1).contiguous(), X_trans)
            if self.fused_kernel:
                nbr = ctx.runGraphOpN(ops.DistGPUFusedGATOp, pg, None, [mirror, src_att, dst_att],
                                      two_pass_backward=self.two_pass_backward, gather_dtype=self.gather_dtype)
            else:
                e_src = ctx.runGraphOp(ops.DistGPUScatterSrc, pg, None, src_att)
                e_dst = ctx.runGraphOp(ops.DistGPUScatterDst, pg, None, dst_att)
                e_msg = e_src + e_dst
                m = ctx.runEdgeForward(lambda t: torch.nn.functional.leaky_relu(t, 0.2), e_msg)
                a = ctx.runGraphOp(ops.DistGPUEdgeSoftMax, pg, None, m)
                nbr = ctx.runGraphOp(ops.DistGPUAggregateDstFuseWeight, pg, None, mirror, a)
            if last:
                self.X[i + 1] = ctx.runVertexForward(lambda t: t.log_softmax(1), nbr)
            else:
                self.X[i + 1] = ctx.runVertexForward(lambda t: torch.relu(t), nbr)

    def Loss(self):
        a = self.X[-1]
        self.loss = torch.nn.functional.nll_loss(a.index_select(0, self.train_rows),
                                                 self.L_GT.index_select(0, self.train_rows))
        self.ctx.appendNNOp(a, self.loss)

    def Update(self):
        for p in self.params():
            if p.W.grad is None:
                continue
            p.all_reduce_to_gradient(p.W.grad)
            p.learn_with_decay_Adam()
            p.next()

    def run_epoch(self):
        if self.epoch != 0:
            for p in self.params():
                p.zero_grad()
        self.Forward()
        self.Loss()
        self.ctx.self_backward(True)
        self.Update()
        self.epoch += 1
        return self.loss
```

Measured before the change: 15.31 billion.

## Add overwrite-mode and strided-input gather plan runs to skip zero-fill and padding copies

Adds run flags to the gather plan so the output can be overwritten instead of accumulated. The hub column GEMM stores directly, and a memset is used only when there are no hub columns. This removes the torch.zeros pre-fill of output buffers in the single-GPU op. The plan also accepts a row-pitched input (lds), and the model pre-pads the input features to a multiple of 4 columns so the per-call pad_rows copy and .contiguous() copy are avoided. The cost is a more complex API and correctness that depends on hub column tiles covering every output element when overwriting.

```diff
diff --git a/include/nts_b200.h b/include/nts_b200.h
--- a/include/nts_b200.h
+++ b/include/nts_b200.h
@@ -90,14 +90,24 @@
 uint64_t nts_gather_plan_bytes(const nts_gather_plan *plan);
 int nts_gather_plan_run(nts_gather_plan *plan, const float *input, float *output, nts_vid_t feature_size,
                         void *stream);
+enum { NTS_PLAN_ACCUMULATE = 0, NTS_PLAN_OVERWRITE = 1, NTS_PLAN_COPY_INPUT = 2 };
+int nts_gather_plan_run_ex(nts_gather_plan *plan, const float *input, nts_vid_t input_ld, float *output,
+                           nts_vid_t feature_size, int flags, void *stream);
 int nts_gather_plan_last_launch(const nts_gather_plan *plan, int *launches, int *grid, int *k, int *u, int *outv);
 enum { NTS_DTYPE_F32 = 0, NTS_DTYPE_BF16 = 1 };
 int nts_gather_plan_run_bf16(nts_gather_plan *plan, const void *input, int input_dtype, float *output,
                              nts_vid_t feature_size, void *stream);
+int nts_gather_plan_run_bf16_ex(nts_gather_plan *plan, const void *input, int input_dtype, nts_vid_t input_ld,
+                                float *output, nts_vid_t feature_size, int flags, void *stream);
 nts_gather_plan *nts_gather_plan_create_tuned_bf16(const nts_vid_t *offsets, const nts_vid_t *indices,
                                                    const float *weight, const nts_vid_t *slot_of, nts_vid_t index_base,
                                                    nts_vid_t n_rows, uint64_t n_edges, nts_vid_t gather_rows,
                                                    nts_vid_t feature_size, void *stream);
+nts_gather_plan *nts_gather_plan_create_tuned_ex(const nts_vid_t *offsets, const nts_vid_t *indices,
+                                                 const float *weight, const nts_vid_t *slot_of, nts_vid_t index_base,
+                                                 nts_vid_t n_rows, uint64_t n_edges, nts_vid_t gather_rows,
+                                                 nts_vid_t feature_size, int gather_dtype, int run_flags,
+                                                 void *stream);
 int nts_gather_plan_set_tuning(int u, int min_blocks, int edges_per_warp);
 int nts_gather_plan_set_variant(int variant);
 
diff --git a/neutronstarlite_b200/_lib.py b/neutronstarlite_b200/_lib.py
--- a/neutronstarlite_b200/_lib.py
+++ b/neutronstarlite_b200/_lib.py
@@ -58,7 +58,10 @@
     "nts_gather_plan_bytes": (_u64, [_vp]),
     "nts_gather_plan_run": (_int, [_vp, _vp, _vp, _u32, _vp]),
     "nts_gather_plan_run_bf16": (_int, [_vp, _vp, _int, _vp, _u32, _vp]),
+    "nts_gather_plan_run_ex": (_int, [_vp, _vp, _u32, _vp, _u32, _int, _vp]),
+    "nts_gather_plan_run_bf16_ex": (_int, [_vp, _vp, _int, _u32, _vp, _u32, _int, _vp]),
     "nts_gather_plan_create_tuned_bf16": (_vp, [_vp, _vp, _vp, _vp, _u32, _u32, _u64, _u32, _u32, _vp]),
+    "nts_gather_plan_create_tuned_ex": (_vp, [_vp, _vp, _vp, _vp, _u32, _u32, _u64, _u32, _u32, _int, _int, _vp]),
     "nts_gather_plan_last_launch": (_int, [_vp] + [C.POINTER(_int)] * 5),
     "nts_gather_plan_set_tuning": (_int, [_int, _int, _int]),
     "nts_gather_plan_set_variant": (_int, [_int]),
diff --git a/neutronstarlite_b200/csrc/nts_common.cuh b/neutronstarlite_b200/csrc/nts_common.cuh
--- a/neutronstarlite_b200/csrc/nts_common.cuh
+++ b/neutronstarlite_b200/csrc/nts_common.cuh
@@ -49,7 +49,7 @@
 int sm_count();
 
 int run_plan_bf16(nts_gather_plan *pl, const void *input, int dtype, uint32_t lds, float *output, uint32_t F,
-                  cudaStream_t st);
+                  cudaStream_t st, int flags = 0);
 int to_bf16_rows(const void *src, int dtype, uint32_t lds, void *dst, uint32_t n_rows, uint32_t F, uint32_t ld,
                  cudaStream_t st);
 
diff --git a/neutronstarlite_b200/csrc/nts_plan.cu b/neutronstarlite_b200/csrc/nts_plan.cu
--- a/neutronstarlite_b200/csrc/nts_plan.cu
+++ b/neutronstarlite_b200/csrc/nts_plan.cu
@@ -172,13 +172,13 @@
   }
 }
 
-__global__ void pad_rows_kernel(const float *__restrict__ src, float *__restrict__ dst, uint32_t n_rows, uint32_t F,
-                                uint32_t ld) {
+__global__ void pad_rows_kernel(const float *__restrict__ src, uint32_t lds, float *__restrict__ dst, uint32_t n_rows,
+                                uint32_t F, uint32_t ld) {
   const uint64_t total = (uint64_t)n_rows * ld;
   for (uint64_t i = (uint64_t)blockIdx.x * blockDim.x + threadIdx.x; i < total; i += (uint64_t)gridDim.x * blockDim.x) {
     const uint64_t r = i / ld;
     const uint32_t c = (uint32_t)(i - r * ld);
-    dst[i] = c < F ? __ldg(src + r * F + c) : 0.f;
+    dst[i] = c < F ? __ldg(src + r * lds + c) : 0.f;
   }
 }
 
@@ -273,6 +273,24 @@
         else
           orow[col + i] += v[i];
       }
+  }
+}
+
+template <int OUTV>
+__device__ __forceinline__ void store_chunk(float *__restrict__ orow, uint32_t col, uint32_t F, float4 a) {
+  if constexpr (OUTV == 4) {
+    *reinterpret_cast<float4 *>(orow + col) = a;
+  } else if constexpr (OUTV == 2) {
+    float2 *p = reinterpret_cast<float2 *>(orow + col);
+    p[0] = make_float2(a.x, a.y);
+    if (col + 2 < F)
+      p[1] = make_float2(a.z, a.w);
+  } else {
+    const float v[4] = {a.x, a.y, a.z, a.w};
+#pragma unroll
+    for (int i = 0; i < 4; i++)
+      if (col + i < F)
+        orow[col + i] = v[i];
   }
 }
 
@@ -694,12 +712,13 @@
   TB Bs[2][kHubBK][kBN];
 };
 
-template <class TB, int OUTV, bool SPLIT, int TN, int KKU>
+template <class TB, int OUTV, bool SPLIT, bool STORE, int TN, int KKU>
 __device__ __forceinline__ void hub_gemm_tile(HubSmem<TN, TB> &sm, uint32_t tile, const float *__restrict__ At,
                                               uint32_t lda, uint32_t M, uint32_t k_lo, uint32_t k_hi, uint32_t k_split,
                                               const TB *__restrict__ B, uint32_t ldb,
                                               const uint32_t *__restrict__ colmap, float *__restrict__ out, uint32_t F,
                                               const uint32_t *__restrict__ rowmap, uint32_t m_tiles, uint32_t n_tiles) {
+  static_assert(!(SPLIT && STORE), "split-K partials must be added, not stored");
   constexpr bool kBf16 = std::is_same<TB, __nv_bfloat16>::value;
   constexpr uint32_t kBV = 16 / sizeof(TB);
   constexpr uint32_t kBN = HubSmem<TN, TB>::kBN;
@@ -793,22 +812,26 @@
 #pragma unroll
     for (int j = 0; j < TN / 4; j++) {
       const uint32_t col = n0 + j * 64 + tx * 4;
-      if (col < F)
-        flush_chunk<OUTV, SPLIT>(orow, col, F,
-                                 make_float4(acc[i][j * 4], acc[i][j * 4 + 1], acc[i][j * 4 + 2], acc[i][j * 4 + 3]));
-    }
-  }
-}
-
-template <class TB, int OUTV, bool SPLIT>
+      const float4 a = make_float4(acc[i][j * 4], acc[i][j * 4 + 1], acc[i][j * 4 + 2], acc[i][j * 4 + 3]);
+      if (col < F) {
+        if constexpr (STORE)
+          store_chunk<OUTV>(orow, col, F, a);
+        else
+          flush_chunk<OUTV, SPLIT>(orow, col, F, a);
+      }
+    }
+  }
+}
+
+template <class TB, int OUTV, bool SPLIT, bool STORE>
 __global__ void __launch_bounds__(kHubThreads, 2)
     hub_block_gemm_kernel(const float *__restrict__ At, uint32_t lda, uint32_t M, uint32_t K, uint32_t k_split,
                           const TB *__restrict__ B, uint32_t ldb, const uint32_t *__restrict__ colmap,
                           float *__restrict__ out, uint32_t F, const uint32_t *__restrict__ rowmap, uint32_t m_tiles,
                           uint32_t n_tiles) {
   __shared__ __align__(16) HubSmem<8, TB> sm;
-  hub_gemm_tile<TB, OUTV, SPLIT, 8, kHubBK>(sm, blockIdx.x, At, lda, M, 0, K, k_split, B, ldb, colmap, out, F, rowmap, m_tiles,
-                                    n_tiles);
+  hub_gemm_tile<TB, OUTV, SPLIT, STORE, 8, kHubBK>(sm, blockIdx.x, At, lda, M, 0, K, k_split, B, ldb, colmap, out, F,
+                                                   rowmap, m_tiles, n_tiles);
 }
 
 static uint32_t hub_row_k_split(uint32_t K, uint32_t m_tiles, uint32_t n_tiles) {
@@ -820,15 +843,16 @@
 
 template <class TB, int OUTV>
 static int launch_hub_blocks(nts_gather_plan *pl, const TB *in, uint32_t ldb, float *out, uint32_t F, bool rows,
-                             cudaStream_t st) {
+                             bool overwrite, cudaStream_t st) {
   const uint32_t n_tiles = (F + kHubBN - 1) / kHubBN;
   if (pl->hub_cols) {
     const uint32_t m_tiles = (pl->n_rows + kHubBM - 1) / kHubBM;
     const uint64_t blocks = (uint64_t)m_tiles * n_tiles;
     NTS_ARG_CHECK(blocks <= 0x7fffffffull, "hub column block grid too large");
-    hub_block_gemm_kernel<TB, OUTV, false><<<(unsigned)blocks, kHubThreads, 0, st>>>(
-        pl->dense, pl->lda_c, pl->n_rows, (uint32_t)pl->hub_cols, (uint32_t)pl->hub_cols, in, ldb, pl->hub_col_ids, out,
-        F, nullptr, m_tiles, n_tiles);
+    auto kern = overwrite ? hub_block_gemm_kernel<TB, OUTV, false, true> : hub_block_gemm_kernel<TB, OUTV, false, false>;
+    kern<<<(unsigned)blocks, kHubThreads, 0, st>>>(pl->dense, pl->lda_c, pl->n_rows, (uint32_t)pl->hub_cols,
+                                                   (uint32_t)pl->hub_cols, in, ldb, pl->hub_col_ids, out, F, nullptr,
+                                                   m_tiles, n_tiles);
     NTS_LAUNCH_CHECK();
   }
   if (pl->hub_rows && rows) {
@@ -836,7 +860,7 @@
     const uint32_t K = pl->gather_rows;
     const uint32_t k_split = hub_row_k_split(K, m_tiles, n_tiles);
     const uint64_t splits = (K + k_split - 1) / k_split;
-    hub_block_gemm_kernel<TB, OUTV, true><<<(unsigned)(splits * m_tiles * n_tiles), kHubThreads, 0, st>>>(
+    hub_block_gemm_kernel<TB, OUTV, true, false><<<(unsigned)(splits * m_tiles * n_tiles), kHubThreads, 0, st>>>(
         pl->dense + (size_t)pl->hub_cols * pl->lda_c, pl->lda_r, (uint32_t)pl->hub_rows, K, k_split, in, ldb, nullptr,
         out, F, pl->hub_row_ids, m_tiles, n_tiles);
     NTS_LAUNCH_CHECK();
@@ -864,7 +888,7 @@
   extern __shared__ __align__(16) unsigned char smem_raw[];
   const uint32_t b = blockIdx.x, grp = b / hub.period;
   if (grp < hub.n_gemm && b - grp * hub.period == hub.period - 1)
-    hub_gemm_tile<T, OUTV, true, TN, TN == 8 ? kHubBK : 4>(
+    hub_gemm_tile<T, OUTV, true, false, TN, TN == 8 ? kHubBK : 4>(
         *reinterpret_cast<HubSmem<TN, T> *>(smem_raw), grp, hub.At, hub.lda, hub.M, hub.k_lo, hub.k_hi, hub.k_split,
         reinterpret_cast<const T *>(in), ldc * GatherT<T>::V, nullptr, out, F, hub.rowmap, hub.m_tiles, hub.n_tiles);
   else
@@ -923,7 +947,8 @@
   }
 
 template <class T>
-static int run_gather(nts_gather_plan *pl, const T *in, uint32_t ld, float *output, uint32_t F, cudaStream_t st) {
+static int run_gather(nts_gather_plan *pl, const T *in, uint32_t ld, float *output, uint32_t F, bool overwrite,
+                      cudaStream_t st) {
   constexpr bool kBf16 = std::is_same<T, __nv_bfloat16>::value;
   PlanShape sh;
   const uint32_t ldc = ld / GatherT<T>::V;
@@ -936,10 +961,12 @@
   sh.outv = (F % 4 == 0 && aligned_to(output, 16)) ? 4 : ((F % 2 == 0 && aligned_to(output, 8)) ? 2 : 1);
   const bool fused = pl->overlap && pl->hub_rows;
   NTS_ARG_CHECK(!fused || g_plan_variant == 0, "the fused slab launches use the register-staging gather (variant 0)");
+  if (overwrite && !pl->hub_cols)
+    NTS_CUDA_OK(cudaMemsetAsync(output, 0, (size_t)pl->n_rows * F * sizeof(float), st));
   if (pl->hub_cols || pl->hub_rows) {
-    const int rc = sh.outv == 4   ? launch_hub_blocks<T, 4>(pl, in, ld, output, F, !fused, st)
-                   : sh.outv == 2 ? launch_hub_blocks<T, 2>(pl, in, ld, output, F, !fused, st)
-                                  : launch_hub_blocks<T, 1>(pl, in, ld, output, F, !fused, st);
+    const int rc = sh.outv == 4   ? launch_hub_blocks<T, 4>(pl, in, ld, output, F, !fused, overwrite, st)
+                   : sh.outv == 2 ? launch_hub_blocks<T, 2>(pl, in, ld, output, F, !fused, overwrite, st)
+                                  : launch_hub_blocks<T, 1>(pl, in, ld, output, F, !fused, overwrite, st);
     if (rc)
       return rc;
   }
@@ -1072,22 +1099,42 @@
   return 0;
 }
 
-static int run_plan(nts_gather_plan *pl, const float *input, float *output, uint32_t F, cudaStream_t st) {
-  if (pl->n_rows == 0 || pl->n_edges == 0 || F == 0)
+static int run_prologue(nts_gather_plan *pl, const void *input, uint32_t lds, float *output, uint32_t F, int flags,
+                        bool *done, cudaStream_t st) {
+  *done = true;
+  NTS_ARG_CHECK((flags & ~(NTS_PLAN_OVERWRITE | NTS_PLAN_COPY_INPUT)) == 0, "unknown plan run flags");
+  if (pl->n_rows == 0 || F == 0)
     return 0;
+  if (pl->n_edges == 0) {
+    if (flags & NTS_PLAN_OVERWRITE) {
+      NTS_ARG_CHECK(output != nullptr, "null output pointer");
+      NTS_CUDA_OK(cudaMemsetAsync(output, 0, (size_t)pl->n_rows * F * sizeof(float), st));
+    }
+    return 0;
+  }
   NTS_ARG_CHECK(input && output, "null feature pointer");
+  NTS_ARG_CHECK(lds >= F, "row stride below the feature width");
+  *done = false;
+  return 0;
+}
+
+static int run_plan(nts_gather_plan *pl, const float *input, uint32_t lds, float *output, uint32_t F, int flags,
+                    cudaStream_t st) {
+  bool done = false;
+  if (const int rc = run_prologue(pl, input, lds, output, F, flags, &done, st))
+    return rc;
+  if (done)
+    return 0;
+  if (lds % 4 == 0 && aligned_to(input, 16) && !(flags & NTS_PLAN_COPY_INPUT))
+    return run_gather<float>(pl, input, lds, output, F, flags & NTS_PLAN_OVERWRITE, st);
   const uint32_t ld = (F + 3u) & ~3u;
-  const float *in = input;
-  if (ld != F || !aligned_to(input, 16)) {
-    if (const int rc = ensure_workspace(pl->workspace, pl->workspace_floats, (size_t)pl->gather_rows * ld))
-      return rc;
-    const uint64_t total = (uint64_t)pl->gather_rows * ld;
-    const unsigned blocks = (unsigned)std::min<uint64_t>((total + 255) / 256, (uint64_t)sm_count() * 32);
-    pad_rows_kernel<<<blocks, 256, 0, st>>>(input, pl->workspace, pl->gather_rows, F, ld);
-    NTS_LAUNCH_CHECK();
-    in = pl->workspace;
-  }
-  return run_gather<float>(pl, in, ld, output, F, st);
+  if (const int rc = ensure_workspace(pl->workspace, pl->workspace_floats, (size_t)pl->gather_rows * ld))
+    return rc;
+  const uint64_t total = (uint64_t)pl->gather_rows * ld;
+  const unsigned blocks = (unsigned)std::min<uint64_t>((total + 255) / 256, (uint64_t)sm_count() * 32);
+  pad_rows_kernel<<<blocks, 256, 0, st>>>(input, lds, pl->workspace, pl->gather_rows, F, ld);
+  NTS_LAUNCH_CHECK();
+  return run_gather<float>(pl, pl->workspace, ld, output, F, flags & NTS_PLAN_OVERWRITE, st);
 }
 
 int to_bf16_rows(const void *src, int dtype, uint32_t lds, void *dst, uint32_t n_rows, uint32_t F, uint32_t ld,
@@ -1109,21 +1156,23 @@
 }
 
 int run_plan_bf16(nts_gather_plan *pl, const void *input, int dtype, uint32_t lds, float *output, uint32_t F,
-                  cudaStream_t st) {
+                  cudaStream_t st, int flags) {
   NTS_ARG_CHECK(dtype == NTS_DTYPE_F32 || dtype == NTS_DTYPE_BF16, "input dtype must be NTS_DTYPE_F32 or NTS_DTYPE_BF16");
   NTS_ARG_CHECK(g_plan_variant == 0, "the TMA row-staging variant (nts_gather_plan_set_variant(1)) gathers FP32 rows only");
-  if (pl->n_rows == 0 || pl->n_edges == 0 || F == 0)
+  bool done = false;
+  if (const int rc = run_prologue(pl, input, lds, output, F, flags, &done, st))
+    return rc;
+  if (done)
     return 0;
-  NTS_ARG_CHECK(input && output, "null feature pointer");
-  NTS_ARG_CHECK(lds >= F, "row stride below the feature width");
-  if (dtype == NTS_DTYPE_BF16 && lds % 8 == 0 && aligned_to(input, 16))
-    return run_gather<__nv_bfloat16>(pl, static_cast<const __nv_bfloat16 *>(input), lds, output, F, st);
+  const bool overwrite = flags & NTS_PLAN_OVERWRITE;
+  if (dtype == NTS_DTYPE_BF16 && lds % 8 == 0 && aligned_to(input, 16) && !(flags & NTS_PLAN_COPY_INPUT))
+    return run_gather<__nv_bfloat16>(pl, static_cast<const __nv_bfloat16 *>(input), lds, output, F, overwrite, st);
   const uint32_t ld = (F + 7u) & ~7u;
   if (const int rc = ensure_workspace(pl->workspace_bf16, pl->workspace_bf16_elems, (size_t)pl->gather_rows * ld))
     return rc;
   if (const int rc = to_bf16_rows(input, dtype, lds, pl->workspace_bf16, pl->gather_rows, F, ld, st))
     return rc;
-  return run_gather<__nv_bfloat16>(pl, pl->workspace_bf16, ld, output, F, st);
+  return run_gather<__nv_bfloat16>(pl, pl->workspace_bf16, ld, output, F, overwrite, st);
 }
 
 }
@@ -1510,7 +1559,7 @@
       float t = 0.f;
       if (cudaEventRecord(e0, st) != cudaSuccess ||
           (bf16 ? run_plan_bf16(pl, x, NTS_DTYPE_BF16, feature_size, y, feature_size, st)
-                : run_plan(pl, x, y, feature_size, st)) != 0 ||
+                : run_plan(pl, x, feature_size, y, feature_size, 0, st)) != 0 ||
           cudaEventRecord(e1, st) != cudaSuccess || cudaEventSynchronize(e1) != cudaSuccess ||
           cudaEventElapsedTime(&t, e0, e1) != cudaSuccess)
         return false;
@@ -1562,7 +1611,8 @@
 
 static nts_gather_plan *create_tuned(const nts_vid_t *offsets, const nts_vid_t *indices, const float *weight,
                                      const nts_vid_t *slot_of, nts_vid_t index_base, nts_vid_t n_rows, uint64_t n_edges,
-                                     nts_vid_t gather_rows, nts_vid_t feature_size, bool bf16, void *stream) {
+                                     nts_vid_t gather_rows, nts_vid_t feature_size, bool bf16, int run_flags,
+                                     void *stream) {
   cudaStream_t st = as_stream(stream);
   const uint64_t row_bytes = bf16 ? ((feature_size + 7ull) & ~7ull) * 2ull : ((feature_size + 3ull) & ~3ull) * 4ull;
   const int s_max = pick_slabs_for_rows(gather_rows, n_edges, n_rows, row_bytes, 16ull << 20);
@@ -1581,8 +1631,8 @@
             cudaMemsetAsync(x, 0, xb, st) == cudaSuccess && cudaMemsetAsync(y, 0, yb, st) == cudaSuccess &&
             cudaEventCreate(&e0) == cudaSuccess && cudaEventCreate(&e1) == cudaSuccess;
   auto run_one = [&](nts_gather_plan *pl) {
-    return bf16 ? run_plan_bf16(pl, x, NTS_DTYPE_BF16, feature_size, y, feature_size, st)
-                : run_plan(pl, x, y, feature_size, st);
+    return bf16 ? run_plan_bf16(pl, x, NTS_DTYPE_BF16, feature_size, y, feature_size, st, run_flags)
+                : run_plan(pl, x, feature_size, y, feature_size, run_flags, st);
   };
   auto time_plan = [&](nts_gather_plan *pl, float *ms) -> bool {
     *ms = 1e30f;
@@ -1676,7 +1726,7 @@
                                               uint64_t n_edges, nts_vid_t gather_rows, nts_vid_t feature_size,
                                               void *stream) {
   return create_tuned(offsets, indices, weight, slot_of, index_base, n_rows, n_edges, gather_rows, feature_size, false,
-                      stream);
+                      0, stream);
 }
 
 nts_gather_plan *nts_gather_plan_create_tuned_bf16(const nts_vid_t *offsets, const nts_vid_t *indices,
@@ -1684,7 +1734,21 @@
                                                    nts_vid_t n_rows, uint64_t n_edges, nts_vid_t gather_rows,
                                                    nts_vid_t feature_size, void *stream) {
   return create_tuned(offsets, indices, weight, slot_of, index_base, n_rows, n_edges, gather_rows, feature_size, true,
-                      stream);
+                      0, stream);
+}
+
+nts_gather_plan *nts_gather_plan_create_tuned_ex(const nts_vid_t *offsets, const nts_vid_t *indices,
+                                                 const float *weight, const nts_vid_t *slot_of, nts_vid_t index_base,
+                                                 nts_vid_t n_rows, uint64_t n_edges, nts_vid_t gather_rows,
+                                                 nts_vid_t feature_size, int gather_dtype, int run_flags,
+                                                 void *stream) {
+  if ((gather_dtype != NTS_DTYPE_F32 && gather_dtype != NTS_DTYPE_BF16) || (run_flags & ~NTS_PLAN_OVERWRITE)) {
+    fail(-1, "nts_gather_plan_create_tuned_ex: gather_dtype must be NTS_DTYPE_F32 or NTS_DTYPE_BF16, run_flags 0 or "
+             "NTS_PLAN_OVERWRITE", __FILE__, __LINE__);
+    return nullptr;
+  }
+  return create_tuned(offsets, indices, weight, slot_of, index_base, n_rows, n_edges, gather_rows, feature_size,
+                      gather_dtype == NTS_DTYPE_BF16, run_flags, stream);
 }
 
 int nts_gather_plan_destroy(nts_gather_plan *pl) {
@@ -1745,13 +1809,29 @@
 
 int nts_gather_plan_run(nts_gather_plan *pl, const float *input, float *output, nts_vid_t feature_size, void *stream) {
   NTS_ARG_CHECK(pl != nullptr, "null plan");
-  return run_plan(pl, input, output, feature_size, as_stream(stream));
+  return run_plan(pl, input, feature_size, output, feature_size, 0, as_stream(stream));
+}
+
+int nts_gather_plan_run_ex(nts_gather_plan *pl, const float *input, nts_vid_t input_ld, float *output,
+                           nts_vid_t feature_size, int flags, void *stream) {
+  NTS_ARG_CHECK(input_ld >= feature_size, "input row pitch below the feature width");
+  NTS_ARG_CHECK(output != nullptr || feature_size == 0, "null output pointer");
+  NTS_ARG_CHECK(pl != nullptr, "null plan");
+  return run_plan(pl, input, input_ld, output, feature_size, flags, as_stream(stream));
 }
 
 int nts_gather_plan_run_bf16(nts_gather_plan *pl, const void *input, int input_dtype, float *output,
                              nts_vid_t feature_size, void *stream) {
   NTS_ARG_CHECK(pl != nullptr, "null plan");
   return run_plan_bf16(pl, input, input_dtype, feature_size, output, feature_size, as_stream(stream));
+}
+
+int nts_gather_plan_run_bf16_ex(nts_gather_plan *pl, const void *input, int input_dtype, nts_vid_t input_ld,
+                                float *output, nts_vid_t feature_size, int flags, void *stream) {
+  NTS_ARG_CHECK(input_ld >= feature_size, "input row pitch below the feature width");
+  NTS_ARG_CHECK(output != nullptr || feature_size == 0, "null output pointer");
+  NTS_ARG_CHECK(pl != nullptr, "null plan");
+  return run_plan_bf16(pl, input, input_dtype, input_ld, output, feature_size, as_stream(stream), flags);
 }
 
 int nts_rows_to_bf16(const void *src, int src_dtype, nts_vid_t lds, void *dst, nts_vid_t n_rows, nts_vid_t feature_size,
diff --git a/neutronstarlite_b200/ops.py b/neutronstarlite_b200/ops.py
--- a/neutronstarlite_b200/ops.py
+++ b/neutronstarlite_b200/ops.py
@@ -12,13 +12,17 @@
     return torch.cuda.current_stream().cuda_stream
 
 
-def _check_input(t, name="input"):
+def row_pitched(t):
+    return t.dim() == 2 and (t.is_contiguous() or (t.stride(1) == 1 and t.stride(0) >= t.shape[1]))
+
+
+def _check_input(t, name="input", pitched=False):
     if not t.is_cuda:
         raise _lib.NtsError("%s must be a CUDA tensor (libnts_b200 has no CPU fallback)" % name)
     if t.dtype != torch.float32 or t.dim() != 2:
         raise _lib.NtsError("%s must be a 2-D float32 tensor" % name)
-    if not t.is_contiguous():
-        raise _lib.NtsError("%s must be contiguous" % name)
+    if not (t.is_contiguous() or (pitched and row_pitched(t))):
+        raise _lib.NtsError("%s must be contiguous" % name + (" or row-pitched" if pitched else ""))
     return t
 
 
@@ -28,19 +32,20 @@
     return gather_dtype
 
 
-def _check_gathered(t, name, gather_dtype):
+def _check_gathered(t, name, gather_dtype, pitched=False):
     if gather_dtype is None or (t.is_cuda and t.dtype == torch.float32):
-        return _check_input(t, name)
+        return _check_input(t, name, pitched)
     if not t.is_cuda:
         raise _lib.NtsError("%s must be a CUDA tensor (libnts_b200 has no CPU fallback)" % name)
     if t.dtype != torch.bfloat16 or t.dim() != 2:
         raise _lib.NtsError("%s must be a 2-D float32 or bfloat16 tensor" % name)
-    if not t.is_contiguous():
-        raise _lib.NtsError("%s must be contiguous" % name)
+    if not (t.is_contiguous() or (pitched and row_pitched(t))):
+        raise _lib.NtsError("%s must be contiguous" % name + (" or row-pitched" if pitched else ""))
     return t
 
 
 _DTYPE_CODE = {torch.float32: 0, torch.bfloat16: 1}
+PLAN_OVERWRITE, PLAN_COPY_INPUT = 1, 2
 
 
 def _ptr(t):
@@ -102,7 +107,7 @@
 class GatherPlan:
 
     def __init__(self, offsets, indices, weight, index_base, n_rows, n_edges, gather_rows, slabs, slot_of=None,
-                 tune_for=0, hubs=(0, 0), gather_dtype=None):
+                 tune_for=0, hubs=(0, 0), gather_dtype=None, tune_accumulate=True):
         L = _lib.load()
         _check_gather_dtype(gather_dtype)
         t0 = _time.perf_counter()
@@ -112,9 +117,10 @@
                                                           int(gather_rows), int(slabs), int(hubs[0]), int(hubs[1]),
                                                           _stream())
         else:
-            create = L.nts_gather_plan_create_tuned_bf16 if gather_dtype is not None else L.nts_gather_plan_create_tuned
-            self.handle = create(_ptr(offsets), _ptr(indices), _ptr(weight), _ptr(slot_of), int(index_base),
-                                 int(n_rows), int(n_edges), int(gather_rows), int(tune_for), _stream())
+            self.handle = L.nts_gather_plan_create_tuned_ex(
+                _ptr(offsets), _ptr(indices), _ptr(weight), _ptr(slot_of), int(index_base), int(n_rows), int(n_edges),
+                int(gather_rows), int(tune_for), _DTYPE_CODE[gather_dtype or torch.float32],
+                0 if tune_accumulate else PLAN_OVERWRITE, _stream())
         self.build_s = _time.perf_counter() - t0
         if not self.handle:
             raise _lib.NtsError("nts_gather_plan_create failed: " + L.nts_last_error().decode(errors="replace"))
@@ -135,16 +141,23 @@
         return ((self.slabs,) + ((self.hub_cols, self.hub_rows) if self.hub_cols or self.hub_rows else ())
                 + (("overlap",) if self.overlap else ()))
 
-    def run(self, x, out, gather_dtype=None):
+    def run(self, x, out, gather_dtype=None, accumulate=True):
+        if not row_pitched(x):
+            raise _lib.NtsError("the gathered input must have contiguous rows (unit column stride)")
+        F = int(x.shape[1])
+        ld = F if x.is_contiguous() else int(x.stride(0))
+        flags = 0 if accumulate else PLAN_OVERWRITE
+        if ld != F and (x.storage_offset() + x.shape[0] * ld) * x.element_size() > x.untyped_storage().nbytes():
+            flags |= PLAN_COPY_INPUT
         if _check_gather_dtype(gather_dtype) is not None:
             if x.dtype not in _DTYPE_CODE:
                 raise _lib.NtsError("BF16 gathers take a float32 or bfloat16 input, not %s" % x.dtype)
-            _lib.call("nts_gather_plan_run_bf16", self.handle, _ptr(x), _DTYPE_CODE[x.dtype], _ptr(out),
-                      int(x.shape[1]), _stream())
+            _lib.call("nts_gather_plan_run_bf16_ex", self.handle, _ptr(x), _DTYPE_CODE[x.dtype], ld, _ptr(out), F,
+                      flags, _stream())
             return out
         if x.dtype == torch.bfloat16:
             raise _lib.NtsError("a bfloat16 input needs gather_dtype=torch.bfloat16")
-        _lib.call("nts_gather_plan_run", self.handle, _ptr(x), _ptr(out), int(x.shape[1]), _stream())
+        _lib.call("nts_gather_plan_run_ex", self.handle, _ptr(x), ld, _ptr(out), F, flags, _stream())
         return out
 
     def bytes(self):
@@ -190,11 +203,11 @@
         if direction == "fwd":
             plan = GatherPlan(chunk.column_offset_gpu, chunk.row_indices_gpu, chunk.edge_weight_forward_gpu,
                               chunk.src_range[0], n_rows, chunk.edge_size, gather_rows, _plan_slabs, tune_for=int(F),
-                              gather_dtype=gather_dtype)
+                              gather_dtype=gather_dtype, tune_accumulate=False)
         else:
             plan = GatherPlan(chunk.row_offset_gpu, chunk.column_indices_gpu, chunk.edge_weight_backward_gpu,
                               chunk.dst_range[0], n_rows, chunk.edge_size, gather_rows, _plan_slabs, tune_for=int(F),
-                              gather_dtype=gather_dtype)
+                              gather_dtype=gather_dtype, tune_accumulate=False)
         share = (direction,) + plan.key()
         if share in plans:
             plan = plans[share]
@@ -212,14 +225,21 @@
     return _chunk_plan(chunk, direction, F, gather_dtype)
 
 
-def gather_by_dst_from_src(chunk, out, x, with_weight=True, gather_dtype=None):
+def _plain_operands(out, x, accumulate):
+    if not accumulate:
+        out.zero_()
+    return x.contiguous()
+
+
+def gather_by_dst_from_src(chunk, out, x, with_weight=True, gather_dtype=None, accumulate=True):
     plan = _bf16_plan(chunk, "fwd", x.shape[1], with_weight, gather_dtype)
     ev = _timer.bracket("fwd", x.shape[1], chunk.edge_size, chunk.batch_size_forward) if _timer else None
     if ev:
         ev[0].record()
     if plan is not None:
-        plan.run(x, out, gather_dtype)
+        plan.run(x, out, gather_dtype, accumulate)
     else:
+        x = _plain_operands(out, x, accumulate)
         _lib.call("nts_gather_by_dst_from_src", _ptr(x), _ptr(out), _ptr(chunk.edge_weight_forward_gpu),
                   _ptr(chunk.row_indices_gpu), _ptr(chunk.column_offset_gpu), chunk.src_range[0], chunk.src_range[1],
                   chunk.dst_range[0], chunk.dst_range[1], chunk.edge_size, chunk.batch_size_forward,
@@ -229,14 +249,15 @@
     return out
 
 
-def gather_by_src_from_dst(chunk, out, grad, with_weight=True, gather_dtype=None):
+def gather_by_src_from_dst(chunk, out, grad, with_weight=True, gather_dtype=None, accumulate=True):
     plan = _bf16_plan(chunk, "bwd", grad.shape[1], with_weight, gather_dtype)
     ev = _timer.bracket("bwd", grad.shape[1], chunk.edge_size, chunk.batch_size_backward) if _timer else None
     if ev:
         ev[0].record()
     if plan is not None:
-        plan.run(grad, out, gather_dtype)
+        plan.run(grad, out, gather_dtype, accumulate)
     else:
+        grad = _plain_operands(out, grad, accumulate)
         _lib.call("nts_gather_by_src_from_dst", _ptr(grad), _ptr(out), _ptr(chunk.edge_weight_backward_gpu),
                   _ptr(chunk.row_offset_gpu), _ptr(chunk.column_indices_gpu), chunk.src_range[0], chunk.src_range[1],
                   chunk.dst_range[0], chunk.dst_range[1], chunk.edge_size, chunk.batch_size_backward,
@@ -269,16 +290,16 @@
         self.gather_dtype = _check_gather_dtype(gather_dtype)
 
     def forward(self, f_input, f_input1=None):
-        x = _check_gathered(f_input, "input", self.gather_dtype)
+        x = _check_gathered(f_input, "input", self.gather_dtype, pitched=True)
         c = self.partitioned_graph_.graph_chunks[0]
-        y = torch.zeros((c.batch_size_forward, x.shape[1]), dtype=torch.float32, device=x.device)
-        return gather_by_dst_from_src(c, y, x, gather_dtype=self.gather_dtype)
-
-    def backward(self, f_output_grad):
-        g = _check_input(f_output_grad, "output_grad")
+        y = torch.empty((c.batch_size_forward, x.shape[1]), dtype=torch.float32, device=x.device)
+        return gather_by_dst_from_src(c, y, x, gather_dtype=self.gather_dtype, accumulate=False)
+
+    def backward(self, f_output_grad):
+        g = _check_input(f_output_grad, "output_grad", pitched=True)
         c = self.partitioned_graph_.graph_chunks[0]
-        dx = torch.zeros((c.batch_size_backward, g.shape[1]), dtype=torch.float32, device=g.device)
-        return gather_by_src_from_dst(c, dx, g, gather_dtype=self.gather_dtype)
+        dx = torch.empty((c.batch_size_backward, g.shape[1]), dtype=torch.float32, device=g.device)
+        return gather_by_src_from_dst(c, dx, g, gather_dtype=self.gather_dtype, accumulate=False)
 
 
 class ForwardGPUfuseOp(ntsGraphOp):
diff --git a/neutronstarlite_b200/toolkits.py b/neutronstarlite_b200/toolkits.py
--- a/neutronstarlite_b200/toolkits.py
+++ b/neutronstarlite_b200/toolkits.py
@@ -95,12 +95,19 @@
         self.train_rows = (self.MASK == 0).nonzero().view(-1)
         self.X = [None] * len(self.layers)
         self.gather_dtype = ops._check_gather_dtype(gather_dtype)
-        if self.gather_dtype is not None and self._input_is_gathered:
-            features = features.detach().to(self.gather_dtype)
-        self.X[0] = features.requires_grad_(True)
         if op_class is None:
             op_class = ops.ForwardSingleGPUfuseOp if partitioned_graph.partitions == 1 else ops.ForwardGPUfuseOp
         self.op_class = op_class
+        self._pitched_input = (self._input_is_gathered and self.gather_dtype is None and
+                               isinstance(op_class, type) and issubclass(op_class, ops.ForwardSingleGPUfuseOp))
+        if self.gather_dtype is not None and self._input_is_gathered:
+            features = features.detach().to(self.gather_dtype)
+        elif self._pitched_input and features.is_cuda and features.dim() == 2 and features.shape[1] % 4:
+            F = features.shape[1]
+            padded = torch.zeros((features.shape[0], (F + 3) // 4 * 4), dtype=features.dtype, device=features.device)
+            padded[:, :F].copy_(features.detach())
+            features = padded[:, :F]
+        self.X[0] = features.requires_grad_(True)
         self.op_kwargs = dict(op_kwargs or {})
         if self.gather_dtype is not None:
             self.op_kwargs["gather_dtype"] = self.gather_dtype
@@ -119,7 +126,8 @@
                 dropped = torch.nn.functional.dropout(x_i, self.drop_rate, training=True)
                 self.ctx.appendNNOp(x_i, dropped)
                 x_i = dropped
-            x_i = x_i.contiguous()
+            if not (self._pitched_input and ops.row_pitched(x_i)):
+                x_i = x_i.contiguous()
             y_i = self.ctx.runGraphOp(self.op_class, self.pg, None, x_i, **self.op_kwargs)
             self.X[i + 1] = self.ctx.runVertexForward(lambda n, v, _l=i: self.vertexForward(n, v, _l), y_i, x_i)
 
```

After: 16.25 billion (median of 6 runs). +6.1%, better.
